# weilonghu/KGC-GCN

Hardware: NVIDIA B200
Metric: edges/sec GCN fwd+bwd (higher is better)
Workload: dtype f32

## Files before the change

### include/kgc_b200.h

```cpp
#ifndef KGC_B200_H_
#define KGC_B200_H_

#include <stddef.h>
#include <stdint.h>

#ifdef __cplusplus
extern "C" {
#endif
#if defined(__GNUC__)
#pragma GCC visibility push(default)
#endif

#define KGC_ABI_VERSION 1

typedef struct { int32_t beg, end, out, flags; } kgc_item_t;

#define KGC_CHUNK_EDGES 32
typedef struct { int32_t head_slot, tail_slot; } kgc_chunk_t;

typedef struct { int32_t eid, a, b; float norm; } kgc_edge_rec_t;

const char* kgc_last_error(void);
int kgc_abi_version(void);

size_t kgc_csr_workspace_bytes(int64_t n_edges2, int64_t n_nodes, int64_t n_types);
int kgc_csr_build(const int64_t* src, const int64_t* dst, const int64_t* type,
                  int64_t n_edges2, int64_t n_edges_in, int64_t n_nodes, int64_t n_dst_rows, int64_t dst_offset,
                  int64_t n_types, int32_t deg_given, int32_t* deg, float* norm,
                  int32_t* perm_dst, int32_t* rowptr_dst, int32_t* rowmid_dst, kgc_edge_rec_t* rec_dst,
                  int32_t* perm_src, int32_t* rowptr_src, kgc_edge_rec_t* rec_src,
                  int32_t* perm_type, int32_t* rowptr_type, kgc_edge_rec_t* rec_type,
                  int64_t type_block_rows, void* workspace, size_t workspace_bytes, void* stream);
int64_t kgc_csr_type_rows(int64_t n_nodes, int64_t n_types, int64_t type_block_rows);
int kgc_block_sum(const float* in, int64_t n_blocks, int64_t n, float* out, void* stream);

int kgc_stream_plan_flags(const int32_t* seg_beg, const int32_t* seg_end, const int32_t* seg_row, int64_t n_seg,
                          int64_t n_rec, int32_t chunk, uint32_t* rowflags, int32_t* rec_seg, int32_t* inter, void* stream);

int kgc_agg_fwd(const float* x, const float* rel, int64_t n_types, const float* ee,
                const kgc_edge_rec_t* rec_dst, const uint32_t* rowflags, const kgc_chunk_t* chunks, int64_t n_rec,
                float* out_final, float* carry, int32_t D, void* stream);

int kgc_rows_fill(const int32_t* rows, int64_t n_rows, const float* addend, float* out, int32_t D, void* stream);

int kgc_rows_reduce(const float* part_in, const kgc_item_t* items, int64_t n_items, int64_t n_large,
                    float* out_final, float* out_part, const float* addend, int32_t D, void* stream);

int kgc_agg_bwd_src(const float* x, const float* rel, int64_t n_types, const float* ee, const float* g3,
                    const kgc_edge_rec_t* rec_src, const uint32_t* rowflags, const kgc_chunk_t* chunks, int64_t n_rec,
                    int64_t n_dst_rows, int64_t n_edges_in, const float* loop_addend,
                    float* d_ee, float* dx_final, float* carry, int32_t D, void* stream);

int kgc_agg_bwd_rel(const float* x, const float* ee, const float* g3,
                    const kgc_edge_rec_t* rec_type, const uint32_t* rowflags, const kgc_chunk_t* chunks, int64_t n_rec,
                    int64_t n_dst_rows, int64_t n_edges_in,
                    float* drel_final, float* carry, int32_t D, void* stream);

int64_t kgc_tail_num_blocks(int64_t n_rows);
int kgc_dropout_mask(const int64_t* seed, int32_t plane, float drop_p, int64_t n_elem, uint8_t* mask, void* stream);
int32_t kgc_keep_pitch(void);
int kgc_tail_fwd(const float* res3, const uint8_t* mask_in, const uint8_t* mask_out, const int64_t* seed, float drop_p,
                 float keep_scale, const float* bias, int64_t n_rows, int32_t Dout, float* pre, double* partials,
                 uint8_t* keep, void* stream);
int kgc_colsum_finalize(const double* partials, int64_t n_blocks, int32_t Dout, double* sums, void* stream);
int kgc_colstats_from_sums(const double* sums, int64_t n_rows, int32_t Dout, float eps, int32_t training,
                           const float* running_mean, const float* running_var, float* stats, void* stream);
int kgc_colstats_finalize(const double* partials, int64_t n_blocks, int64_t n_rows, int32_t Dout, float eps,
                          float momentum, float* running_mean, float* running_var, int64_t* num_batches_tracked,
                          double* sums, float* stats, void* stream);
int kgc_colsum_finalize2(const double* partials, int64_t n_blocks, int32_t Dout, double* sums, float* sums32,
                         void* stream);
int kgc_tail_apply(const float* pre, const float* stats, const float* gamma, const float* beta,
                   int64_t n_rows, int32_t Dout, float* all_ent, const int64_t* out_seed, float out_drop_p,
                   uint8_t* out_keep, void* stream);
int kgc_tail_bwd_reduce(const float* g_ent, const float* pre, const float* stats, const float* gamma, const float* beta,
                        int64_t n_rows, int32_t Dout, double* partials, const uint8_t* out_keep, float out_scale,
                        void* stream);
int kgc_tail_bwd_apply(const float* g_ent, const float* pre, const float* stats, const float* gamma, const float* beta,
                       const double* sums, int32_t training, int64_t n_rows, int64_t n_rows_global, int32_t Dout,
                       float* d_out, const uint8_t* keep, float keep_scale, float* d_res2, const uint8_t* out_keep,
                       float out_scale, void* stream);

int kgc_conv_prep(const float* rels, int32_t n_rels, const float* loop_rel, const float* loop_edge, const float* w_in,
                  const float* w_out, const float* w_loop, const float* w_rel, int32_t D, int32_t Dout, float* relp,
                  float* all_rel, float* packed_fwd, float* packed_bwd, void* stream);
int kgc_conv_param_grads(const float* m_loop, const float* w_loop, const float* loop_rel, const float* loop_edge,
                         const float* relp, const float* w_rel, const float* g_rel, const float* d_relp,
                         int32_t n_rels, int32_t D, int32_t Dout, float* d_w_loop, float* d_loop_rel,
                         float* d_loop_edge, float* d_rels, float* d_w_rel, const float* rel_add, void* stream);

size_t kgc_gemm_packed_b_bytes(int32_t N, int32_t K);
int kgc_gemm_pack_b(const float* B, int64_t stride_k, int64_t stride_n, int32_t N, int32_t K, float* packed,
                    void* stream);
int kgc_gemm_nt(const float* A, int64_t M, int32_t K, int64_t lda, const float* packed_b, int32_t N, float* C,
                int64_t ldc, void* stream);
int kgc_gemm_nt_batch(int32_t n_prob, const float* const* A, int64_t M, int32_t K, int64_t lda,
                      const float* const* packed_b, int32_t N, float* const* C, int64_t ldc, void* stream);
int kgc_gemm_nt_batch_masked(int32_t n_prob, const float* const* A, int64_t M, int32_t K, int64_t lda,
                             const float* const* packed_b, int32_t N, float* const* C, int64_t ldc, const uint8_t* keep,
                             int32_t keep_pitch, float keep_scale, void* stream);
int kgc_gemm_nt_trans(const float* At, int64_t M, int32_t K, int64_t ldat, const float* packed_b, int32_t N,
                      float* Ct, int64_t ldct, void* stream);
void kgc_gemm_set_debug(long long* buf);

size_t kgc_gemm_tn_workspace_bytes(int64_t M, int32_t Ka, int32_t Nb);
int kgc_gemm_tn(const float* A, int64_t lda, const float* B, int64_t ldb, int64_t M, int32_t Ka, int32_t Nb,
                float* C, void* workspace, size_t workspace_bytes, void* stream);

size_t kgc_gemm_tn_tc_workspace_bytes(int64_t M, int32_t Ka, int32_t Nb);
int kgc_gemm_tn_tc(const float* A, int64_t lda, const float* B, int64_t ldb, int64_t M, int32_t Ka, int32_t Nb,
                   float* C, void* workspace, size_t workspace_bytes, void* stream);

int kgc_gemm_nt_splitk(const float* A, int64_t lda, const float* Bt, int64_t ldb, int64_t K, int32_t Ma, int32_t Nb,
                       float* C, void* workspace, size_t workspace_bytes, void* stream);

int kgc_gemm_tn_tc_batch(int32_t n_prob, const float* const* A, int64_t lda, const float* const* B, int64_t ldb,
                         int64_t M, int32_t Ka, int32_t Nb, float* const* C, void* workspace, size_t workspace_bytes,
                         void* stream);
int kgc_gemm_tn_tc_batch_masked(int32_t n_prob, const float* const* A, int64_t lda, const float* const* B, int64_t ldb,
                                int64_t M, int32_t Ka, int32_t Nb, float* const* C, void* workspace, size_t workspace_bytes,
                                const uint8_t* keep, int32_t keep_pitch, float keep_scale, void* stream);

int kgc_label_build(const int64_t* qid, int64_t B, const int64_t* triples, const int64_t* ptr,
                    const int32_t* idx, int64_t n_entity, float pos, float add,
                    int64_t* triple_out, float* label, void* stream);

int kgc_neg_sample(const int64_t* qid, int64_t B, const int64_t* ptr, const int32_t* idx, int64_t n_entity,
                   const uint32_t* draws, int32_t k, int32_t tries, int32_t* neg, void* stream);

int kgc_edge_sample(const int64_t* src, const int64_t* dst, const int64_t* type, int64_t n_triples, const uint32_t* draws,
                    int64_t m, int64_t* sub_src, int64_t* sub_dst, int64_t* sub_type, int64_t* eids, void* stream);

size_t kgc_bn2d_partials_bytes(int32_t C);
int kgc_bn2d_relu_drop_fwd(const float* x, int64_t B, int32_t C, int32_t HW, const float* gamma, const float* beta,
                           float* running_mean, float* running_var, float eps, float momentum, int32_t training,
                           int32_t relu, const int64_t* seed, float drop_p, double* partials, float* stats, float* y,
                           void* stream);
int kgc_bn2d_relu_drop_bwd(const float* dy, const float* x, int64_t B, int32_t C, int32_t HW, const float* gamma,
                           const float* beta, const float* stats, int32_t training, int32_t relu, const int64_t* seed,
                           float drop_p, double* partials, float* sums, float* dx, void* stream);

int kgc_conv1ch_supported(int32_t F, int32_t K, int32_t H, int32_t W);
size_t kgc_conv1ch_bwd_workspace_bytes(int64_t B, int32_t F, int32_t K);
int kgc_conv1ch_fwd(const float* x, const float* w, const float* bias, int64_t B, int32_t F, int32_t K, int32_t H,
                    int32_t W, float* y, void* stream);
int kgc_conv1ch_bwd(const float* dy, const float* x, const float* w, int64_t B, int32_t F, int32_t K, int32_t H,
                    int32_t W, float* dx, float* dw, void* workspace, void* stream);

typedef struct { float* param; const float* grad; float* exp_avg; float* exp_avg_sq; } kgc_opt_tensor_t;
int32_t kgc_opt_chunk_elems(void);
int kgc_clip_adam_step(const kgc_opt_tensor_t* tensors, const int32_t* items, int64_t n_items, const float* hyper,
                       double* state, double* partials, void* stream);

int kgc_p2p_allreduce(void* const* stage_ptrs_dev, int64_t offset_bytes, void* const* flag_ptrs_dev, int32_t rank,
                      int32_t world, uint32_t* epoch, int32_t* error, const void* in, void* out, int64_t n_bytes,
                      int32_t is_double, void* stream);
int kgc_p2p_barrier(void* const* flag_ptrs_dev, int32_t rank, int32_t world, uint32_t* epoch, int32_t* error, void* stream);
int kgc_p2p_halo_gather(void* const* table_ptrs_dev, int32_t rank, const int32_t* rows, const int32_t* order, int64_t n_rows,
                        int64_t block_rows, int32_t D, void* stream);
int kgc_p2p_halo_reduce(void* const* part_ptrs_dev, int32_t world, const int32_t* idx, const int32_t* row_ids, int64_t n_rows,
                        const float* addend, float* out, int32_t D, void* stream);

typedef struct kgc_ingest kgc_ingest_t;
int kgc_ingest_open(const char* data_dir, kgc_ingest_t** out);
void kgc_ingest_close(kgc_ingest_t* h);
int64_t kgc_ingest_count(const kgc_ingest_t* h, int32_t what);
int kgc_ingest_copy(const kgc_ingest_t* h, int32_t array, void* dst, int64_t capacity_bytes);
const char* kgc_ingest_name(const kgc_ingest_t* h, int32_t kind, int64_t id);

int kgc_score_1n_fwd(const float* ent, int64_t n_ent, int32_t D, int64_t ld_ent, const float* packed_x, int32_t B,
                     const float* bias, float* pred, int64_t ld_pred, void* stream);
int kgc_score_1n_logits(const float* ent, int64_t n_ent, int32_t D, int64_t ld_ent, const float* packed_x, int32_t B,
                        const float* bias, float* logits, int64_t ld_logits, void* stream);
int kgc_score_1n_bwd_logit(const float* d_pred, int64_t ld_dp, const float* pred, int64_t ld_p, int64_t n_ent,
                           int32_t B, int32_t ldt, float* d_logitT, float* d_bias, void* stream);

int64_t kgc_label_mask_words(int64_t n_entity);
int kgc_label_mask_build(const int64_t* qid, int64_t B, const int64_t* triples, const int64_t* ptr, const int32_t* idx,
                         int64_t n_entity, uint32_t* mask, int64_t* triple_out, void* stream);
int kgc_bce_1n_bwd_logit(const float* pred, int64_t ld_p, const uint32_t* mask, int64_t n_ent, int32_t B, int32_t ldt,
                         float pos, float add, float* d_logitT, float* d_bias, double* loss_partial, float* loss,
                         void* stream);
int kgc_score_1n_fwd_t(const float* ent, int64_t n_ent, int32_t D, int64_t ld_ent, const float* packed_x, int32_t B,
                       const float* bias, float* pred_t, int64_t ld_t, void* stream);
int64_t kgc_bce_1n_t_blocks(int64_t n_ent);
int kgc_label_mask_t_build(const int64_t* qid, int64_t B, const int64_t* ptr, const int32_t* idx, int64_t n_entity,
                           uint32_t* mask_t, void* stream);
int kgc_bce_1n_bwd_logit_t(float* pred_t, const uint32_t* mask_t, int64_t n_ent, int32_t B, int32_t ldt, float pos, float add,
                           float* d_bias, double* loss_partial, float* loss, void* stream);

int32_t kgc_score_kpad(int32_t d);
int kgc_score_pack_entities(const float* all_ent, const float* bias, int64_t n, int32_t d,
                            uint16_t* e_bf16, void* stream);
int kgc_score_pack_queries(const float* xq, int64_t b, int32_t d, uint16_t* q_bf16, void* stream);
size_t kgc_score_pairs_workspace_bytes(int64_t n_pairs, int32_t kpad);
int kgc_score_pairs(const uint16_t* q_bf16, const uint16_t* e_bf16, const int32_t* pair_q, const int32_t* pair_e,
                    int64_t n_pairs, int32_t kpad, float* s_out, void* workspace, size_t workspace_bytes,
                    void* stream);
int kgc_score_rank(const uint16_t* q_bf16, const uint16_t* e_bf16, int64_t b, int64_t n, int32_t kpad,
                   const float* thr, int32_t* count_gt, int32_t* count_eq, void* stream);
int kgc_rank_count_dense(const float* logits, int64_t ld, int64_t n_ent, int64_t b, const float* thr,
                         int32_t* count_gt, int32_t* count_eq, void* stream);
int kgc_rank_finalize(const int32_t* count_gt, const int32_t* count_eq, const float* thr, const float* s_filt,
                      const int64_t* filt_ptr, const int32_t* filt_idx, const int64_t* obj, int64_t b,
                      int32_t* ranks, int32_t* eq_out, double* sums13, void* stream);

#if defined(__GNUC__)
#pragma GCC visibility pop
#endif
#ifdef __cplusplus
}
#endif
#endif
```

### kgc-gcn_b200/_lib.py

```python
import ctypes
import os

import torch

_HERE = os.path.dirname(os.path.abspath(__file__))
LIB_PATH = os.environ.get('KGC_LIB_PATH') or os.path.join(_HERE, 'libkgc_b200.so')
_LIB = None

_vp, _i64, _i32, _f32, _sz = ctypes.c_void_p, ctypes.c_int64, ctypes.c_int32, ctypes.c_float, ctypes.c_size_t

SIGNATURES = {
    'kgc_last_error': (ctypes.c_char_p, []),
    'kgc_abi_version': (ctypes.c_int, []),
    'kgc_csr_workspace_bytes': (_sz, [_i64, _i64, _i64]),
    'kgc_csr_build': (ctypes.c_int, [_vp, _vp, _vp, _i64, _i64, _i64, _i64, _i64, _i64, _i32, _vp, _vp, _vp, _vp, _vp,
                                     _vp, _vp, _vp, _vp, _vp, _vp, _vp, _i64, _vp, _sz, _vp]),
    'kgc_csr_type_rows': (_i64, [_i64, _i64, _i64]),
    'kgc_block_sum': (ctypes.c_int, [_vp, _i64, _i64, _vp, _vp]),
    'kgc_stream_plan_flags': (ctypes.c_int, [_vp, _vp, _vp, _i64, _i64, _i32, _vp, _vp, _vp, _vp]),
    'kgc_agg_fwd': (ctypes.c_int, [_vp, _vp, _i64, _vp, _vp, _vp, _vp, _i64, _vp, _vp, _i32, _vp]),
    'kgc_rows_fill': (ctypes.c_int, [_vp, _i64, _vp, _vp, _i32, _vp]),
    'kgc_rows_reduce': (ctypes.c_int, [_vp, _vp, _i64, _i64, _vp, _vp, _vp, _i32, _vp]),
    'kgc_agg_bwd_src': (ctypes.c_int, [_vp, _vp, _i64, _vp, _vp, _vp, _vp, _vp, _i64, _i64, _i64, _vp, _vp, _vp, _vp, _i32, _vp]),
    'kgc_agg_bwd_rel': (ctypes.c_int, [_vp, _vp, _vp, _vp, _vp, _vp, _i64, _i64, _i64, _vp, _vp, _i32, _vp]),
    'kgc_tail_num_blocks': (_i64, [_i64]),
    'kgc_dropout_mask': (ctypes.c_int, [_vp, _i32, _f32, _i64, _vp, _vp]),
    'kgc_keep_pitch': (_i32, []),
    'kgc_tail_fwd': (ctypes.c_int, [_vp, _vp, _vp, _vp, _f32, _f32, _vp, _i64, _i32, _vp, _vp, _vp, _vp]),
    'kgc_colsum_finalize': (ctypes.c_int, [_vp, _i64, _i32, _vp, _vp]),
    'kgc_colstats_from_sums': (ctypes.c_int, [_vp, _i64, _i32, _f32, _i32, _vp, _vp, _vp, _vp]),
    'kgc_colstats_finalize': (ctypes.c_int, [_vp, _i64, _i64, _i32, _f32, _f32, _vp, _vp, _vp, _vp, _vp, _vp]),
    'kgc_colsum_finalize2': (ctypes.c_int, [_vp, _i64, _i32, _vp, _vp, _vp]),
    'kgc_tail_apply': (ctypes.c_int, [_vp, _vp, _vp, _vp, _i64, _i32, _vp, _vp, _f32, _vp, _vp]),
    'kgc_tail_bwd_reduce': (ctypes.c_int, [_vp, _vp, _vp, _vp, _vp, _i64, _i32, _vp, _vp, _f32, _vp]),
    'kgc_tail_bwd_apply': (ctypes.c_int, [_vp, _vp, _vp, _vp, _vp, _vp, _i32, _i64, _i64, _i32, _vp, _vp, _f32, _vp, _vp, _f32, _vp]),
    'kgc_gemm_packed_b_bytes': (_sz, [_i32, _i32]),
    'kgc_gemm_pack_b': (ctypes.c_int, [_vp, _i64, _i64, _i32, _i32, _vp, _vp]),
    'kgc_gemm_nt': (ctypes.c_int, [_vp, _i64, _i32, _i64, _vp, _i32, _vp, _i64, _vp]),
    'kgc_conv_prep': (ctypes.c_int, [_vp, _i32] + [_vp] * 6 + [_i32, _i32] + [_vp] * 5),
    'kgc_conv_param_grads': (ctypes.c_int, [_vp] * 8 + [_i32, _i32, _i32] + [_vp] * 7),
    'kgc_gemm_nt_batch': (ctypes.c_int, [_i32, _vp, _i64, _i32, _i64, _vp, _i32, _vp, _i64, _vp]),
    'kgc_gemm_nt_batch_masked': (ctypes.c_int, [_i32, _vp, _i64, _i32, _i64, _vp, _i32, _vp, _i64, _vp, _i32, _f32, _vp]),
    'kgc_gemm_tn_tc_batch_masked': (ctypes.c_int, [_i32, _vp, _i64, _vp, _i64, _i64, _i32, _i32, _vp, _vp, _sz, _vp, _i32, _f32, _vp]),
    'kgc_gemm_nt_trans': (ctypes.c_int, [_vp, _i64, _i32, _i64, _vp, _i32, _vp, _i64, _vp]),
    'kgc_gemm_nt_splitk': (ctypes.c_int, [_vp, _i64, _vp, _i64, _i64, _i32, _i32, _vp, _vp, _sz, _vp]),
    'kgc_gemm_set_debug': (None, [_vp]),
    'kgc_gemm_tn_workspace_bytes': (_sz, [_i64, _i32, _i32]),
    'kgc_gemm_tn_tc_workspace_bytes': (_sz, [_i64, _i32, _i32]),
    'kgc_gemm_tn_tc': (ctypes.c_int, [_vp, _i64, _vp, _i64, _i64, _i32, _i32, _vp, _vp, _sz, _vp]),
    'kgc_gemm_tn_tc_batch': (ctypes.c_int, [_i32, _vp, _i64, _vp, _i64, _i64, _i32, _i32, _vp, _vp, _sz, _vp]),
    'kgc_gemm_tn': (ctypes.c_int, [_vp, _i64, _vp, _i64, _i64, _i32, _i32, _vp, _vp, _sz, _vp]),
    'kgc_label_build': (ctypes.c_int, [_vp, _i64, _vp, _vp, _vp, _i64, _f32, _f32, _vp, _vp, _vp]),
    'kgc_neg_sample': (ctypes.c_int, [_vp, _i64, _vp, _vp, _i64, _vp, _i32, _i32, _vp, _vp]),
    'kgc_edge_sample': (ctypes.c_int, [_vp, _vp, _vp, _i64, _vp, _i64, _vp, _vp, _vp, _vp, _vp]),
    'kgc_bn2d_partials_bytes': (_sz, [_i32]),
    'kgc_bn2d_relu_drop_fwd': (ctypes.c_int, [_vp, _i64, _i32, _i32, _vp, _vp, _vp, _vp, _f32, _f32, _i32, _i32, _vp, _f32, _vp, _vp, _vp, _vp]),
    'kgc_bn2d_relu_drop_bwd': (ctypes.c_int, [_vp, _vp, _i64, _i32, _i32, _vp, _vp, _vp, _i32, _i32, _vp, _f32, _vp, _vp, _vp, _vp]),
    'kgc_conv1ch_supported': (_i32, [_i32, _i32, _i32, _i32]),
    'kgc_conv1ch_bwd_workspace_bytes': (_sz, [_i64, _i32, _i32]),
    'kgc_conv1ch_fwd': (ctypes.c_int, [_vp, _vp, _vp, _i64, _i32, _i32, _i32, _i32, _vp, _vp]),
    'kgc_conv1ch_bwd': (ctypes.c_int, [_vp, _vp, _vp, _i64, _i32, _i32, _i32, _i32, _vp, _vp, _vp, _vp]),
    'kgc_opt_chunk_elems': (_i32, []),
    'kgc_clip_adam_step': (ctypes.c_int, [_vp, _vp, _i64, _vp, _vp, _vp, _vp]),
    'kgc_p2p_allreduce': (ctypes.c_int, [_vp, _i64, _vp, _i32, _i32, _vp, _vp, _vp, _vp, _i64, _i32, _vp]),
    'kgc_p2p_barrier': (ctypes.c_int, [_vp, _i32, _i32, _vp, _vp, _vp]),
    'kgc_p2p_halo_gather': (ctypes.c_int, [_vp, _i32, _vp, _vp, _i64, _i64, _i32, _vp]),
    'kgc_p2p_halo_reduce': (ctypes.c_int, [_vp, _i32, _vp, _vp, _i64, _vp, _vp, _i32, _vp]),
    'kgc_ingest_open': (ctypes.c_int, [ctypes.c_char_p, _vp]),
    'kgc_ingest_close': (None, [_vp]),
    'kgc_ingest_count': (_i64, [_vp, _i32]),
    'kgc_ingest_copy': (ctypes.c_int, [_vp, _i32, _vp, _i64]),
    'kgc_ingest_name': (ctypes.c_char_p, [_vp, _i32, _i64]),
    'kgc_score_1n_fwd': (ctypes.c_int, [_vp, _i64, _i32, _i64, _vp, _i32, _vp, _vp, _i64, _vp]),
    'kgc_score_1n_logits': (ctypes.c_int, [_vp, _i64, _i32, _i64, _vp, _i32, _vp, _vp, _i64, _vp]),
    'kgc_rank_count_dense': (ctypes.c_int, [_vp, _i64, _i64, _i64, _vp, _vp, _vp, _vp]),
    'kgc_score_1n_bwd_logit': (ctypes.c_int, [_vp, _i64, _vp, _i64, _i64, _i32, _i32, _vp, _vp, _vp]),
    'kgc_label_mask_words': (_i64, [_i64]),
    'kgc_label_mask_build': (ctypes.c_int, [_vp, _i64, _vp, _vp, _vp, _i64, _vp, _vp, _vp]),
    'kgc_bce_1n_bwd_logit': (ctypes.c_int, [_vp, _i64, _vp, _i64, _i32, _i32, _f32, _f32, _vp, _vp, _vp, _vp, _vp]),
    'kgc_score_1n_fwd_t': (ctypes.c_int, [_vp, _i64, _i32, _i64, _vp, _i32, _vp, _vp, _i64, _vp]),
    'kgc_bce_1n_t_blocks': (_i64, [_i64]),
    'kgc_label_mask_t_build': (ctypes.c_int, [_vp, _i64, _vp, _vp, _i64, _vp, _vp]),
    'kgc_bce_1n_bwd_logit_t': (ctypes.c_int, [_vp, _vp, _i64, _i32, _i32, _f32, _f32, _vp, _vp, _vp, _vp]),
    'kgc_score_kpad': (_i32, [_i32]),
    'kgc_score_pack_entities': (ctypes.c_int, [_vp, _vp, _i64, _i32, _vp, _vp]),
    'kgc_score_pack_queries': (ctypes.c_int, [_vp, _i64, _i32, _vp, _vp]),
    'kgc_score_pairs_workspace_bytes': (_sz, [_i64, _i32]),
    'kgc_score_pairs': (ctypes.c_int, [_vp, _vp, _vp, _vp, _i64, _i32, _vp, _vp, _sz, _vp]),
    'kgc_score_rank': (ctypes.c_int, [_vp, _vp, _i64, _i64, _i32, _vp, _vp, _vp, _vp]),
    'kgc_rank_finalize': (ctypes.c_int, [_vp, _vp, _vp, _vp, _vp, _vp, _vp, _i64, _vp, _vp, _vp, _vp]),
}


def lib():
    global _LIB
    if _LIB is None:
        if not os.path.exists(LIB_PATH):
            raise RuntimeError('{} is missing: build it with `python -c "import __graft_entry__ as g; g.build()"` '
                               '(nvcc, sm_100a). There is no CPU or PyTorch fallback.'.format(LIB_PATH))
        handle = ctypes.CDLL(LIB_PATH)
        for name, (res, args) in SIGNATURES.items():
            fn = getattr(handle, name)
            fn.restype, fn.argtypes = res, args
        if handle.kgc_abi_version() != 1:
            raise RuntimeError('libkgc_b200.so ABI version mismatch')
        _LIB = handle
    return _LIB


LAUNCHES = 0
_KERNELS_PER_CALL = {'kgc_csr_build': 16, 'kgc_label_mask_build': 2, 'kgc_bce_1n_bwd_logit': 2, 'kgc_bce_1n_bwd_logit_t': 2, 'kgc_label_mask_t_build': 2, 'kgc_score_pairs': 3, 'kgc_rank_finalize': 2, 'kgc_gemm_tn': 2, 'kgc_gemm_tn_tc': 2, 'kgc_gemm_tn_tc_batch': 2, 'kgc_gemm_tn_tc_batch_masked': 2}


def call(name, *args):
    global LAUNCHES
    h = lib()
    LAUNCHES += _KERNELS_PER_CALL.get(name, 1)
    rc = getattr(h, name)(*args)
    if rc != 0:
        raise RuntimeError('{} failed: {}'.format(name, h.kgc_last_error().decode('utf-8', 'replace')))


_WARNED = set()


def library_path(site, reason):
    msg = 'kgc_gcn_b200: {} is running on the torch library path ({})'.format(site, reason)
    if os.environ.get('KGC_STRICT', '0') not in ('', '0'):
        raise RuntimeError(msg + ' and KGC_STRICT=1 forbids it')
    if site not in _WARNED:
        _WARNED.add(site)
        import warnings
        warnings.warn(msg, RuntimeWarning, stacklevel=3)


def ptr(t):
    return None if t is None else ctypes.c_void_p(t.data_ptr())


def stream():
    return ctypes.c_void_p(torch.cuda.current_stream().cuda_stream)


def require_cuda(t, dtype, name):
    if not (torch.is_tensor(t) and t.is_cuda):
        raise RuntimeError('{} must be a CUDA tensor: the M-GCN hot path runs on the GPU only (no CPU fallback)'.format(name))
    if t.dtype != dtype:
        raise TypeError('{} must be {}, got {}'.format(name, dtype, t.dtype))
    return t if t.is_contiguous() else t.contiguous()
```

### kgc-gcn_b200/conv.py

```python
import os

import torch
import torch.nn as nn

from . import _lib
from .plan import get_plan


def get_param(shape):
    param = nn.Parameter(torch.empty(*shape))
    nn.init.xavier_uniform_(param.data)
    return param


def _mm(a, b, out):
    return torch.mm(a, b, out=out)


def gemm_nt(a, b_kn, out, plan=None, tag='b', packed=None):
    M, K = a.shape
    N = out.shape[1]
    if a.stride(1) != 1 or out.stride(1) != 1:
        raise ValueError('gemm_nt needs unit inner strides')
    p = _lib.ptr
    if packed is None:
        nbytes = int(_lib.lib().kgc_gemm_packed_b_bytes(N, K))
        if nbytes == 0:
            raise ValueError('gemm_nt: unsupported shape K={} N={}'.format(K, N))
        packed = plan.scratch('gemm_pack_' + tag, (nbytes // 4,)) if plan is not None else \
            torch.empty((nbytes // 4,), dtype=torch.float32, device=a.device)
        _lib.call('kgc_gemm_pack_b', p(b_kn), b_kn.stride(0), b_kn.stride(1), N, K, p(packed), _lib.stream())
    dst = out if (out.data_ptr() % 16 == 0 and out.stride(0) % 4 == 0) else \
        torch.empty((M, (N + 3) // 4 * 4), dtype=torch.float32, device=a.device)[:, :N]
    _lib.call('kgc_gemm_nt', p(a), M, K, a.stride(0), p(packed), N, p(dst), dst.stride(0), _lib.stream())
    if dst is not out:
        out.copy_(dst)
    return out


def gemm_nt_batch(a_list, packed_list, out_list, keep=None, keep_scale=1.0):
    import ctypes
    n = len(a_list)
    M, K = a_list[0].shape
    N = out_list[0].shape[1]
    lda, ldc = a_list[0].stride(0), out_list[0].stride(0)
    for a, o in zip(a_list, out_list):
        if a.shape != (M, K) or o.shape != (M, N) or a.stride() != (lda, 1) or o.stride() != (ldc, 1):
            raise ValueError('gemm_nt_batch needs operands of identical shape and strides')
    arr = lambda ts: (ctypes.c_void_p * n)(*[t.data_ptr() for t in ts])
    if keep is not None:
        _lib.call('kgc_gemm_nt_batch_masked', n, arr(a_list), M, K, lda, arr(packed_list), N, arr(out_list), ldc,
                  _lib.ptr(keep), keep.stride(0), float(keep_scale), _lib.stream())
    else:
        _lib.call('kgc_gemm_nt_batch', n, arr(a_list), M, K, lda, arr(packed_list), N, arr(out_list), ldc, _lib.stream())
    return out_list


def gemm_tn_batch(a_list, b_list, out_list, plan=None, keep=None, keep_scale=1.0):
    import ctypes
    n = len(a_list)
    M, Ka = a_list[0].shape
    Nb = b_list[0].shape[1]
    lda, ldb = a_list[0].stride(0), b_list[0].stride(0)
    same = all(a.shape == (M, Ka) and b.shape == (M, Nb) and a.stride() == (lda, 1) and b.stride() == (ldb, 1)
               and o.is_contiguous() for a, b, o in zip(a_list, b_list, out_list))
    if not same or Ka > 128 or Nb > 224:
        if keep is not None:
            raise ValueError('gemm_tn_batch: the masked form needs Ka <= 128, Nb <= 224 and operands of identical shape')
        for a, b, o in zip(a_list, b_list, out_list):
            gemm_tn(a, b, o, plan)
        return out_list
    nbytes = int(_lib.lib().kgc_gemm_tn_tc_workspace_bytes(M, Ka, Nb))
    ws = plan.scratch('kgc_gemm_tn_tc_ws', (nbytes // 4,)) if plan is not None else \
        torch.empty((nbytes // 4,), dtype=torch.float32, device=a_list[0].device)
    arr = lambda ts: (ctypes.c_void_p * n)(*[t.data_ptr() for t in ts])
    if keep is not None:
        _lib.call('kgc_gemm_tn_tc_batch_masked', n, arr(a_list), lda, arr(b_list), ldb, M, Ka, Nb, arr(out_list), _lib.ptr(ws),
                  nbytes, _lib.ptr(keep), keep.stride(0), float(keep_scale), _lib.stream())
    else:
        _lib.call('kgc_gemm_tn_tc_batch', n, arr(a_list), lda, arr(b_list), ldb, M, Ka, Nb, arr(out_list), _lib.ptr(ws), nbytes,
                  _lib.stream())
    return out_list


def _pack_b(b_kn):
    K, N = b_kn.shape
    nbytes = int(_lib.lib().kgc_gemm_packed_b_bytes(N, K))
    if nbytes == 0:
        raise ValueError('unsupported small operand K={} N={} (K <= 256, N <= 1024)'.format(K, N))
    packed = torch.empty((nbytes // 4,), dtype=torch.float32, device=b_kn.device)
    _lib.call('kgc_gemm_pack_b', _lib.ptr(b_kn), b_kn.stride(0), b_kn.stride(1), N, K, _lib.ptr(packed), _lib.stream())
    return packed


def gemm_nt_trans(a_t, b_kn, out_t):
    K, M = a_t.shape
    N = b_kn.shape[1]
    if a_t.stride(1) != 1 or out_t.stride(1) != 1 or out_t.shape != (N, M):
        raise ValueError('gemm_nt_trans needs unit inner strides and out_t of shape [N, M]')
    p = _lib.ptr
    _lib.call('kgc_gemm_nt_trans', p(a_t), M, K, a_t.stride(0), p(_pack_b(b_kn)), N, p(out_t), out_t.stride(0), _lib.stream())
    return out_t


def gemm_nt_splitk(a, bt, out):
    Ma, K = a.shape
    Nb = bt.shape[0]
    if a.stride(1) != 1 or bt.stride(1) != 1 or not out.is_contiguous():
        raise ValueError('gemm_nt_splitk needs unit inner strides and a contiguous output')
    nbytes = int(_lib.lib().kgc_gemm_tn_tc_workspace_bytes(K, Ma, Nb))
    ws = torch.empty((nbytes // 4,), dtype=torch.float32, device=a.device)
    p = _lib.ptr
    _lib.call('kgc_gemm_nt_splitk', p(a), a.stride(0), p(bt), bt.stride(0), K, Ma, Nb, p(out), p(ws), nbytes, _lib.stream())
    return out


class _LinearFn(torch.autograd.Function):

    @staticmethod
    def forward(ctx, x, weight, bias):
        x_, w_ = x.detach(), weight.detach()
        y = gemm_nt_splitk(x_, w_, torch.empty((x_.shape[0], w_.shape[0]), dtype=torch.float32, device=x.device))
        if bias is not None:
            y += bias.detach()
        ctx.save_for_backward(x_, w_)
        ctx.has_bias = bias is not None
        return y

    @staticmethod
    def backward(ctx, dy):
        x, w = ctx.saved_tensors
        dy = dy.contiguous()
        dx = dw = db = None
        if ctx.needs_input_grad[0]:
            dx = gemm_nt_trans(w, dy.t(), torch.empty_like(x))
        if ctx.needs_input_grad[1]:
            dw = gemm_nt_trans(x, dy, torch.empty_like(w))
        if ctx.has_bias and ctx.needs_input_grad[2]:
            db = dy.sum(0)
        return dx, dw, db


def linear_tc_supported(x, weight):
    B, F = x.shape
    O = weight.shape[0]
    return (x.is_cuda and x.dtype == torch.float32 and weight.dtype == torch.float32 and x.is_contiguous()
            and weight.is_contiguous() and 0 < B <= 128 and O <= 224 and O % 4 == 0 and F % 32 == 0 and F >= 4096
            and x.data_ptr() % 16 == 0 and weight.data_ptr() % 16 == 0)


def linear_tc(x, weight, bias=None):
    return _LinearFn.apply(x, weight, bias)


def gemm_tn(a, b, out, plan=None, tensor_cores=True):
    M, Ka = a.shape
    Nb = b.shape[1]
    if a.stride(1) != 1 or b.stride(1) != 1 or not out.is_contiguous():
        raise ValueError('gemm_tn needs unit inner strides and a contiguous output')
    if Nb > 256:
        raise ValueError('gemm_tn supports Nb <= 256')
    name = 'kgc_gemm_tn_tc' if (tensor_cores and Nb <= 224) else 'kgc_gemm_tn'
    for i0 in range(0, Ka, 128):
        kb = min(128, Ka - i0)
        a_blk, out_blk = a[:, i0:i0 + kb], out[i0:i0 + kb]
        nbytes = int(getattr(_lib.lib(), name + '_workspace_bytes')(M, kb, Nb))
        ws = plan.scratch(name + '_ws', (nbytes // 4,)) if plan is not None else \
            torch.empty((nbytes // 4,), dtype=torch.float32, device=a.device)
        p = _lib.ptr
        _lib.call(name, p(a_blk), a.stride(0), p(b), b.stride(0), M, kb, Nb, p(out_blk), p(ws), nbytes, _lib.stream())
    return out


class _Done(object):

    def wait(self):
        return None


class _StreamJoin(object):

    def __init__(self, stream):
        self.stream = stream

    def wait(self):
        torch.cuda.current_stream().wait_stream(self.stream)


class _Collectives(object):

    def __init__(self, group, world, n_global, n_hub=0, hub_idx_mine=None, hub_rows_mine=None, p2p=None, rank=0,
                 halo_rows=None, n_loc=None):
        self.group, self.world, self.n_global, self.rank = group, int(world), int(n_global), int(rank)
        self.n_loc = None if n_loc is None else int(n_loc)
        self.p2p = p2p
        self.halo_rows = halo_rows
        self.n_hub, self.hub_idx_mine, self.hub_rows_mine = int(n_hub), hub_idx_mine, hub_rows_mine

    def sum_hub_rows(self, planes, n_loc):
        if self.n_hub == 0:
            return
        buf = planes[:, n_loc:, :].contiguous()
        self.all_reduce(buf, 'hub_f')
        if self.hub_idx_mine.numel():
            planes[:, self.hub_rows_mine, :] = buf[:, self.hub_idx_mine, :]

    def spread_hub_rows(self, planes, n_planes, n_loc):
        if self.n_hub == 0:
            return
        buf = torch.zeros((n_planes, self.n_hub, planes.shape[2]), dtype=planes.dtype, device=planes.device)
        if self.hub_idx_mine.numel():
            buf[:, self.hub_idx_mine, :] = planes[:n_planes, self.hub_rows_mine, :]
        self.all_reduce(buf, 'hub_b')
        planes[:n_planes, n_loc:, :] = buf

    def all_gather_rows(self, x_local, async_op=False):
        import torch.distributed as dist
        out = torch.empty((self.world * x_local.shape[0],) + tuple(x_local.shape[1:]), dtype=x_local.dtype,
                          device=x_local.device)
        work = dist.all_gather_into_tensor(out, x_local.contiguous(), group=self.group, async_op=async_op)
        return (out, work) if async_op else out

    def gather_compact(self, x_blk):
        full = self.all_gather_rows(x_blk)
        return torch.cat([x_blk, full.index_select(0, self.halo_rows)], 0)

    def reduce_compact(self, partial, block):
        full = partial.new_zeros((self.world * block, partial.shape[1]))
        full[self.rank * block:(self.rank + 1) * block] = partial[:block]
        full[self.halo_rows] = partial[block:block + self.halo_rows.numel()]
        return self.reduce_scatter_rows(full)

    def reduce_scatter_rows(self, full, async_op=False):
        import torch.distributed as dist
        rows = full.shape[0] // self.world
        if dist.get_backend(self.group) == 'gloo':
            dist.all_reduce(full, group=self.group)
            r = dist.get_rank(self.group)
            out = full[r * rows:(r + 1) * rows].clone()
            return (out, None) if async_op else out
        out = torch.empty((rows,) + tuple(full.shape[1:]), dtype=full.dtype, device=full.device)
        work = dist.reduce_scatter_tensor(out, full.contiguous(), group=self.group, async_op=async_op)
        return (out, work) if async_op else out

    def all_reduce(self, t, tag=None):
        if self.p2p is not None and tag is not None and self.p2p.all_reduce(t, tag):
            return t
        import torch.distributed as dist
        dist.all_reduce(t, group=self.group)
        return t


class _ConvFn(torch.autograd.Function):

    @staticmethod
    def forward(ctx, x, rels, ee, w_in, w_out, w_loop, w_rel, loop_rel, loop_edge, gamma, beta, bias,
                plan, mask_in, mask_out, keep_scale, training, running_mean, running_var, eps, coll, seed, drop_p,
                bn_track=None, out_drop=None):
        Nl, D = x.shape
        Dout = w_in.shape[1]
        p, st = _lib.ptr, _lib.stream
        x = _lib.require_cuda(x, torch.float32, 'x')
        ee = _lib.require_cuda(ee, torch.float32, 'edge_embs')
        n_global = Nl if coll is None else coll.n_global
        n_hub = 0 if coll is None else coll.n_hub
        n_loc = Nl if coll is None or coll.n_loc is None else coll.n_loc
        if not 0 <= n_loc - Nl <= 1:
            raise ValueError('x has {} rows, the partition expects {} or {}'.format(Nl, n_loc, n_loc - 1))
        Nb = n_loc + n_hub
        compact = coll is not None and coll.halo_rows is not None
        n_table = Nl if coll is None else (Nb + coll.halo_rows.numel() if compact else Nb * coll.world)
        hybrid = coll is not None and coll.p2p is not None and coll.p2p.hybrid
        n_dst = n_table if hybrid else Nb
        if ee.shape[0] != plan.num_edges2 or n_dst != plan.num_dst_rows or plan.num_nodes != n_table:
            raise ValueError('edge_embs / x do not match the graph plan')
        T = rels.shape[0] + 1
        if T != plan.num_types:
            raise ValueError('rels_embs rows + 1 must equal the number of edge types of the plan')
        nf = int(_lib.lib().kgc_gemm_packed_b_bytes(Dout, D)) // 4
        nbk = int(_lib.lib().kgc_gemm_packed_b_bytes(D, Dout)) // 4
        if nf == 0 or nbk == 0:
            raise ValueError('unsupported layer width {} -> {} (<= 256)'.format(D, Dout))
        relp = torch.empty((T, D), dtype=torch.float32, device=x.device)
        all_rel_pad = torch.empty((T, Dout), dtype=torch.float32, device=x.device)
        packed_f = torch.empty((3, nf), dtype=torch.float32, device=x.device)
        packed_b = torch.empty((4, nbk), dtype=torch.float32, device=x.device)
        rels_c, wts = rels.detach().contiguous(), [w.detach().contiguous() for w in (w_in, w_out, w_loop, w_rel)]
        main, side = torch.cuda.current_stream(), plan.side_stream()
        side.wait_stream(main)
        with torch.cuda.stream(side):
            _lib.call('kgc_conv_prep', p(rels_c), T - 1, p(loop_rel.detach()), p(loop_edge.detach()), p(wts[0]), p(wts[1]),
                      p(wts[2]), p(wts[3]), D, Dout, p(relp), p(all_rel_pad), p(packed_f), p(packed_b), st())
        gather = None
        if coll is None:
            x_full = x
        elif coll.p2p is not None:
            ex = coll.p2p.exchange_stream
            ex.wait_stream(main)
            with torch.cuda.stream(ex):
                x_full = coll.p2p.gather(x, fence=not training)
            gather = _StreamJoin(ex)
        elif compact:
            x_blk = x if Nb == Nl else torch.cat([x, x.new_zeros((Nb - Nl, D))], 0)
            x_full, gather = coll.gather_compact(x_blk), _Done()
        else:
            x_full, gather = coll.all_gather_rows(x if Nb == Nl else torch.cat([x, x.new_zeros((Nb - Nl, D))], 0),
                                                  async_op=True)

        res3 = plan.scratch('res3', (3, Nl, Dout))
        if gather is not None:
            main.wait_stream(side)
            gemm_nt(x, None, res3[2], packed=packed_f[2])
            gather.wait()
        if max(x_full.shape[0], 3 * n_dst, ee.shape[0]) * (D // 4) >= 1 << 32:
            raise ValueError('kgc_gcn_b200: node / edge tables of 2^32 float4 elements or more are not supported')
        agg = torch.empty((2, n_dst, D), dtype=torch.float32, device=x.device)

        def level0(sp, out_final, carry):
            _lib.call('kgc_agg_fwd', p(x_full), p(rels_c), T - 1, p(ee), p(plan.rec_dst), p(sp.rowflags), p(sp.chunks), sp.n_rec,
                      p(out_final), p(carry), D, st())
        plan.run_reduction(plan.fwd, level0, agg, D, tag='f')
        if gather is None:
            main.wait_stream(side)

        if hybrid:
            coll.p2p.reduce_agg(agg)
        if gather is not None:
            coll.sum_hub_rows(agg, n_loc)
            gemm_nt_batch([agg[0, :Nl], agg[1, :Nl]], [packed_f[0], packed_f[1]], [res3[0], res3[1]])
        else:
            gemm_nt_batch([agg[0], agg[1], x], [packed_f[0], packed_f[1], packed_f[2]], [res3[0], res3[1], res3[2]])

        nb = int(_lib.lib().kgc_tail_num_blocks(Nl))
        partials = plan.scratch('colpart', (nb, 2, Dout), torch.float64)
        sums = torch.empty((2, Dout), dtype=torch.float64, device=x.device)
        pre = torch.empty((Nl, Dout), dtype=torch.float32, device=x.device)
        stats = torch.empty((3, Dout), dtype=torch.float32, device=x.device)
        all_ent = torch.empty((Nl, Dout), dtype=torch.float32, device=x.device)
        dropping = (mask_in is not None or seed is not None) and drop_p > 0.0
        keep = torch.empty((Nl, int(_lib.lib().kgc_keep_pitch())), dtype=torch.uint8, device=x.device) if dropping else None
        _lib.call('kgc_tail_fwd', p(res3), p(mask_in), p(mask_out), p(seed), float(drop_p), float(keep_scale), p(bias),
                  Nl, Dout, p(pre), p(partials), p(keep), st())
        if training and coll is None:
            mom, nbt = bn_track if bn_track is not None else (0.0, None)
            _lib.call('kgc_colstats_finalize', p(partials), nb, n_global, Dout, float(eps), float(mom),
                      p(running_mean) if bn_track is not None else None, p(running_var) if bn_track is not None else None,
                      p(nbt), None, p(stats), st())
        else:
            if training:
                _lib.call('kgc_colsum_finalize', p(partials), nb, Dout, p(sums), st())
                coll.all_reduce(sums, 'bn_f')
            _lib.call('kgc_colstats_from_sums', p(sums), n_global, Dout, float(eps), int(training), p(running_mean),
                      p(running_var), p(stats), st())
        out_p, out_seed = out_drop if out_drop is not None else (0.0, None)
        out_keep = torch.empty((Nl, int(_lib.lib().kgc_keep_pitch())), dtype=torch.uint8, device=x.device) if out_seed is not None else None
        _lib.call('kgc_tail_apply', p(pre), p(stats), p(gamma), p(beta), Nl, Dout, p(all_ent), p(out_seed), float(out_p),
                  p(out_keep), st())
        ctx.out_scale = 1.0 / (1.0 - float(out_p)) if out_seed is not None else 1.0
        all_rel = all_rel_pad[:-1]

        ctx.plan, ctx.training, ctx.keep_scale, ctx.has_bias, ctx.coll = plan, bool(training), float(keep_scale), \
            bias is not None, coll
        ctx.drop_p = float(drop_p)
        ctx.save_for_backward(x, x_full, relp, ee, w_in, w_out, w_loop, w_rel, loop_rel, loop_edge, gamma, beta, agg, pre,
                              all_ent, stats, keep, packed_b, out_keep)
        ctx.mark_non_differentiable(stats)
        return all_ent, all_rel, stats

    @staticmethod
    def backward(ctx, g_ent, g_rel, _g_stats):
        (x, x_full, relp, ee, w_in, w_out, w_loop, w_rel, loop_rel, loop_edge, gamma, beta, agg, pre, all_ent, stats, keep,
         packed_b, out_keep) = ctx.saved_tensors
        plan, coll = ctx.plan, ctx.coll
        Nl, D = x.shape
        n_global = Nl if coll is None else coll.n_global
        n_hub = 0 if coll is None else coll.n_hub
        n_loc = Nl if coll is None or coll.n_loc is None else coll.n_loc
        Nb = n_loc + n_hub
        Dout = w_in.shape[1]
        T = relp.shape[0]
        p, st = _lib.ptr, _lib.stream
        dev = x.device
        if g_ent is None:
            g_ent = torch.zeros_like(all_ent)
        g_ent = g_ent.contiguous()

        nb = int(_lib.lib().kgc_tail_num_blocks(Nl))
        partials = plan.scratch('colpart', (nb, 2, Dout), torch.float64)
        sums = torch.empty((2, Dout), dtype=torch.float64, device=dev)
        d_out = plan.scratch('d_out', (Nl, Dout))
        _lib.call('kgc_tail_bwd_reduce', p(g_ent), p(pre), p(stats), p(gamma), p(beta), Nl, Dout, p(partials), p(out_keep),
                  ctx.out_scale, st())
        if coll is None:
            sums32 = torch.empty((2, Dout), dtype=torch.float32, device=dev)
            _lib.call('kgc_colsum_finalize2', p(partials), nb, Dout, p(sums), p(sums32), st())
        else:
            _lib.call('kgc_colsum_finalize', p(partials), nb, Dout, p(sums), st())
            coll.all_reduce(sums, 'bn_b')
            sums32 = sums.float()
        mode = os.environ.get('KGC_TAIL_PLANES', '')
        three = (3 * Nl * Dout * 4 > (48 << 20)) if mode not in ('1', '3') else mode == '3'
        d_res2 = plan.scratch('d_res2', (2, Nl, Dout)) if three else None
        _lib.call('kgc_tail_bwd_apply', p(g_ent), p(pre), p(stats), p(gamma), p(beta), p(sums), int(ctx.training), Nl,
                  n_global, Dout, p(d_out), p(keep), ctx.keep_scale, p(d_res2), p(out_keep), ctx.out_scale, st())
        ups = [d_res2[0], d_res2[1], d_out] if three else [d_out, d_out, d_out]
        gkeep = None if three else keep
        d_beta, d_gamma = sums32[0], sums32[1]

        flat = torch.empty((3 * D * Dout + T * D + (Dout if ctx.has_bias else 0),), dtype=torch.float32, device=dev)
        d_w_in, d_w_out, m_loop = (flat[k * D * Dout:(k + 1) * D * Dout].view(D, Dout) for k in range(3))
        d_relp = flat[3 * D * Dout:3 * D * Dout + T * D].view(T, D)
        main, side = torch.cuda.current_stream(), plan.side_stream()
        side.wait_stream(main)
        with torch.cuda.stream(side):
            gemm_tn_batch([agg[0, :Nl], agg[1, :Nl], x], ups, [d_w_in, d_w_out, m_loop], plan,
                          keep=gkeep, keep_scale=ctx.keep_scale)
            if ctx.has_bias:
                torch.sum(d_out, 0, out=flat[3 * D * Dout + T * D:])

        hybrid = coll is not None and coll.p2p is not None and coll.p2p.hybrid
        g3 = coll.p2p.g3_planes() if hybrid else plan.scratch('g3', (3, Nb, D))
        gemm_nt_batch(ups, [packed_b[0], packed_b[1], packed_b[2]],
                      [g3[0, :Nl], g3[1, :Nl], g3[2, :Nl]], keep=gkeep, keep_scale=ctx.keep_scale)
        if n_hub:
            coll.spread_hub_rows(g3, 2, n_loc)
        if hybrid:
            coll.p2p.gather_g()
        p2p = None if coll is None else coll.p2p
        d_x_full = p2p.partial if (p2p is not None and not hybrid) else torch.empty((plan.num_nodes, D), dtype=torch.float32, device=dev)
        d_ee = torch.empty_like(ee)
        loop_addend = g3[2] if (coll is None or hybrid) else None

        def level0_src(sp, out_final, carry):
            _lib.call('kgc_agg_bwd_src', p(x_full), p(relp), relp.shape[0], p(ee), p(g3), p(plan.rec_src), p(sp.rowflags), p(sp.chunks),
                      sp.n_rec, plan.num_dst_rows, plan.num_edges_in, p(loop_addend), p(d_ee), p(out_final), p(carry),
                      D, st())
        plan.run_reduction(plan.bwd_src, level0_src, d_x_full, D, addend=loop_addend, tag='s')
        scatter = None
        if hybrid:
            ex = p2p.exchange_stream
            ex.wait_stream(main)
            with torch.cuda.stream(ex):
                p2p.reduce_dx(d_x_full, channel=1)
            d_x = d_x_full[:Nl]
        elif p2p is not None:
            d_x = torch.empty((Nl, D), dtype=torch.float32, device=dev)
            ex = p2p.exchange_stream
            ex.wait_stream(main)
            with torch.cuda.stream(ex):
                p2p.reduce(g3[2, :Nl], Nl, out=d_x, channel=1)
        compact = coll is not None and coll.halo_rows is not None
        if coll is not None and p2p is None and not compact:
            d_x, scatter = coll.reduce_scatter_rows(d_x_full, async_op=True)

        def level0_rel(sp, out_final, carry):
            _lib.call('kgc_agg_bwd_rel', p(x_full), p(ee), p(g3), p(plan.rec_type), p(sp.rowflags), p(sp.chunks), sp.n_rec,
                      plan.num_dst_rows, plan.num_edges_in, p(out_final), p(carry), D, st())
        plan.run_rel_reduction(level0_rel, d_relp, D)

        main.wait_stream(side)
        if coll is None:
            d_x = d_x_full
        elif p2p is not None:
            coll.all_reduce(flat, 'flat')
            main.wait_stream(p2p.exchange_stream)
        elif compact:
            coll.all_reduce(flat, 'flat')
            d_x = coll.reduce_compact(d_x_full, Nb)[:Nl] + g3[2, :Nl]
        else:
            coll.all_reduce(flat, 'flat')
            if scatter is not None:
                scatter.wait()
            d_x = d_x[:Nl] + g3[2, :Nl]
        d_bias = flat[3 * D * Dout + T * D:] * 3.0 if ctx.has_bias else None
        small = torch.empty((2 * D * Dout + 2 * D + (T - 1) * D,), dtype=torch.float32, device=dev)
        d_w_loop, d_w_rel = small[:D * Dout].view(D, Dout), small[D * Dout:2 * D * Dout].view(D, Dout)
        o = 2 * D * Dout
        d_loop_rel, d_loop_edge, d_rels = small[o:o + D].view(1, D), small[o + D:o + 2 * D].view(1, D), small[o + 2 * D:].view(T - 1, D)
        g_rel_c = None if g_rel is None else g_rel.contiguous()
        rel_add = None
        if g_rel_c is not None and T - 1 >= 256 and g_rel_c.data_ptr() % 16 == 0 and Dout % 4 == 0 and (D * Dout) % 32 == 0:
            rel_add = gemm_nt(g_rel_c, None, torch.empty((T - 1, D), dtype=torch.float32, device=dev), packed=packed_b[3])
            gemm_tn(relp[:T - 1], g_rel_c, d_w_rel, plan)
        _lib.call('kgc_conv_param_grads', p(m_loop), p(w_loop.detach().contiguous()), p(loop_rel.detach()), p(loop_edge.detach()),
                  p(relp), p(w_rel.detach().contiguous()), p(g_rel_c), p(d_relp), T - 1, D, Dout, p(d_w_loop), p(d_loop_rel),
                  p(d_loop_edge), p(d_rels), p(d_w_rel), p(rel_add), st())
        return (d_x, d_rels, d_ee, d_w_in, d_w_out, d_w_loop, d_w_rel, d_loop_rel, d_loop_edge, d_gamma, d_beta, d_bias,
                None, None, None, None, None, None, None, None, None, None, None, None, None)


class MGCNConv(nn.Module):

    def __init__(self, in_channels, out_channels, num_relations, bias=False, dropout=0.1, **kwargs):
        super(MGCNConv, self).__init__()
        self.in_channels = in_channels
        self.out_channels = out_channels
        self.num_relations = num_relations
        self.aggr = 'add'

        self.ent_bn = nn.BatchNorm1d(out_channels)
        self.drop = nn.Dropout(dropout)
        self.act = torch.tanh

        self.loop_weight = get_param((in_channels, out_channels))
        self.in_weight = get_param((in_channels, out_channels))
        self.out_weight = get_param((in_channels, out_channels))
        self.rels_weight = get_param((in_channels, out_channels))
        self.loop_rel = get_param((1, in_channels))
        self.loop_edge = get_param((1, in_channels))

        if bias is True:
            self.register_parameter('bias', nn.Parameter(torch.zeros(out_channels)))
        else:
            self.register_parameter('bias', None)
        self._forced_masks = None
        self.register_buffer('_drop_seed', torch.zeros(1, dtype=torch.int64), persistent=False)
        self._drop_seeded = False

    def set_dropout_masks(self, mask_in, mask_out):
        self._forced_masks = None if mask_in is None else (mask_in, mask_out)

    def compute_norm(self, edge_index, num_ent):
        ei = torch.cat([edge_index, edge_index], 1).contiguous()
        et = torch.zeros(ei.size(1), dtype=torch.int64, device=ei.device)
        return get_plan(ei, et, num_ent, 1).norm[:edge_index.size(1)].clone()

    def _masks(self, n_rows, device):
        p = self.drop.p
        if not self.training or p == 0.0:
            return None, None, 1.0, None, 0.0
        if self._forced_masks is not None:
            m_in, m_out = self._forced_masks
            return (m_in.to(device=device, dtype=torch.uint8).contiguous(),
                    m_out.to(device=device, dtype=torch.uint8).contiguous(), 1.0 / (1.0 - p), None, p)
        if not self._drop_seeded:
            self._drop_seed.fill_(int(torch.randint(0, 2 ** 62, (1,)).item()))
            self._drop_seeded = True
        self._drop_seed.add_(0x9E3779B97F4A7C15 & 0x7FFFFFFFFFFFFFFF)
        return None, None, 1.0 / (1.0 - p), self._drop_seed.clone(), p

    def _out_drop_cfg(self, p, seed):
        if not self.training or not p or p <= 0.0:
            return None
        if seed is None:
            if not self._drop_seeded:
                self._drop_seed.fill_(int(torch.randint(0, 2 ** 62, (1,)).item()))
                self._drop_seeded = True
            self._drop_seed.add_(0x9E3779B97F4A7C15 & 0x7FFFFFFFFFFFFFFF)
            seed = self._drop_seed.clone()
        self._last_out_seed = seed
        return float(p), seed

    def dropout_masks(self, seed, n_rows):
        out = []
        for plane in (0, 1):
            m = torch.empty((n_rows, self.out_channels), dtype=torch.uint8, device=seed.device)
            _lib.call('kgc_dropout_mask', _lib.ptr(seed), plane, float(self.drop.p), m.numel(), _lib.ptr(m), _lib.stream())
            out.append(m)
        return out

    def forward(self, x, edge_index, edge_type, edge_norm, edge_embs, rels_embs, size=None, _out_drop=0.0):
        num_ent = x.size(0)
        plan = get_plan(edge_index, edge_type, num_ent, rels_embs.size(0) + 1)
        m_in, m_out, keep_scale, seed, drop_p = self._masks(num_ent, x.device)
        self._last_seed = seed
        bn = self.ent_bn
        use_batch_stats = self.training or bn.running_mean is None
        track = self.training and bn.track_running_stats and bn.running_mean is not None
        fused = track and bn.momentum is not None
        all_ent, all_rel, stats = _ConvFn.apply(
            x, rels_embs, edge_embs, self.in_weight, self.out_weight, self.loop_weight, self.rels_weight,
            self.loop_rel, self.loop_edge, bn.weight, bn.bias, self.bias, plan, m_in, m_out, keep_scale,
            use_batch_stats, bn.running_mean, bn.running_var, bn.eps, None, seed, drop_p,
            (float(bn.momentum), bn.num_batches_tracked) if fused else None, self._out_drop_cfg(_out_drop, seed))
        if track and not fused:
            self._update_running_stats(stats, num_ent)
        return all_ent, all_rel

    def _update_running_stats(self, stats, n_rows):
        bn = self.ent_bn
        if self.training and bn.track_running_stats and bn.running_mean is not None:
            with torch.no_grad():
                bn.num_batches_tracked += 1
                mom = bn.momentum if bn.momentum is not None else 1.0 / float(bn.num_batches_tracked)
                unbias = float(n_rows) / float(max(n_rows - 1, 1))
                bn.running_mean.mul_(1.0 - mom).add_(stats[0], alpha=mom)
                bn.running_var.mul_(1.0 - mom).add_(stats[1], alpha=mom * unbias)

    def forward_partitioned(self, x_local, part, edge_embs_local, rels_embs):
        m_in, m_out, keep_scale, seed, drop_p = self._masks(x_local.size(0), x_local.device)
        if seed is not None:
            seed = seed + part.rank
        self._last_seed = seed
        bn = self.ent_bn
        use_batch_stats = self.training or bn.running_mean is None
        coll = _Collectives(part.group, part.world, part.num_nodes, part.n_hub, part.hub_idx_mine, part.hub_rows_mine,
                            part.p2p(x_local.shape[1]), part.rank, getattr(part, 'halo_rows64', None), part.n_loc)
        all_ent, all_rel, stats = _ConvFn.apply(
            x_local, rels_embs, edge_embs_local, self.in_weight, self.out_weight, self.loop_weight, self.rels_weight,
            self.loop_rel, self.loop_edge, bn.weight, bn.bias, self.bias, part.plan, m_in, m_out, keep_scale,
            use_batch_stats, bn.running_mean, bn.running_var, bn.eps, coll, seed, drop_p)
        self._update_running_stats(stats, part.num_nodes)
        return all_ent, all_rel

    def __repr__(self):
        return '{}({}, {}, num_relations={})'.format(self.__class__.__name__, self.in_channels, self.out_channels,
                                                     self.num_relations)
```

### kgc-gcn_b200/csrc/common.cuh

```cuda
#pragma once
#include <cuda_runtime.h>
#include <stdint.h>
#include <stdio.h>
#include <string>

#include "kgc_b200.h"

namespace kgc {

void set_error(const std::string& msg);

inline int fail(const char* where, const std::string& what) {
  set_error(std::string(where) + ": " + what);
  return 1;
}

#define KGC_CUDA_TRY(expr)                                                          \
  do {                                                                              \
    cudaError_t _e = (expr);                                                        \
    if (_e != cudaSuccess) return ::kgc::fail(__func__, std::string(#expr) + " -> " + cudaGetErrorString(_e)); \
  } while (0)

#define KGC_REQUIRE(cond, msg)                          \
  do {                                                  \
    if (!(cond)) return ::kgc::fail(__func__, (msg));   \
  } while (0)

#define KGC_LAUNCH_CHECK() KGC_CUDA_TRY(cudaGetLastError())

inline cudaStream_t as_stream(void* s) { return reinterpret_cast<cudaStream_t>(s); }

constexpr int kNumSMs = 148;

struct SmemAttrCache {
  size_t set[64] = {0};
  template <typename Kernel>
  cudaError_t ensure(Kernel kern, size_t smem) {
    int dev = 0;
    cudaError_t e = cudaGetDevice(&dev);
    if (e != cudaSuccess) return e;
    const bool tracked = dev >= 0 && dev < 64;
    if (tracked && smem <= set[dev]) return cudaSuccess;
    e = cudaFuncSetAttribute(kern, cudaFuncAttributeMaxDynamicSharedMemorySize, (int)smem);
    if (e == cudaSuccess && tracked) set[dev] = smem;
    return e;
  }
};

__host__ __device__ inline int64_t ceil_div(int64_t a, int64_t b) { return (a + b - 1) / b; }

__device__ __forceinline__ float4 ld_stream(const float4* p) {
  float4 r;
  asm volatile("ld.global.nc.L1::no_allocate.v4.f32 {%0,%1,%2,%3}, [%4];"
               : "=f"(r.x), "=f"(r.y), "=f"(r.z), "=f"(r.w)
               : "l"(p));
  return r;
}
__device__ __forceinline__ void st_stream(float4* p, const float4& v) {
  asm volatile("st.global.L1::no_allocate.v4.f32 [%0], {%1,%2,%3,%4};" ::"l"(p), "f"(v.x), "f"(v.y), "f"(v.z),
               "f"(v.w));
}
__device__ __forceinline__ int4 ld_rec(const kgc_edge_rec_t* p) {
  return __ldg(reinterpret_cast<const int4*>(p));
}

__device__ __forceinline__ uint4 philox4x32_10(uint4 c, uint2 k) {
#pragma unroll
  for (int r = 0; r < 10; ++r) {
    const uint32_t hi0 = __umulhi(0xD2511F53u, c.x), lo0 = 0xD2511F53u * c.x;
    const uint32_t hi1 = __umulhi(0xCD9E8D57u, c.z), lo1 = 0xCD9E8D57u * c.z;
    c = make_uint4(hi1 ^ c.y ^ k.x, lo1, hi0 ^ c.w ^ k.y, lo0);
    k.x += 0x9E3779B9u;
    k.y += 0xBB67AE85u;
  }
  return c;
}
__device__ __forceinline__ float4 philox_mask4(int64_t idx4, uint32_t plane, uint64_t seed, uint32_t drop_thr, float s) {
  const uint4 r = philox4x32_10(make_uint4((uint32_t)idx4, (uint32_t)(idx4 >> 32), plane, 0u),
                                make_uint2((uint32_t)seed, (uint32_t)(seed >> 32)));
  return make_float4(r.x >= drop_thr ? s : 0.f, r.y >= drop_thr ? s : 0.f, r.z >= drop_thr ? s : 0.f,
                     r.w >= drop_thr ? s : 0.f);
}

inline void ensure_thread_context() {
  static thread_local bool done = false;
  if (!done) {
    cudaFree(nullptr);
    done = true;
  }
}

}
```

### kgc-gcn_b200/csrc/gemm_tf32x3.cu

```cuda
#include <cuda.h>

#include <cstdlib>
#include "common.cuh"

namespace kgc {
namespace {

constexpr int kBM = 128;
constexpr int kBK = 32;
constexpr int kUK = 8;
constexpr int kMaxKB = 8;
constexpr int kMaxStages = 8;
constexpr int kAStages = 4;
constexpr int kAccCols = 256;
constexpr int kTmemColsTS = kAccCols + kAStages * 64;
constexpr int kTileA = kBM * kBK * 4;
constexpr int kThreadsG = 480;
constexpr int kSplitWarps = 8;
constexpr int kBBudget = 116 * 1024;
constexpr int kTmemColsG = 256;
constexpr int kEpiBuf = 32 * 128;
constexpr int kEpiStage = 4 * 2 * kEpiBuf;

__device__ __forceinline__ uint32_t s_u32(const void* p) { return (uint32_t)__cvta_generic_to_shared(p); }
__device__ __forceinline__ void mb_init(uint64_t* bar, uint32_t count) {
  asm volatile("mbarrier.init.shared::cta.b64 [%0], %1;" ::"r"(s_u32(bar)), "r"(count));
}
__device__ __forceinline__ void mb_expect_tx(uint64_t* bar, uint32_t bytes) {
  asm volatile("mbarrier.arrive.expect_tx.shared::cta.b64 _, [%0], %1;" ::"r"(s_u32(bar)), "r"(bytes) : "memory");
}
__device__ __forceinline__ void mb_arrive(uint64_t* bar) {
  asm volatile("mbarrier.arrive.shared::cta.b64 _, [%0];" ::"r"(s_u32(bar)) : "memory");
}
__device__ __forceinline__ void mb_wait(uint64_t* bar, uint32_t parity) {
  asm volatile(
      "{\n"
      ".reg .pred P1;\n"
      "LAB_WAIT:\n"
      "mbarrier.try_wait.parity.shared::cta.b64 P1, [%0], %1;\n"
      "@P1 bra DONE;\n"
      "bra LAB_WAIT;\n"
      "DONE:\n"
      "}" ::"r"(s_u32(bar)),
      "r"(parity)
      : "memory");
}
__device__ __forceinline__ void tma_2d(void* smem_dst, const CUtensorMap* map, uint64_t* bar, int c0, int c1) {
  asm volatile(
      "cp.async.bulk.tensor.2d.shared::cluster.global.mbarrier::complete_tx::bytes [%0], [%1, {%3, %4}], [%2];" ::"r"(
          s_u32(smem_dst)),
      "l"(reinterpret_cast<uint64_t>(map)), "r"(s_u32(bar)), "r"(c0), "r"(c1)
      : "memory");
}
__device__ __forceinline__ void tma_3d(void* smem_dst, const CUtensorMap* map, uint64_t* bar, int c0, int c1, int c2) {
  asm volatile(
      "cp.async.bulk.tensor.3d.shared::cluster.global.mbarrier::complete_tx::bytes [%0], [%1, {%3, %4, %5}], [%2];" ::"r"(
          s_u32(smem_dst)),
      "l"(reinterpret_cast<uint64_t>(map)), "r"(s_u32(bar)), "r"(c0), "r"(c1), "r"(c2)
      : "memory");
}
__device__ __forceinline__ void tma_store_2d(const CUtensorMap* map, const void* smem_src, int c0, int c1) {
  asm volatile("cp.async.bulk.tensor.2d.global.shared::cta.bulk_group [%0, {%2, %3}], [%1];" ::"l"(
                   reinterpret_cast<uint64_t>(map)),
               "r"(s_u32(smem_src)), "r"(c0), "r"(c1)
               : "memory");
}
__device__ __forceinline__ void tma_store_3d(const CUtensorMap* map, const void* smem_src, int c0, int c1, int c2) {
  asm volatile("cp.async.bulk.tensor.3d.global.shared::cta.bulk_group [%0, {%2, %3, %4}], [%1];" ::"l"(
                   reinterpret_cast<uint64_t>(map)),
               "r"(s_u32(smem_src)), "r"(c0), "r"(c1), "r"(c2)
               : "memory");
}
__device__ __forceinline__ void umma_tf32(uint32_t tmem_d, uint64_t adesc, uint64_t bdesc, uint32_t idesc, uint32_t acc) {
  asm volatile(
      "{\n"
      ".reg .pred p;\n"
      "setp.ne.b32 p, %4, 0;\n"
      "tcgen05.mma.cta_group::1.kind::tf32 [%0], %1, %2, %3, p;\n"
      "}" ::"r"(tmem_d),
      "l"(adesc), "l"(bdesc), "r"(idesc), "r"(acc)
      : "memory");
}
__device__ __forceinline__ void umma_tf32_ts(uint32_t tmem_d, uint32_t a_tmem, uint64_t bdesc, uint32_t idesc, uint32_t acc) {
  asm volatile(
      "{\n"
      ".reg .pred p;\n"
      "setp.ne.b32 p, %4, 0;\n"
      "tcgen05.mma.cta_group::1.kind::tf32 [%0], [%1], %2, %3, p;\n"
      "}" ::"r"(tmem_d),
      "r"(a_tmem), "l"(bdesc), "r"(idesc), "r"(acc)
      : "memory");
}
__device__ __forceinline__ void tmem_st16_g(uint32_t taddr, const uint32_t (&v)[16]) {
  asm volatile(
      "tcgen05.st.sync.aligned.32x32b.x16.b32 [%0], "
      "{%1, %2, %3, %4, %5, %6, %7, %8, %9, %10, %11, %12, %13, %14, %15, %16};" ::"r"(taddr),
      "r"(v[0]), "r"(v[1]), "r"(v[2]), "r"(v[3]), "r"(v[4]), "r"(v[5]), "r"(v[6]), "r"(v[7]), "r"(v[8]), "r"(v[9]),
      "r"(v[10]), "r"(v[11]), "r"(v[12]), "r"(v[13]), "r"(v[14]), "r"(v[15])
      : "memory");
}
__device__ __forceinline__ bool elect_one() {
  uint32_t pred = 0;
  asm volatile(
      "{\n"
      ".reg .b32 rx;\n"
      ".reg .pred px;\n"
      "elect.sync rx|px, 0xFFFFFFFF;\n"
      "@px mov.s32 %0, 1;\n"
      "}"
      : "+r"(pred));
  return pred != 0;
}
__device__ __forceinline__ uint32_t tf32_rn(float v) { return (__float_as_uint(v) + 0x1000u) & 0xFFFFE000u; }
__device__ __forceinline__ void split_tf32(uint32_t v, uint32_t& hi, uint32_t& lo) {
  hi = tf32_rn(__uint_as_float(v));
  lo = tf32_rn(__uint_as_float(v) - __uint_as_float(hi));
}
__device__ __forceinline__ void umma_commit_g(uint64_t* bar) {
  asm volatile("tcgen05.commit.cta_group::1.mbarrier::arrive::one.shared::cluster.b64 [%0];" ::"r"(s_u32(bar)) : "memory");
}
__device__ __forceinline__ void tmem_ld32_g(uint32_t taddr, uint32_t (&v)[32]) {
  asm volatile(
      "tcgen05.ld.sync.aligned.32x32b.x32.b32 "
      "{%0, %1, %2, %3, %4, %5, %6, %7, %8, %9, %10, %11, %12, %13, %14, %15, "
      "%16, %17, %18, %19, %20, %21, %22, %23, %24, %25, %26, %27, %28, %29, %30, %31}, [%32];"
      : "=r"(v[0]), "=r"(v[1]), "=r"(v[2]), "=r"(v[3]), "=r"(v[4]), "=r"(v[5]), "=r"(v[6]), "=r"(v[7]), "=r"(v[8]),
        "=r"(v[9]), "=r"(v[10]), "=r"(v[11]), "=r"(v[12]), "=r"(v[13]), "=r"(v[14]), "=r"(v[15]), "=r"(v[16]),
        "=r"(v[17]), "=r"(v[18]), "=r"(v[19]), "=r"(v[20]), "=r"(v[21]), "=r"(v[22]), "=r"(v[23]), "=r"(v[24]),
        "=r"(v[25]), "=r"(v[26]), "=r"(v[27]), "=r"(v[28]), "=r"(v[29]), "=r"(v[30]), "=r"(v[31])
      : "r"(taddr));
}
__device__ __forceinline__ uint64_t sw128_desc(uint32_t smem_addr) {
  uint64_t d = 0;
  d |= (uint64_t)((smem_addr & 0x3FFFF) >> 4);
  d |= (uint64_t)(1024 >> 4) << 32;
  d |= (uint64_t)1 << 46;
  d |= (uint64_t)2 << 61;
  return d;
}

constexpr int kMaxBatch = 3;
struct GemmMaps {
  CUtensorMap a[kMaxBatch], bhi[kMaxBatch], blo[kMaxBatch], c[kMaxBatch], c16[kMaxBatch];
};

struct GemmParams {
  int64_t M;
  int32_t n_prob;
  int32_t N, K;
  int32_t n_kb, ksteps, NT, n_ntiles, n_mtiles, stages;
  float* C;
  int64_t ldc;
  const float* row_bias;
  int32_t act;
  int32_t trans_c;
  int32_t trans_a;
  const uint8_t* keep;
  int32_t keep_pitch;
  float keep_scale;
  long long* dbg;
};

__global__ void __launch_bounds__(kThreadsG, 1)
gemm_tf32x3_kernel(const __grid_constant__ GemmMaps maps, const GemmParams P) {
  extern __shared__ uint8_t smem_raw[];
  if (P.dbg != nullptr && threadIdx.x == 0) {
    long long g;
    asm volatile("mov.u64 %0, %globaltimer;" : "=l"(g));
    atomicMin(reinterpret_cast<long long*>(P.dbg) + 8 * 64 + 0, g);
    if (blockIdx.x == 0) { P.dbg[8 * 64 + 2] = g; P.dbg[8 * 64 + 3] = clock64(); }
  }
  uint8_t* base = reinterpret_cast<uint8_t*>((reinterpret_cast<uintptr_t>(smem_raw) + 1023) & ~uintptr_t(1023));
  const int warp = threadIdx.x / 32, lane = threadIdx.x % 32;
  const int tile_b = P.NT * kBK * 4;
  const int tile_b_al = (tile_b + 1023) & ~1023;
  uint8_t* s_bhi = base;
  uint8_t* s_blo = s_bhi + P.n_kb * tile_b_al;
  const int kStages = P.stages;
  uint8_t* s_a = s_blo + P.n_kb * tile_b_al;
  uint8_t* s_stage = s_a + kStages * kTileA;
  uint64_t* bars = reinterpret_cast<uint64_t*>(s_stage + kEpiStage);
  uint64_t* b_full = bars;
  uint64_t* raw_full = bars + 1;
  uint64_t* raw_empty = raw_full + kMaxStages;
  uint64_t* split_full = raw_empty + kMaxStages;
  uint64_t* split_empty = split_full + kAStages;
  uint64_t* acc_full = split_empty + kAStages;
  uint64_t* acc_empty = acc_full + 2;
  uint32_t* tmem_slot = reinterpret_cast<uint32_t*>(acc_empty + 2);

  if (warp == 0 && lane == 0) {
    mb_init(b_full, 1);
    for (int i = 0; i < kStages; ++i) {
      mb_init(raw_full + i, 1);
      mb_init(raw_empty + i, kSplitWarps);
    }
    for (int i = 0; i < kAStages; ++i) {
      mb_init(split_full + i, kSplitWarps);
      mb_init(split_empty + i, 1);
    }
    for (int i = 0; i < 2; ++i) {
      mb_init(acc_full + i, 1);
      mb_init(acc_empty + i, 4);
    }
    asm volatile("fence.mbarrier_init.release.cluster;" ::: "memory");
    asm volatile("fence.proxy.async.shared::cta;" ::: "memory");
  }
  if (warp == 14) {
    asm volatile("tcgen05.alloc.cta_group::1.sync.aligned.shared::cta.b32 [%0], %1;" ::"r"(s_u32(tmem_slot)), "r"(kTmemColsTS)
                 : "memory");
    asm volatile("tcgen05.relinquish_alloc_permit.cta_group::1.sync.aligned;" ::: "memory");
  }
  asm volatile("tcgen05.fence::before_thread_sync;" ::: "memory");
  __syncthreads();
  asm volatile("tcgen05.fence::after_thread_sync;" ::: "memory");
  const uint32_t tmem_base = *tmem_slot;
  const uint32_t tmem_a = tmem_base + kAccCols;
  const bool dbg_on = P.dbg != nullptr && blockIdx.x == 0;
  int dbg_n = 0;
#define KGC_DBG(role) do { if (dbg_on && dbg_n < 64) P.dbg[(role) * 64 + dbg_n++] = clock64(); } while (0)

  const int groups = P.n_prob * P.n_ntiles;
  const int prob = (blockIdx.x % groups) / P.n_ntiles;
  const int nt = blockIdx.x % P.n_ntiles;
  const int first = blockIdx.x / groups;
  const int step = gridDim.x / groups;
  const CUtensorMap* map_a = &maps.a[prob];
  const CUtensorMap* map_bhi = &maps.bhi[prob];
  const CUtensorMap* map_blo = &maps.blo[prob];
  const CUtensorMap* map_c = &maps.c[prob];
  const CUtensorMap* map_c16 = &maps.c16[prob];

  if (warp == 0) {
    if (lane == 0) {
      mb_expect_tx(b_full, 2u * P.n_kb * tile_b);
      for (int kb = 0; kb < P.n_kb; ++kb) {
        tma_2d(s_bhi + kb * tile_b_al, map_bhi, b_full, kb * kBK, nt * P.NT);
        tma_2d(s_blo + kb * tile_b_al, map_blo, b_full, kb * kBK, nt * P.NT);
      }
      int stage = 0;
      uint32_t phase = 0;
      for (int mt = first; mt < P.n_mtiles; mt += step) {
        for (int kb = 0; kb < P.n_kb; ++kb) {
          mb_wait(raw_empty + stage, phase ^ 1);
          KGC_DBG(0);
          mb_expect_tx(raw_full + stage, kTileA);
          if (P.trans_a) tma_3d(s_a + stage * kTileA, map_a, raw_full + stage, 0, kb * kBK, mt * (kBM / 32));
          else tma_2d(s_a + stage * kTileA, map_a, raw_full + stage, kb * kBK, mt * kBM);
          if (++stage == kStages) { stage = 0; phase ^= 1; }
        }
      }
    }
  } else if (warp >= 2 && warp < 2 + kSplitWarps) {
    const int quarter = warp % 4, half = (warp - 2) / 4;
    const int r = quarter * 32 + lane;
    int stage = 0, ts = 0;
    uint32_t phase = 0, tphase = 0;
    const bool masked = P.keep != nullptr && prob < 2 && !P.trans_a;
    uint32_t kcur[kMaxKB], knxt[kMaxKB];
#pragma unroll
    for (int j = 0; j < kMaxKB; ++j) kcur[j] = knxt[j] = 0u;
    auto load_keep = [&](int mt_, uint32_t (&w)[kMaxKB]) {
      const int64_t grow = (int64_t)mt_ * kBM + r;
      if (mt_ < P.n_mtiles && grow < P.M) {
        const uint4* kp = reinterpret_cast<const uint4*>(P.keep + grow * P.keep_pitch);
#pragma unroll
        for (int q = 0; q < kMaxKB / 2; ++q) {
          const uint4 t4 = __ldg(kp + q);
          w[2 * q] = half ? t4.y : t4.x;
          w[2 * q + 1] = half ? t4.w : t4.z;
        }
      }
    };
    if (masked) load_keep(first, knxt);
    for (int mt = first; mt < P.n_mtiles; mt += step) {
      if (masked) {
#pragma unroll
        for (int j = 0; j < kMaxKB; ++j) kcur[j] = knxt[j];
        load_keep(mt + step, knxt);
      }
      for (int kb = 0; kb < P.n_kb; ++kb) {
        uint32_t kw = 0;
        if (masked) {
#pragma unroll
          for (int j = 0; j < kMaxKB; ++j)
            if (kb == j) kw = kcur[j];
          if (prob == 1) kw >>= 4;
        }
        mb_wait(raw_full + stage, phase);
        if (warp == 2 && lane == 0) KGC_DBG(1);
        uint32_t h[16], l[16];
        if (P.trans_a) {
          const uint8_t* col = s_a + stage * kTileA + quarter * 4096 + ((lane & 3) << 2);
#pragma unroll
          for (int i = 0; i < 16; ++i) {
            const int kk = half * 16 + i;
            const uint32_t v = *reinterpret_cast<const uint32_t*>(col + kk * 128 + (((lane >> 2) ^ (kk & 7)) << 4));
            split_tf32(v, h[i], l[i]);
          }
        } else {
          const uint8_t* row = s_a + stage * kTileA + r * 128;
          uint4 v[4];
#pragma unroll
          for (int i = 0; i < 4; ++i) v[i] = *reinterpret_cast<const uint4*>(row + (((half * 4 + i) ^ (r & 7)) << 4));
          if (masked) {
#pragma unroll
            for (int i = 0; i < 4; ++i) {
              const uint32_t nb = kw >> (8 * i);
              v[i].x = (nb & 1u) ? __float_as_uint(__uint_as_float(v[i].x) * P.keep_scale) : 0u;
              v[i].y = (nb & 2u) ? __float_as_uint(__uint_as_float(v[i].y) * P.keep_scale) : 0u;
              v[i].z = (nb & 4u) ? __float_as_uint(__uint_as_float(v[i].z) * P.keep_scale) : 0u;
              v[i].w = (nb & 8u) ? __float_as_uint(__uint_as_float(v[i].w) * P.keep_scale) : 0u;
            }
          }
#pragma unroll
          for (int i = 0; i < 4; ++i) {
            split_tf32(v[i].x, h[4 * i + 0], l[4 * i + 0]);
            split_tf32(v[i].y, h[4 * i + 1], l[4 * i + 1]);
            split_tf32(v[i].z, h[4 * i + 2], l[4 * i + 2]);
            split_tf32(v[i].w, h[4 * i + 3], l[4 * i + 3]);
          }
        }
        __syncwarp();
        if (lane == 0) mb_arrive(raw_empty + stage);
        mb_wait(split_empty + ts, tphase ^ 1);
        if (warp == 2 && lane == 0) KGC_DBG(2);
        asm volatile("tcgen05.fence::after_thread_sync;" ::: "memory");
        const uint32_t taddr = tmem_a + ((uint32_t)(quarter * 32) << 16) + ts * 64 + half * 16;
        tmem_st16_g(taddr, h);
        tmem_st16_g(taddr + 32, l);
        asm volatile("tcgen05.wait::st.sync.aligned;" ::: "memory");
        asm volatile("tcgen05.fence::before_thread_sync;" ::: "memory");
        __syncwarp();
        if (lane == 0) mb_arrive(split_full + ts);
        if (warp == 2 && lane == 0) KGC_DBG(3);
        if (++stage == kStages) { stage = 0; phase ^= 1; }
        if (++ts == kAStages) { ts = 0; tphase ^= 1; }
      }
    }
  } else if (warp == 1) {
    {
      const uint32_t idesc = (1u << 4) | (2u << 7) | (2u << 10) | ((uint32_t)(P.NT >> 3) << 17) | ((uint32_t)(kBM >> 4) << 24);
      int ts = 0, acc = 0;
      uint32_t tphase = 0, acc_phase = 0;
      mb_wait(b_full, 0);
      asm volatile("tcgen05.fence::after_thread_sync;" ::: "memory");
      for (int mt = first; mt < P.n_mtiles; mt += step) {
        mb_wait(acc_empty + acc, acc_phase ^ 1);
        asm volatile("tcgen05.fence::after_thread_sync;" ::: "memory");
        const uint32_t d_addr = tmem_base + acc * (kAccCols / 2);
        for (int kb = 0; kb < P.n_kb; ++kb) {
          mb_wait(split_full + ts, tphase);
          if (lane == 0) KGC_DBG(4);
          asm volatile("tcgen05.fence::after_thread_sync;" ::: "memory");
          const int nk = min(kBK / kUK, P.ksteps - kb * (kBK / kUK));
          const uint32_t a_hi = tmem_a + ts * 64, a_lo = a_hi + 32;
          const uint64_t b_hi = sw128_desc(s_u32(s_bhi + kb * tile_b_al));
          const uint64_t b_lo = sw128_desc(s_u32(s_blo + kb * tile_b_al));
          if (elect_one()) {
#pragma unroll
            for (int k = 0; k < kBK / kUK; ++k) {
              if (k < nk) {
                umma_tf32_ts(d_addr, a_lo + 8 * k, b_hi + 2 * k, idesc, (k != 0 || kb != 0) ? 1u : 0u);
                umma_tf32_ts(d_addr, a_hi + 8 * k, b_lo + 2 * k, idesc, 1u);
                umma_tf32_ts(d_addr, a_hi + 8 * k, b_hi + 2 * k, idesc, 1u);
              }
            }
            umma_commit_g(split_empty + ts);
            if (kb == P.n_kb - 1) umma_commit_g(acc_full + acc);
          }
          __syncwarp();
          if (lane == 0) KGC_DBG(5);
          if (++ts == kAStages) { ts = 0; tphase ^= 1; }
        }
        if (++acc == 2) { acc = 0; acc_phase ^= 1; }
      }
    }
  } else if (warp >= 10 && warp <= 13) {
    const int quarter = warp % 4;
    uint8_t* stg = s_stage + (warp - 10) * (2 * kEpiBuf);
    const int64_t row_q = quarter * 32;
    int acc = 0, buf = 0;
    uint32_t acc_phase = 0;
    for (int mt = first; mt < P.n_mtiles; mt += step) {
      mb_wait(acc_full + acc, acc_phase);
      if (warp == 10 && lane == 0) KGC_DBG(6);
      asm volatile("tcgen05.fence::after_thread_sync;" ::: "memory");
      const int64_t m0 = (int64_t)mt * kBM + row_q;
      const uint32_t taddr = tmem_base + ((uint32_t)(quarter * 32) << 16) + acc * (kAccCols / 2);
      for (int c0 = 0; c0 < P.NT; c0 += 32) {
        uint32_t v[32];
        tmem_ld32_g(taddr + c0, v);
        asm volatile("tcgen05.wait::ld.sync.aligned;" ::: "memory");
        if (c0 + 32 >= P.NT) {
          asm volatile("tcgen05.fence::before_thread_sync;" ::: "memory");
          __syncwarp();
          if (lane == 0) mb_arrive(acc_empty + acc);
        }
        if (lane == 0) asm volatile("cp.async.bulk.wait_group.read 1;" ::: "memory");
        __syncwarp();
        uint8_t* bb = stg + buf * kEpiBuf;
        const bool wide = c0 + 32 <= P.NT;
        if (P.row_bias != nullptr) {
          const float bv = m0 + lane < P.M ? P.row_bias[m0 + lane] : 0.f;
#pragma unroll
          for (int j = 0; j < 32; ++j) {
            const float z = __uint_as_float(v[j]) + bv;
            v[j] = __float_as_uint(P.act == 1 ? 1.f / (1.f + expf(-z)) : z);
          }
        }
        if (P.trans_c) {
#pragma unroll
          for (int j = 0; j < 32; ++j)
            *reinterpret_cast<uint32_t*>(bb + j * 128 + ((((lane >> 2) ^ (j & 7)) << 4) | ((lane & 3) << 2))) = v[j];
        } else if (wide) {
          uint8_t* bx = bb + lane * 128;
          const int sw = lane & 7;
#pragma unroll
          for (int q = 0; q < 8; ++q)
            *reinterpret_cast<uint4*>(bx + ((q ^ sw) << 4)) = make_uint4(v[4 * q], v[4 * q + 1], v[4 * q + 2], v[4 * q + 3]);
        } else {
          uint8_t* bx = bb + lane * 64;
          const int sw = (lane >> 1) & 3;
#pragma unroll
          for (int q = 0; q < 4; ++q)
            *reinterpret_cast<uint4*>(bx + ((q ^ sw) << 4)) = make_uint4(v[4 * q], v[4 * q + 1], v[4 * q + 2], v[4 * q + 3]);
        }
        asm volatile("fence.proxy.async.shared::cta;" ::: "memory");
        __syncwarp();
        if (lane == 0) {
          const int col = nt * P.NT + c0;
          if (m0 < P.M && col < P.N) {
            if (P.trans_c) tma_store_2d(wide ? map_c : map_c16, bb, (int)m0, col);
            else tma_store_2d(wide ? map_c : map_c16, bb, col, (int)m0);
          }
          asm volatile("cp.async.bulk.commit_group;" ::: "memory");
        }
        buf ^= 1;
      }
      if (warp == 10 && lane == 0) KGC_DBG(7);
      if (++acc == 2) { acc = 0; acc_phase ^= 1; }
    }
    if (lane == 0) asm volatile("cp.async.bulk.wait_group 0;" ::: "memory");
  }
  asm volatile("tcgen05.fence::before_thread_sync;" ::: "memory");
  __syncthreads();
  if (P.dbg != nullptr && threadIdx.x == 0) {
    long long g;
    asm volatile("mov.u64 %0, %globaltimer;" : "=l"(g));
    atomicMax(reinterpret_cast<long long*>(P.dbg) + 8 * 64 + 1, g);
    if (blockIdx.x == 0) { P.dbg[8 * 64 + 4] = g; P.dbg[8 * 64 + 5] = clock64(); }
  }
  if (warp == 14) {
    asm volatile("tcgen05.dealloc.cta_group::1.sync.aligned.b32 %0, %1;" ::"r"(tmem_base), "r"(kTmemColsTS) : "memory");
  }
}

__global__ void pack_b_kernel(const float* __restrict__ B, int64_t sk, int64_t sn, int N, int K, int n_pad, int k_pad,
                              float* __restrict__ hi, float* __restrict__ lo) {
  const int i = blockIdx.x * blockDim.x + threadIdx.x;
  if (i >= n_pad * k_pad) return;
  const int n = i / k_pad, k = i % k_pad;
  float v = 0.f;
  if (n < N && k < K) v = B[(int64_t)k * sk + (int64_t)n * sn];
  uint32_t h, l;
  split_tf32(__float_as_uint(v), h, l);
  hi[i] = __uint_as_float(h);
  lo[i] = __uint_as_float(l);
}

struct PrepArgs {
  const float *rels, *loop_rel, *loop_edge, *w0, *w1, *w2, *w_rel;
  int n_rels, D, Dout;
  int n_pad_f, k_pad_f, n_pad_b, k_pad_b;
  float *relp, *all_rel, *packed_f, *packed_b;
};

__global__ void __launch_bounds__(256) conv_prep_kernel(const PrepArgs a) {
  const int T = a.n_rels + 1;
  int i = blockIdx.x * blockDim.x + threadIdx.x;
  const int n0 = T * a.D, n1 = T * a.Dout, nf = a.n_pad_f * a.k_pad_f, nb = a.n_pad_b * a.k_pad_b;
  if (i < n0) {
    const int t = i / a.D, c = i % a.D;
    a.relp[i] = t < a.n_rels ? a.rels[i] : a.loop_rel[c];
    return;
  }
  i -= n0;
  if (i < n1) {
    const int t = i / a.Dout, o = i % a.Dout;
    const float* r = t < a.n_rels ? a.rels + (int64_t)t * a.D : a.loop_rel;
    float acc = 0.f;
#pragma unroll 25
    for (int c = 0; c < a.D; ++c) acc = fmaf(r[c], a.w_rel[(int64_t)c * a.Dout + o], acc);
    a.all_rel[i] = acc;
    return;
  }
  i -= n1;
  if (i < 3 * nf) {
    const int h = i / nf, j0 = i % nf, k = j0 / a.n_pad_f, n = j0 % a.n_pad_f, j = n * a.k_pad_f + k;
    float v = 0.f;
    if (n < a.Dout && k < a.D) {
      const float* wh = h == 0 ? a.w0 : (h == 1 ? a.w1 : a.w2);
      v = wh[(int64_t)k * a.Dout + n];
      if (h == 2) v *= a.loop_rel[k] * a.loop_edge[k];
    }
    uint32_t hi, lo;
    split_tf32(__float_as_uint(v), hi, lo);
    float* dst = a.packed_f + (int64_t)h * 2 * nf;
    dst[j] = __uint_as_float(hi);
    dst[nf + j] = __uint_as_float(lo);
    return;
  }
  i -= 3 * nf;
  if (i < 4 * nb) {
    const int h = i / nb, j = i % nb, n = j / a.k_pad_b, k = j % a.k_pad_b;
    float v = 0.f;
    if (n < a.D && k < a.Dout) {
      const float* wh = h == 0 ? a.w0 : (h == 1 ? a.w1 : (h == 2 ? a.w2 : a.w_rel));
      v = wh[(int64_t)n * a.Dout + k];
      if (h == 2) v *= a.loop_rel[n] * a.loop_edge[n];
    }
    uint32_t hi, lo;
    split_tf32(__float_as_uint(v), hi, lo);
    float* dst = a.packed_b + (int64_t)h * 2 * nb;
    dst[j] = __uint_as_float(hi);
    dst[nb + j] = __uint_as_float(lo);
  }
}

struct ParamGradArgs {
  const float *m_loop, *w_loop, *loop_rel, *loop_edge, *relp, *w_rel, *g_rel, *d_relp;
  int n_rels, D, Dout;
  float *d_w_loop, *d_loop_rel, *d_loop_edge, *d_rels, *d_w_rel;
};

__global__ void __launch_bounds__(256) conv_param_grads_kernel(const ParamGradArgs a) {
  const int T = a.n_rels + 1;
  int i = blockIdx.x * blockDim.x + threadIdx.x;
  const int nw = a.D * a.Dout;
  if (i < nw) {
    const int c = i / a.Dout;
    a.d_w_loop[i] = a.loop_rel[c] * a.loop_edge[c] * a.m_loop[i];
    return;
  }
  i -= nw;
  if (i < nw) {
    const int c = i / a.Dout, o = i % a.Dout;
    float acc = 0.f;
    if (a.g_rel != nullptr) {
#pragma unroll 8
      for (int t = 0; t < a.n_rels; ++t) acc = fmaf(a.relp[(int64_t)t * a.D + c], a.g_rel[(int64_t)t * a.Dout + o], acc);
    }
    a.d_w_rel[i] = acc;
    return;
  }
  i -= nw;
  const int pair = i / 32, lane = i % 32;
  if (pair < T * a.D) {
    const int t = pair / a.D, c = pair % a.D;
    const float* u = t < a.n_rels ? a.g_rel + (int64_t)t * a.Dout : a.m_loop + (int64_t)c * a.Dout;
    const float* w = t < a.n_rels ? a.w_rel + (int64_t)c * a.Dout : a.w_loop + (int64_t)c * a.Dout;
    float acc = 0.f;
    if (t == a.n_rels || a.g_rel != nullptr)
      for (int o = lane; o < a.Dout; o += 32) acc = fmaf(u[o], w[o], acc);
#pragma unroll
    for (int s = 16; s > 0; s >>= 1) acc += __shfl_xor_sync(0xFFFFFFFFu, acc, s);
    if (lane == 0) {
      const float val = a.d_relp[pair];
      if (t < a.n_rels) {
        a.d_rels[pair] = val + acc;
      } else {
        a.d_loop_edge[c] = acc * a.loop_rel[c];
        a.d_loop_rel[c] = acc * a.loop_edge[c] + val;
      }
    }
  }
}

__global__ void __launch_bounds__(256) conv_param_grads2_kernel(const ParamGradArgs a, const float* __restrict__ rel_add) {
  int i = blockIdx.x * blockDim.x + threadIdx.x;
  const int nw = a.D * a.Dout;
  if (i < nw) {
    const int c = i / a.Dout;
    a.d_w_loop[i] = a.loop_rel[c] * a.loop_edge[c] * a.m_loop[i];
    return;
  }
  i -= nw;
  const int n_el = a.n_rels * a.D, n_el_pad = (n_el + 31) & ~31;
  if (i < n_el_pad) {
    if (i < n_el) a.d_rels[i] = a.d_relp[i] + rel_add[i];
    return;
  }
  i -= n_el_pad;
  const int c = i / 32, lane = i % 32;
  if (c < a.D) {
    const float* u = a.m_loop + (int64_t)c * a.Dout;
    const float* w = a.w_loop + (int64_t)c * a.Dout;
    float acc = 0.f;
    for (int o = lane; o < a.Dout; o += 32) acc = fmaf(u[o], w[o], acc);
#pragma unroll
    for (int s = 16; s > 0; s >>= 1) acc += __shfl_xor_sync(0xFFFFFFFFu, acc, s);
    if (lane == 0) {
      a.d_loop_edge[c] = acc * a.loop_rel[c];
      a.d_loop_rel[c] = acc * a.loop_edge[c] + a.d_relp[(int64_t)a.n_rels * a.D + c];
    }
  }
}

typedef CUresult (*EncodeTiledFn)(CUtensorMap*, CUtensorMapDataType, cuuint32_t, void*, const cuuint64_t*, const cuuint64_t*,
                                  const cuuint32_t*, const cuuint32_t*, CUtensorMapInterleave, CUtensorMapSwizzle,
                                  CUtensorMapL2promotion, CUtensorMapFloatOOBfill);
int encode_fn(EncodeTiledFn* out) {
  ensure_thread_context();
  static EncodeTiledFn cached = nullptr;
  if (!cached) {
    void* fn = nullptr;
    cudaDriverEntryPointQueryResult qres;
    KGC_CUDA_TRY(cudaGetDriverEntryPoint("cuTensorMapEncodeTiled", &fn, cudaEnableDefault, &qres));
    KGC_REQUIRE(qres == cudaDriverEntryPointSuccess && fn != nullptr, "cuTensorMapEncodeTiled not available");
    cached = reinterpret_cast<EncodeTiledFn>(fn);
  }
  *out = cached;
  return 0;
}
int make_map_f32(CUtensorMap* map, const void* ptr, int64_t rows, int64_t cols, int64_t pitch, int box_rows,
                 CUtensorMapSwizzle swizzle = CU_TENSOR_MAP_SWIZZLE_128B, int box_cols = kBK) {
  EncodeTiledFn enc;
  if (encode_fn(&enc)) return 1;
  KGC_REQUIRE((reinterpret_cast<uintptr_t>(ptr) & 15) == 0 && (pitch * 4) % 16 == 0, "operand must be 16-byte aligned with a 16-byte pitch");
  cuuint64_t dims[2] = {(cuuint64_t)cols, (cuuint64_t)rows};
  cuuint64_t strides[1] = {(cuuint64_t)pitch * 4};
  cuuint32_t box[2] = {(cuuint32_t)box_cols, (cuuint32_t)box_rows};
  cuuint32_t estr[2] = {1, 1};
  CUresult r = enc(map, CU_TENSOR_MAP_DATA_TYPE_FLOAT32, 2, const_cast<void*>(ptr), dims, strides, box, estr,
                   CU_TENSOR_MAP_INTERLEAVE_NONE, swizzle, CU_TENSOR_MAP_L2_PROMOTION_L2_256B,
                   CU_TENSOR_MAP_FLOAT_OOB_FILL_NONE);
  KGC_REQUIRE(r == CUDA_SUCCESS, "cuTensorMapEncodeTiled failed (" + std::to_string((int)r) + ")");
  return 0;
}

int make_map_f32_groups(CUtensorMap* map, const void* ptr, int64_t rows, int groups, int64_t pitch, int box_groups,
                        CUtensorMapSwizzle swizzle) {
  EncodeTiledFn enc;
  if (encode_fn(&enc)) return 1;
  KGC_REQUIRE((reinterpret_cast<uintptr_t>(ptr) & 15) == 0 && (pitch * 4) % 16 == 0, "operand must be 16-byte aligned with a 16-byte pitch");
  cuuint64_t dims[3] = {32, (cuuint64_t)rows, (cuuint64_t)groups};
  cuuint64_t strides[2] = {(cuuint64_t)pitch * 4, 128};
  cuuint32_t box[3] = {32, 32, (cuuint32_t)box_groups};
  cuuint32_t estr[3] = {1, 1, 1};
  CUresult r = enc(map, CU_TENSOR_MAP_DATA_TYPE_FLOAT32, 3, const_cast<void*>(ptr), dims, strides, box, estr,
                   CU_TENSOR_MAP_INTERLEAVE_NONE, swizzle, CU_TENSOR_MAP_L2_PROMOTION_L2_256B,
                   CU_TENSOR_MAP_FLOAT_OOB_FILL_NONE);
  KGC_REQUIRE(r == CUDA_SUCCESS, "cuTensorMapEncodeTiled (grouped operand) failed (" + std::to_string((int)r) + ")");
  return 0;
}
int make_map_f32_mn_groups(CUtensorMap* map, const void* ptr, int64_t rows, int groups, int64_t pitch) {
  return make_map_f32_groups(map, ptr, rows, groups, pitch, groups, CU_TENSOR_MAP_SWIZZLE_128B_ATOM_32B);
}

int make_map_f32_parts(CUtensorMap* map, const void* ptr, int64_t parts, int64_t rows, int64_t cols) {
  EncodeTiledFn enc;
  if (encode_fn(&enc)) return 1;
  KGC_REQUIRE((reinterpret_cast<uintptr_t>(ptr) & 15) == 0 && cols % 4 == 0, "partials must be 16-byte aligned with a 16-byte pitch");
  cuuint64_t dims[3] = {(cuuint64_t)cols, (cuuint64_t)rows, (cuuint64_t)parts};
  cuuint64_t strides[2] = {(cuuint64_t)cols * 4, (cuuint64_t)rows * cols * 4};
  cuuint32_t box[3] = {32, 32, 1};
  cuuint32_t estr[3] = {1, 1, 1};
  CUresult r = enc(map, CU_TENSOR_MAP_DATA_TYPE_FLOAT32, 3, const_cast<void*>(ptr), dims, strides, box, estr,
                   CU_TENSOR_MAP_INTERLEAVE_NONE, CU_TENSOR_MAP_SWIZZLE_128B, CU_TENSOR_MAP_L2_PROMOTION_L2_256B,
                   CU_TENSOR_MAP_FLOAT_OOB_FILL_NONE);
  KGC_REQUIRE(r == CUDA_SUCCESS, "cuTensorMapEncodeTiled failed (" + std::to_string((int)r) + ")");
  return 0;
}

struct Tiling {
  int n_kb, k_pad, ksteps, NT, n_ntiles, n_pad;
};
int make_tiling(int N, int K, Tiling* t) {
  if (N <= 0 || K <= 0 || K > kMaxKB * kBK || N > 1024) return 1;
  t->n_kb = (K + kBK - 1) / kBK;
  t->k_pad = t->n_kb * kBK;
  t->ksteps = (K + kUK - 1) / kUK;
  int nt_max = kBBudget / (2 * t->n_kb * kBK * 4);
  nt_max = nt_max / 16 * 16;
  if (nt_max > 128) nt_max = 128;
  if (nt_max < 16) return 1;
  t->n_ntiles = (N + nt_max - 1) / nt_max;
  t->NT = ((N + t->n_ntiles - 1) / t->n_ntiles + 15) / 16 * 16;
  t->n_pad = t->NT * t->n_ntiles;
  return 0;
}


constexpr int kTnRows = 32;
constexpr int kTnBox = kTnRows * 128;
constexpr int kTnStages = 3;
constexpr int kTnLoStages = 2;
constexpr int kTnMaxGb = 7;

struct GemmTnMaps {
  CUtensorMap a[kMaxBatch], b[kMaxBatch], a3[kMaxBatch], b3[kMaxBatch], p[kMaxBatch];
};

struct GemmTnParams {
  int64_t M;
  int32_t n_prob, n_slabs;
  int32_t Ka, Nb, ga, gb, n_pad;
  int32_t ga_full, gb_full;
  int32_t kmajor;
  int64_t rows_per_cta;
  float* partial;
  const uint8_t* keep;
  int32_t keep_pitch;
  float keep_scale;
  long long* dbg;
};

__device__ __forceinline__ uint64_t sw128_mn_desc(uint32_t smem_addr) {
  uint64_t d = 0;
  d |= (uint64_t)((smem_addr & 0x3FFFF) >> 4);
  d |= (uint64_t)(kTnBox >> 4) << 16;
  d |= (uint64_t)(512 >> 4) << 32;
  d |= (uint64_t)1 << 46;
  d |= (uint64_t)1 << 61;
  return d;
}

__global__ void __launch_bounds__(kThreadsG, 1)
gemm_tn_tc_kernel(const __grid_constant__ GemmTnMaps maps, const GemmTnParams P) {
  extern __shared__ uint8_t smem_raw[];
  if (P.dbg != nullptr && threadIdx.x == 0) {
    long long g;
    asm volatile("mov.u64 %0, %globaltimer;" : "=l"(g));
    atomicMin(reinterpret_cast<long long*>(P.dbg) + 8 * 64 + 0, g);
    if (blockIdx.x == 0) { P.dbg[8 * 64 + 2] = g; P.dbg[8 * 64 + 3] = clock64(); }
  }
  uint8_t* base = reinterpret_cast<uint8_t*>((reinterpret_cast<uintptr_t>(smem_raw) + 1023) & ~uintptr_t(1023));
  const int warp = threadIdx.x / 32, lane = threadIdx.x % 32;
  const int stage_bytes = (P.ga + P.gb) * kTnBox;
  uint8_t* s_raw = base;
  uint8_t* s_lo = s_raw + kTnStages * stage_bytes;
  uint64_t* bars = reinterpret_cast<uint64_t*>(s_lo + kTnLoStages * stage_bytes);
  uint64_t* raw_full = bars;
  uint64_t* split_full = raw_full + kTnStages;
  uint64_t* empty = split_full + kTnStages;
  uint64_t* lo_empty = empty + kTnStages;
  uint64_t* acc_full = lo_empty + kTnLoStages;
  uint32_t* tmem_slot = reinterpret_cast<uint32_t*>(acc_full + 1);

  if (warp == 0 && lane == 0) {
    for (int i = 0; i < kTnStages; ++i) {
      mb_init(raw_full + i, 1);
      mb_init(split_full + i, kSplitWarps);
      mb_init(empty + i, 1);
    }
    for (int i = 0; i < kTnLoStages; ++i) mb_init(lo_empty + i, 1);
    mb_init(acc_full, 1);
    asm volatile("fence.mbarrier_init.release.cluster;" ::: "memory");
    asm volatile("fence.proxy.async.shared::cta;" ::: "memory");
  }
  if (warp == 14) {
    asm volatile("tcgen05.alloc.cta_group::1.sync.aligned.shared::cta.b32 [%0], %1;" ::"r"(s_u32(tmem_slot)), "r"(kTmemColsG)
                 : "memory");
    asm volatile("tcgen05.relinquish_alloc_permit.cta_group::1.sync.aligned;" ::: "memory");
  }
  asm volatile("tcgen05.fence::before_thread_sync;" ::: "memory");
  __syncthreads();
  asm volatile("tcgen05.fence::after_thread_sync;" ::: "memory");
  const uint32_t tmem_base = *tmem_slot;
  const bool dbg_on = P.dbg != nullptr && blockIdx.x == 0;
  int dbg_n = 0;

  const int prob = blockIdx.x % P.n_prob, slab = blockIdx.x / P.n_prob;
  const CUtensorMap* map_a = &maps.a[prob];
  const CUtensorMap* map_b = &maps.b[prob];
  const CUtensorMap* map_a3 = &maps.a3[prob];
  const CUtensorMap* map_b3 = &maps.b3[prob];
  const CUtensorMap* map_p = &maps.p[prob];
  const int64_t m0 = slab * P.rows_per_cta;
  const int64_t m1 = m0 + P.rows_per_cta < P.M ? m0 + P.rows_per_cta : P.M;
  const int n_kb = m1 > m0 ? (int)((m1 - m0 + kTnRows - 1) / kTnRows) : 0;

  if (warp == 0) {
    if (lane == 0) {
      int stage = 0;
      uint32_t phase = 0;
      for (int kb = 0; kb < n_kb; ++kb) {
        mb_wait(empty + stage, phase ^ 1);
        KGC_DBG(0);
        uint8_t* dst = s_raw + stage * stage_bytes;
        const int row = (int)(m0 + (int64_t)kb * kTnRows);
        if (P.kmajor) {
          mb_expect_tx(raw_full + stage, (uint32_t)(kTileA + P.n_pad * 128));
          tma_2d(dst, map_a, raw_full + stage, row, 0);
          tma_2d(dst + kTileA, map_b, raw_full + stage, row, 0);
          if (++stage == kTnStages) { stage = 0; phase ^= 1; }
          continue;
        }
        mb_expect_tx(raw_full + stage, (uint32_t)stage_bytes);
        if (P.ga_full > 0) tma_3d(dst, map_a3, raw_full + stage, 0, row, 0);
        for (int g = P.ga_full; g < P.ga; ++g) tma_2d(dst + g * kTnBox, map_a, raw_full + stage, g * 32, row);
        if (P.gb_full > 0) tma_3d(dst + P.ga * kTnBox, map_b3, raw_full + stage, 0, row, 0);
        for (int g = P.gb_full; g < P.gb; ++g) tma_2d(dst + (P.ga + g) * kTnBox, map_b, raw_full + stage, g * 32, row);
        if (++stage == kTnStages) { stage = 0; phase ^= 1; }
      }
    }
  } else if (warp >= 2 && warp < 2 + kSplitWarps) {
    const int t = threadIdx.x - 64;
    constexpr int kSplitThreads = kSplitWarps * 32;
    int stage = 0, ls = 0;
    uint32_t phase = 0, lphase = 0;
    const int n_vec = stage_bytes / 16;
    const bool masked = P.keep != nullptr && prob < 2 && !P.kmajor;
    const int brow_t = (t & 255) >> 3;
    const int c16_t = ((((t & 7) >> 1) ^ (brow_t & 3)) << 1) | (t & 1);
    uint32_t nbn[kTnMaxGb];
#pragma unroll
    for (int g = 0; g < kTnMaxGb; ++g) nbn[g] = 0u;
    if (masked && n_kb > 0 && m0 + brow_t < m1) {
      const uint8_t* kp = P.keep + (m0 + brow_t) * P.keep_pitch + c16_t;
#pragma unroll
      for (int g = 0; g < kTnMaxGb; ++g)
        if (g < P.gb) nbn[g] = (uint32_t)__ldg(kp + g * 8);
    }
    for (int kb = 0; kb < n_kb; ++kb) {
      mb_wait(raw_full + stage, phase);
      if (t == 0) KGC_DBG(1);
      mb_wait(lo_empty + ls, lphase ^ 1);
      if (t == 0) KGC_DBG(2);
      uint4* hi = reinterpret_cast<uint4*>(s_raw + stage * stage_bytes);
      uint4* lo = reinterpret_cast<uint4*>(s_lo + ls * stage_bytes);
      const int rows_valid = P.kmajor ? kTnRows : (int)min((int64_t)kTnRows, m1 - (m0 + (int64_t)kb * kTnRows));
      if (masked) {
        uint32_t nbc[kTnMaxGb];
#pragma unroll
        for (int g = 0; g < kTnMaxGb; ++g) nbc[g] = nbn[g];
        if (kb + 1 < n_kb) {
          const uint8_t* kp = P.keep + (m0 + (int64_t)(kb + 1) * kTnRows + brow_t) * P.keep_pitch + c16_t;
          const bool ok = m0 + (int64_t)(kb + 1) * kTnRows + brow_t < m1;
#pragma unroll
          for (int g = 0; g < kTnMaxGb; ++g) nbn[g] = (ok && g < P.gb) ? (uint32_t)__ldg(kp + g * 8) : 0u;
        }
#pragma unroll
        for (int k = 0; k < 4 + kTnMaxGb; ++k) {
          if (k < 4 + P.gb) {
            const int v = t + k * kSplitThreads;
            uint4 x = hi[v];
            if (brow_t >= rows_valid) x = make_uint4(0u, 0u, 0u, 0u);
            else if (k >= 4) {
              uint32_t nb = nbc[k >= 4 ? k - 4 : 0];
              if (prob == 1) nb >>= 4;
              x.x = (nb & 1u) ? __float_as_uint(__uint_as_float(x.x) * P.keep_scale) : 0u;
              x.y = (nb & 2u) ? __float_as_uint(__uint_as_float(x.y) * P.keep_scale) : 0u;
              x.z = (nb & 4u) ? __float_as_uint(__uint_as_float(x.z) * P.keep_scale) : 0u;
              x.w = (nb & 8u) ? __float_as_uint(__uint_as_float(x.w) * P.keep_scale) : 0u;
            }
            uint4 h, l;
            split_tf32(x.x, h.x, l.x);
            split_tf32(x.y, h.y, l.y);
            split_tf32(x.z, h.z, l.z);
            split_tf32(x.w, h.w, l.w);
            hi[v] = h;
            lo[v] = l;
          }
        }
      } else
      for (int v = t; v < n_vec; v += kSplitThreads) {
        uint4 x = hi[v];
        if (((v & 255) >> 3) >= rows_valid) x = make_uint4(0u, 0u, 0u, 0u);
        uint4 h, l;
        split_tf32(x.x, h.x, l.x);
        split_tf32(x.y, h.y, l.y);
        split_tf32(x.z, h.z, l.z);
        split_tf32(x.w, h.w, l.w);
        hi[v] = h;
        lo[v] = l;
      }
      asm volatile("fence.proxy.async.shared::cta;" ::: "memory");
      __syncwarp();
      if (lane == 0) mb_arrive(split_full + stage);
      if (t == 0) KGC_DBG(3);
      if (++stage == kTnStages) { stage = 0; phase ^= 1; }
      if (++ls == kTnLoStages) { ls = 0; lphase ^= 1; }
    }
  } else if (warp == 1) {
    const uint32_t idesc = (1u << 4) | (2u << 7) | (2u << 10) | (1u << 15) | (1u << 16) | ((uint32_t)(P.n_pad >> 3) << 17) |
                           ((uint32_t)(kBM >> 4) << 24);
    int stage = 0, ls = 0;
    uint32_t phase = 0;
    for (int kb = 0; kb < n_kb; ++kb) {
      mb_wait(split_full + stage, phase);
      if (lane == 0) KGC_DBG(4);
      asm volatile("tcgen05.fence::after_thread_sync;" ::: "memory");
      const uint32_t hi_a = s_u32(s_raw + stage * stage_bytes), hi_b = hi_a + P.ga * kTnBox;
      const uint32_t lo_a = s_u32(s_lo + ls * stage_bytes), lo_b = lo_a + P.ga * kTnBox;
      if (P.kmajor) {
        const uint32_t idesc_k = (1u << 4) | (2u << 7) | (2u << 10) | ((uint32_t)(P.n_pad >> 3) << 17) | ((uint32_t)(kBM >> 4) << 24);
        const uint64_t a_hi = sw128_desc(hi_a), a_lo = sw128_desc(lo_a);
        const uint64_t b_hi = sw128_desc(hi_a + kTileA), b_lo = sw128_desc(lo_a + kTileA);
        if (elect_one()) {
          for (int k = 0; k < kTnRows / kUK; ++k) {
            umma_tf32(tmem_base, a_lo + 2 * k, b_hi + 2 * k, idesc_k, (kb | k) != 0 ? 1u : 0u);
            umma_tf32(tmem_base, a_hi + 2 * k, b_lo + 2 * k, idesc_k, 1u);
            umma_tf32(tmem_base, a_hi + 2 * k, b_hi + 2 * k, idesc_k, 1u);
          }
          umma_commit_g(empty + stage);
          umma_commit_g(lo_empty + ls);
          if (kb == n_kb - 1) umma_commit_g(acc_full);
        }
      } else if (elect_one()) {
        for (int k = 0; k < kTnRows / kUK; ++k) {
          const uint32_t off = k * 1024;
          umma_tf32(tmem_base, sw128_mn_desc(lo_a + off), sw128_mn_desc(hi_b + off), idesc, (kb | k) != 0 ? 1u : 0u);
          umma_tf32(tmem_base, sw128_mn_desc(hi_a + off), sw128_mn_desc(lo_b + off), idesc, 1u);
          umma_tf32(tmem_base, sw128_mn_desc(hi_a + off), sw128_mn_desc(hi_b + off), idesc, 1u);
        }
        umma_commit_g(empty + stage);
        umma_commit_g(lo_empty + ls);
        if (kb == n_kb - 1) umma_commit_g(acc_full);
      }
      __syncwarp();
      if (lane == 0) KGC_DBG(5);
      if (++stage == kTnStages) { stage = 0; phase ^= 1; }
      if (++ls == kTnLoStages) ls = 0;
    }
  } else if (warp >= 10 && warp <= 13) {
    const int quarter = warp % 4;
    const int i = quarter * 32 + lane;
    float* out = P.partial + (((int64_t)prob * P.n_slabs + slab) * P.Ka + i) * P.Nb;
    if (n_kb > 0) {
      mb_wait(acc_full, 0);
      if (warp == 10 && lane == 0) KGC_DBG(6);
      asm volatile("tcgen05.fence::after_thread_sync;" ::: "memory");
      const uint32_t taddr = tmem_base + ((uint32_t)(quarter * 32) << 16);
      uint8_t* stg = s_raw + (warp - 10) * (2 * kEpiBuf);
      int buf = 0;
      for (int c0 = 0; c0 < P.n_pad; c0 += 32) {
        uint32_t v[32];
        tmem_ld32_g(taddr + c0, v);
        asm volatile("tcgen05.wait::ld.sync.aligned;" ::: "memory");
        if (lane == 0) asm volatile("cp.async.bulk.wait_group.read 1;" ::: "memory");
        __syncwarp();
        uint8_t* bb = stg + buf * kEpiBuf;
        uint8_t* bx = bb + lane * 128;
        const int sw = lane & 7;
#pragma unroll
        for (int q = 0; q < 8; ++q)
          *reinterpret_cast<uint4*>(bx + ((q ^ sw) << 4)) = make_uint4(v[4 * q], v[4 * q + 1], v[4 * q + 2], v[4 * q + 3]);
        asm volatile("fence.proxy.async.shared::cta;" ::: "memory");
        __syncwarp();
        if (lane == 0) {
          if (c0 < P.Nb && quarter * 32 < P.Ka) tma_store_3d(map_p, bb, c0, quarter * 32, slab);
          asm volatile("cp.async.bulk.commit_group;" ::: "memory");
        }
        buf ^= 1;
      }
      if (lane == 0) asm volatile("cp.async.bulk.wait_group 0;" ::: "memory");
      if (warp == 10 && lane == 0) KGC_DBG(7);
    } else if (i < P.Ka) {
      for (int j = 0; j < P.Nb; ++j) out[j] = 0.f;
    }
  }
  asm volatile("tcgen05.fence::before_thread_sync;" ::: "memory");
  __syncthreads();
  if (P.dbg != nullptr && threadIdx.x == 0) {
    long long g;
    asm volatile("mov.u64 %0, %globaltimer;" : "=l"(g));
    atomicMax(reinterpret_cast<long long*>(P.dbg) + 8 * 64 + 1, g);
    if (blockIdx.x == 0) { P.dbg[8 * 64 + 4] = g; P.dbg[8 * 64 + 5] = clock64(); }
  }
  if (warp == 14) {
    asm volatile("tcgen05.dealloc.cta_group::1.sync.aligned.b32 %0, %1;" ::"r"(tmem_base), "r"(kTmemColsG) : "memory");
  }
}

struct TnOut { float* c[kMaxBatch]; };
__global__ void __launch_bounds__(256)
gemm_tn_partials_reduce(const float* __restrict__ partial_all, int n_parts, int n_elem, const TnOut outs) {
  __shared__ double sm[8][33];
  const float* partial = partial_all + (int64_t)blockIdx.y * n_parts * n_elem;
  float* C = blockIdx.y == 0 ? outs.c[0] : (blockIdx.y == 1 ? outs.c[1] : outs.c[2]);
  const int e = blockIdx.x * 32 + threadIdx.x;
  double s = 0.0;
  if (e < n_elem) {
    int g = threadIdx.y;
    for (; g + 24 < n_parts; g += 32) {
      const float v0 = partial[(int64_t)g * n_elem + e], v1 = partial[(int64_t)(g + 8) * n_elem + e];
      const float v2 = partial[(int64_t)(g + 16) * n_elem + e], v3 = partial[(int64_t)(g + 24) * n_elem + e];
      s += (double)v0; s += (double)v1; s += (double)v2; s += (double)v3;
    }
    for (; g < n_parts; g += 8) s += (double)partial[(int64_t)g * n_elem + e];
  }
  sm[threadIdx.y][threadIdx.x] = s;
  __syncthreads();
  if (threadIdx.y == 0 && e < n_elem) {
    double t = sm[0][threadIdx.x];
#pragma unroll
    for (int k = 1; k < 8; ++k) t += sm[k][threadIdx.x];
    C[e] = (float)t;
  }
}

int make_map_f32_mn(CUtensorMap* map, const void* ptr, int64_t rows, int64_t cols, int64_t pitch) {
  return make_map_f32(map, ptr, rows, cols, pitch, kTnRows, CU_TENSOR_MAP_SWIZZLE_128B_ATOM_32B);
}

}
}

using namespace kgc;

static long long* g_gemm_dbg = nullptr;

extern "C" int kgc_conv_prep(const float* rels, int32_t n_rels, const float* loop_rel, const float* loop_edge, const float* w_in,
                             const float* w_out, const float* w_loop, const float* w_rel, int32_t D, int32_t Dout, float* relp,
                             float* all_rel, float* packed_fwd, float* packed_bwd, void* stream) {
  Tiling tf, tb;
  KGC_REQUIRE(make_tiling(Dout, D, &tf) == 0 && make_tiling(D, Dout, &tb) == 0, "unsupported layer width (<= 256)");
  KGC_REQUIRE(n_rels >= 0 && rels && loop_rel && loop_edge && w_in && w_out && w_loop && w_rel && relp && all_rel && packed_fwd && packed_bwd,
              "null buffer");
  PrepArgs a;
  a.rels = rels; a.loop_rel = loop_rel; a.loop_edge = loop_edge; a.w0 = w_in; a.w1 = w_out; a.w2 = w_loop; a.w_rel = w_rel;
  a.n_rels = n_rels; a.D = D; a.Dout = Dout;
  a.n_pad_f = tf.n_pad; a.k_pad_f = tf.k_pad; a.n_pad_b = tb.n_pad; a.k_pad_b = tb.k_pad;
  a.relp = relp; a.all_rel = all_rel; a.packed_f = packed_fwd; a.packed_b = packed_bwd;
  const int64_t total = (int64_t)(n_rels + 1) * (D + Dout) + 3 * (int64_t)tf.n_pad * tf.k_pad + 4 * (int64_t)tb.n_pad * tb.k_pad;
  conv_prep_kernel<<<(unsigned)ceil_div(total, 256), 256, 0, as_stream(stream)>>>(a);
  KGC_LAUNCH_CHECK();
  return 0;
}

extern "C" int kgc_conv_param_grads(const float* m_loop, const float* w_loop, const float* loop_rel, const float* loop_edge,
                                    const float* relp, const float* w_rel, const float* g_rel, const float* d_relp,
                                    int32_t n_rels, int32_t D, int32_t Dout, float* d_w_loop, float* d_loop_rel,
                                    float* d_loop_edge, float* d_rels, float* d_w_rel, const float* rel_add, void* stream) {
  KGC_REQUIRE(m_loop && w_loop && loop_rel && loop_edge && relp && w_rel && d_relp && d_w_loop && d_loop_rel && d_loop_edge && d_rels && d_w_rel,
              "null buffer");
  ParamGradArgs a;
  a.m_loop = m_loop; a.w_loop = w_loop; a.loop_rel = loop_rel; a.loop_edge = loop_edge; a.relp = relp; a.w_rel = w_rel;
  a.g_rel = g_rel; a.d_relp = d_relp; a.n_rels = n_rels; a.D = D; a.Dout = Dout;
  a.d_w_loop = d_w_loop; a.d_loop_rel = d_loop_rel; a.d_loop_edge = d_loop_edge; a.d_rels = d_rels; a.d_w_rel = d_w_rel;
  if (rel_add != nullptr) {
    KGC_REQUIRE((D * Dout) % 32 == 0, "D * Dout must be a multiple of 32");
    const int64_t total2 = (int64_t)D * Dout + (((int64_t)n_rels * D + 31) & ~31ll) + (int64_t)D * 32;
    conv_param_grads2_kernel<<<(unsigned)ceil_div(total2, 256), 256, 0, as_stream(stream)>>>(a, rel_add);
    KGC_LAUNCH_CHECK();
    return 0;
  }
  const int64_t total = 2 * (int64_t)D * Dout + (int64_t)(n_rels + 1) * D * 32;
  conv_param_grads_kernel<<<(unsigned)ceil_div(total, 256), 256, 0, as_stream(stream)>>>(a);
  KGC_LAUNCH_CHECK();
  return 0;
}

extern "C" size_t kgc_gemm_packed_b_bytes(int32_t N, int32_t K) {
  Tiling t;
  if (make_tiling(N, K, &t)) return 0;
  return (size_t)2 * t.n_pad * t.k_pad * sizeof(float);
}

extern "C" int kgc_gemm_pack_b(const float* B, int64_t stride_k, int64_t stride_n, int32_t N, int32_t K, float* packed,
                               void* stream) {
  Tiling t;
  KGC_REQUIRE(make_tiling(N, K, &t) == 0, "unsupported GEMM shape (K <= 256, N <= 1024)");
  const int total = t.n_pad * t.k_pad;
  pack_b_kernel<<<(total + 255) / 256, 256, 0, as_stream(stream)>>>(B, stride_k, stride_n, N, K, t.n_pad, t.k_pad, packed,
                                                                    packed + total);
  KGC_LAUNCH_CHECK();
  return 0;
}

extern "C" void kgc_gemm_set_debug(long long* buf) { g_gemm_dbg = buf; }

static int launch_gemm_nt(int n_prob, const float* const* A, int64_t M, int32_t K, int64_t lda, const float* const* packed_b,
                          int32_t N, float* const* C, int64_t ldc, const float* row_bias, int32_t act, int32_t trans_c,
                          int32_t trans_a, void* stream, const uint8_t* keep = nullptr, int32_t keep_pitch = 0,
                          float keep_scale = 1.f) {
  Tiling t;
  KGC_REQUIRE(n_prob >= 1 && n_prob <= kMaxBatch, "1..3 problems per launch");
  KGC_REQUIRE(make_tiling(N, K, &t) == 0, "unsupported GEMM shape (K <= 256, N <= 1024)");
  KGC_REQUIRE(M > 0 && lda >= (trans_a ? M : (int64_t)K) && ldc >= (trans_c ? M : (int64_t)N), "bad leading dimensions");
  KGC_REQUIRE(!trans_a || M % 32 == 0, "a transposed A operand needs M % 32 == 0");
  KGC_REQUIRE(ldc % 4 == 0, "C needs a 16-byte row pitch (TMA store)");
  GemmMaps maps;
  const int total = t.n_pad * t.k_pad;
  for (int i = 0; i < kMaxBatch; ++i) {
    const int j = i < n_prob ? i : 0;
    KGC_REQUIRE((reinterpret_cast<uintptr_t>(C[j]) & 15) == 0, "C must be 16-byte aligned (TMA store)");
    if (trans_c) {
      if (make_map_f32(&maps.c[i], C[j], N, M, ldc, 32, CU_TENSOR_MAP_SWIZZLE_128B, 32)) return 1;
      if (make_map_f32(&maps.c16[i], C[j], N, M, ldc, 16, CU_TENSOR_MAP_SWIZZLE_128B, 32)) return 1;
    } else {
      if (make_map_f32(&maps.c[i], C[j], M, N, ldc, 32, CU_TENSOR_MAP_SWIZZLE_128B, 32)) return 1;
      if (make_map_f32(&maps.c16[i], C[j], M, N, ldc, 32, CU_TENSOR_MAP_SWIZZLE_64B, 16)) return 1;
    }
    if (trans_a) {
      if (make_map_f32_groups(&maps.a[i], A[j], K, (int)(M / 32), lda, kBM / 32, CU_TENSOR_MAP_SWIZZLE_128B)) return 1;
    } else if (make_map_f32(&maps.a[i], A[j], M, K, lda, kBM)) {
      return 1;
    }
    if (make_map_f32(&maps.bhi[i], packed_b[j], t.n_pad, t.k_pad, t.k_pad, t.NT)) return 1;
    if (make_map_f32(&maps.blo[i], packed_b[j] + total, t.n_pad, t.k_pad, t.k_pad, t.NT)) return 1;
  }
  GemmParams P;
  P.M = M; P.N = N; P.K = K; P.n_prob = n_prob;
  P.n_kb = t.n_kb; P.ksteps = t.ksteps; P.NT = t.NT; P.n_ntiles = t.n_ntiles;
  P.n_mtiles = (int32_t)ceil_div(M, kBM);
  P.C = C[0]; P.ldc = ldc; P.row_bias = row_bias; P.act = act; P.trans_c = trans_c; P.trans_a = trans_a; P.dbg = g_gemm_dbg;
  KGC_REQUIRE(keep == nullptr || (!trans_a && keep_pitch % 16 == 0 && keep_pitch >= 8 * kMaxKB && (reinterpret_cast<uintptr_t>(keep) & 15) == 0),
              "keep flags: one byte per 4 columns, 16-byte aligned rows of at least 64 bytes");
  P.keep = keep; P.keep_pitch = keep_pitch; P.keep_scale = keep_scale;
  const int tile_b_al = (t.NT * kBK * 4 + 1023) & ~1023;
  const size_t fixed = (size_t)2 * t.n_kb * tile_b_al + kEpiStage + 512 + 1024;
  int stages = (int)((226 * 1024 - fixed) / kTileA);
  if (stages > kMaxStages) stages = kMaxStages;
  KGC_REQUIRE(stages >= 2, "shared-memory plan does not fit");
  P.stages = stages;
  const size_t smem = fixed + (size_t)stages * kTileA;
  static SmemAttrCache attr;
  KGC_CUDA_TRY(attr.ensure(gemm_tf32x3_kernel, smem));
  const int groups = n_prob * t.n_ntiles;
  int per = kNumSMs / groups;
  if (per > P.n_mtiles) per = P.n_mtiles;
  if (per < 1) per = 1;
  gemm_tf32x3_kernel<<<per * groups, kThreadsG, smem, as_stream(stream)>>>(maps, P);
  KGC_LAUNCH_CHECK();
  return 0;
}

extern "C" int kgc_gemm_nt(const float* A, int64_t M, int32_t K, int64_t lda, const float* packed_b, int32_t N, float* C,
                           int64_t ldc, void* stream) {
  return launch_gemm_nt(1, &A, M, K, lda, &packed_b, N, &C, ldc, nullptr, 0, 0, 0, stream);
}

extern "C" int kgc_gemm_nt_batch(int32_t n_prob, const float* const* A, int64_t M, int32_t K, int64_t lda,
                                 const float* const* packed_b, int32_t N, float* const* C, int64_t ldc, void* stream) {
  KGC_REQUIRE(A && packed_b && C, "null pointer table");
  return launch_gemm_nt(n_prob, A, M, K, lda, packed_b, N, C, ldc, nullptr, 0, 0, 0, stream);
}

extern "C" int kgc_gemm_nt_batch_masked(int32_t n_prob, const float* const* A, int64_t M, int32_t K, int64_t lda,
                                        const float* const* packed_b, int32_t N, float* const* C, int64_t ldc,
                                        const uint8_t* keep, int32_t keep_pitch, float keep_scale, void* stream) {
  KGC_REQUIRE(A && packed_b && C, "null pointer table");
  return launch_gemm_nt(n_prob, A, M, K, lda, packed_b, N, C, ldc, nullptr, 0, 0, 0, stream, keep, keep_pitch, keep_scale);
}

extern "C" int kgc_gemm_nt_trans(const float* At, int64_t M, int32_t K, int64_t ldat, const float* packed_b, int32_t N,
                                 float* Ct, int64_t ldct, void* stream) {
  return launch_gemm_nt(1, &At, M, K, ldat, &packed_b, N, &Ct, ldct, nullptr, 0, 1, 1, stream);
}

extern "C" int kgc_score_1n_fwd(const float* ent, int64_t n_ent, int32_t D, int64_t ld_ent, const float* packed_x, int32_t B,
                                const float* bias, float* pred, int64_t ld_pred, void* stream) {
  KGC_REQUIRE(bias != nullptr, "bias is required");
  return launch_gemm_nt(1, &ent, n_ent, D, ld_ent, &packed_x, B, &pred, ld_pred, bias, 1, 1, 0, stream);
}

constexpr int64_t kTnMaxSlabRows = 1024;

static int64_t tn_max_slab_rows() {
  static int64_t rows = 0;
  if (rows == 0) {
    const char* e = getenv("KGC_TN_SLAB_ROWS");
    rows = e != nullptr && atoll(e) >= 64 ? atoll(e) : kTnMaxSlabRows;
  }
  return rows;
}

static int64_t tn_slabs(int64_t M, int n_prob) {
  const int64_t per_wave = kNumSMs / n_prob > 0 ? kNumSMs / n_prob : 1;
  int64_t slabs = ceil_div(M, (int64_t)2 * kTnRows);
  if (slabs > per_wave) slabs = per_wave;
  const int64_t need = ceil_div(M, tn_max_slab_rows());
  if (slabs < need) slabs = ceil_div(need, per_wave) * per_wave;
  return slabs < 1 ? 1 : slabs;
}

extern "C" int kgc_score_1n_fwd_t(const float* ent, int64_t n_ent, int32_t D, int64_t ld_ent, const float* packed_x, int32_t B,
                                  const float* bias, float* pred_t, int64_t ld_t, void* stream) {
  KGC_REQUIRE(bias != nullptr, "bias is required");
  return launch_gemm_nt(1, &ent, n_ent, D, ld_ent, &packed_x, B, &pred_t, ld_t, bias, 1, 0, 0, stream);
}

extern "C" int kgc_score_1n_logits(const float* ent, int64_t n_ent, int32_t D, int64_t ld_ent, const float* packed_x, int32_t B,
                                   const float* bias, float* logits, int64_t ld_logits, void* stream) {
  KGC_REQUIRE(bias != nullptr, "bias is required");
  return launch_gemm_nt(1, &ent, n_ent, D, ld_ent, &packed_x, B, &logits, ld_logits, bias, 0, 1, 0, stream);
}

extern "C" size_t kgc_gemm_tn_tc_workspace_bytes(int64_t M, int32_t Ka, int32_t Nb) {
  int64_t parts = kNumSMs;
  for (int n = 1; n <= kMaxBatch; ++n) {
    const int64_t s = tn_slabs(M > 0 ? M : 1, n) * n;
    if (s > parts) parts = s;
  }
  return (size_t)parts * Ka * Nb * sizeof(float);
}

static int launch_gemm_tn_tc(int n_prob, const float* const* A, int64_t lda, const float* const* B, int64_t ldb, int64_t M,
                             int32_t Ka, int32_t Nb, float* const* C, void* workspace, size_t workspace_bytes, int32_t kmajor,
                             void* stream, const uint8_t* keep = nullptr, int32_t keep_pitch = 0, float keep_scale = 1.f) {
  KGC_REQUIRE(n_prob >= 1 && n_prob <= kMaxBatch, "1..3 problems per launch");
  KGC_REQUIRE(M > 0 && Ka > 0 && Nb > 0 && Ka <= 128 && Nb <= 224, "supported: Ka <= 128, Nb <= 224");
  KGC_REQUIRE(Nb % 4 == 0 && lda % 4 == 0 && ldb % 4 == 0 && (kmajor || Ka % 4 == 0), "dimensions and leading dimensions must be multiples of 4");
  KGC_REQUIRE(workspace && workspace_bytes >= kgc_gemm_tn_tc_workspace_bytes(M, Ka, Nb), "workspace too small");
  GemmTnParams P;
  P.n_pad = (Nb + 15) / 16 * 16;
  P.kmajor = kmajor;
  P.M = M; P.Ka = Ka; P.Nb = Nb; P.n_prob = n_prob;
  P.ga = 4;
  P.gb = (P.n_pad + 31) / 32;
  int slabs = (int)tn_slabs(M, n_prob);
  P.rows_per_cta = ceil_div(ceil_div(M, slabs), kTnRows) * kTnRows;
  slabs = (int)ceil_div(M, P.rows_per_cta);
  P.n_slabs = slabs;
  P.partial = static_cast<float*>(workspace);
  P.dbg = g_gemm_dbg;
  KGC_REQUIRE(keep == nullptr || (!kmajor && keep_pitch >= 8 * P.gb), "keep flags: one byte per 4 columns of B, rows that cover the padded width");
  P.keep = keep; P.keep_pitch = keep_pitch; P.keep_scale = keep_scale;
  P.ga_full = kmajor ? 0 : Ka / 32;
  P.gb_full = kmajor ? 0 : Nb / 32;
  GemmTnMaps maps;
  TnOut outs;
  for (int i = 0; i < kMaxBatch; ++i) {
    const int j = i < n_prob ? i : 0;
    outs.c[i] = C[j];
    if (kmajor) {
      if (make_map_f32(&maps.a[i], A[j], Ka, M, lda, kBM) || make_map_f32(&maps.b[i], B[j], Nb, M, ldb, P.n_pad)) return 1;
    } else if (make_map_f32_mn(&maps.a[i], A[j], M, Ka, lda) || make_map_f32_mn(&maps.b[i], B[j], M, Nb, ldb)) {
      return 1;
    }
    maps.a3[i] = maps.a[i]; maps.b3[i] = maps.b[i];
    if (P.ga_full > 0 && make_map_f32_mn_groups(&maps.a3[i], A[j], M, P.ga_full, lda)) return 1;
    if (P.gb_full > 0 && make_map_f32_mn_groups(&maps.b3[i], B[j], M, P.gb_full, ldb)) return 1;
    if (make_map_f32_parts(&maps.p[i], P.partial + (int64_t)j * slabs * Ka * Nb, slabs, Ka, Nb)) return 1;
  }
  const size_t stage = (size_t)(P.ga + P.gb) * kTnBox;
  const size_t smem = (kTnStages + kTnLoStages) * stage + 512 + 1024;
  KGC_REQUIRE(smem <= 227 * 1024, "shared-memory plan does not fit");
  static SmemAttrCache attr;
  KGC_CUDA_TRY(attr.ensure(gemm_tn_tc_kernel, smem));
  cudaStream_t st = as_stream(stream);
  gemm_tn_tc_kernel<<<slabs * n_prob, kThreadsG, smem, st>>>(maps, P);
  KGC_LAUNCH_CHECK();
  gemm_tn_partials_reduce<<<dim3((Ka * Nb + 31) / 32, n_prob), dim3(32, 8), 0, st>>>(P.partial, slabs, Ka * Nb, outs);
  KGC_LAUNCH_CHECK();
  return 0;
}

extern "C" int kgc_gemm_tn_tc(const float* A, int64_t lda, const float* B, int64_t ldb, int64_t M, int32_t Ka, int32_t Nb,
                              float* C, void* workspace, size_t workspace_bytes, void* stream) {
  return launch_gemm_tn_tc(1, &A, lda, &B, ldb, M, Ka, Nb, &C, workspace, workspace_bytes, 0, stream);
}

extern "C" int kgc_gemm_tn_tc_batch(int32_t n_prob, const float* const* A, int64_t lda, const float* const* B, int64_t ldb,
                                    int64_t M, int32_t Ka, int32_t Nb, float* const* C, void* workspace,
                                    size_t workspace_bytes, void* stream) {
  KGC_REQUIRE(A && B && C, "null pointer table");
  return launch_gemm_tn_tc(n_prob, A, lda, B, ldb, M, Ka, Nb, C, workspace, workspace_bytes, 0, stream);
}

extern "C" int kgc_gemm_tn_tc_batch_masked(int32_t n_prob, const float* const* A, int64_t lda, const float* const* B, int64_t ldb,
                                           int64_t M, int32_t Ka, int32_t Nb, float* const* C, void* workspace,
                                           size_t workspace_bytes, const uint8_t* keep, int32_t keep_pitch, float keep_scale,
                                           void* stream) {
  KGC_REQUIRE(A && B && C, "null pointer table");
  return launch_gemm_tn_tc(n_prob, A, lda, B, ldb, M, Ka, Nb, C, workspace, workspace_bytes, 0, stream, keep, keep_pitch,
                           keep_scale);
}

extern "C" int kgc_gemm_nt_splitk(const float* A, int64_t lda, const float* Bt, int64_t ldb, int64_t K, int32_t Ma, int32_t Nb,
                                  float* C, void* workspace, size_t workspace_bytes, void* stream) {
  return launch_gemm_tn_tc(1, &A, lda, &Bt, ldb, K, Ma, Nb, &C, workspace, workspace_bytes, 1, stream);
}
```

### kgc-gcn_b200/csrc/tail.cu

```cuda
#include "common.cuh"

namespace kgc {
namespace {

constexpr int kThreads = 256;
constexpr int kMaxBlocks = 4 * kNumSMs;

struct Stripe {
  int64_t row_beg, row_end;
};
__device__ __forceinline__ Stripe block_stripe(int64_t n_rows) {
  const int64_t per = (n_rows + gridDim.x - 1) / gridDim.x;
  Stripe s;
  s.row_beg = blockIdx.x * per;
  s.row_end = s.row_beg + per < n_rows ? s.row_beg + per : n_rows;
  return s;
}

__device__ __forceinline__ float4 mask4(const uint8_t* m, int64_t idx4, float s) {
  const uchar4 v = *reinterpret_cast<const uchar4*>(m + idx4 * 4);
  return make_float4(v.x ? s : 0.f, v.y ? s : 0.f, v.z ? s : 0.f, v.w ? s : 0.f);
}

constexpr int kKeepPitch = 64;
__device__ __forceinline__ uint32_t nibble(const float4& m) {
  return (m.x != 0.f ? 1u : 0u) | (m.y != 0.f ? 2u : 0u) | (m.z != 0.f ? 4u : 0u) | (m.w != 0.f ? 8u : 0u);
}

__device__ __forceinline__ float4 keep4(const float4& g, uint32_t nb, float s) {
  return make_float4((nb & 1u) ? g.x * s : 0.f, (nb & 2u) ? g.y * s : 0.f, (nb & 4u) ? g.z * s : 0.f, (nb & 8u) ? g.w * s : 0.f);
}

struct DropCfg {
  const uint8_t* mask_in;
  const uint8_t* mask_out;
  const int64_t* seed;
  uint32_t drop_thr;
  float keep_scale;
};
__device__ __forceinline__ float4 drop_scale4(const DropCfg& d, int plane, int64_t i) {
  const uint8_t* m = plane == 0 ? d.mask_in : d.mask_out;
  if (m != nullptr) return mask4(m, i, d.keep_scale);
  if (d.seed != nullptr) return philox_mask4(i, (uint32_t)plane, (uint64_t)__ldg(d.seed), d.drop_thr, d.keep_scale);
  return make_float4(1.f, 1.f, 1.f, 1.f);
}

__device__ __forceinline__ void block_store_partials(double4 a, double4 b, int rl, int c, int RL, int Do4,
                                                     double* partials, double4* sm) {
  const bool active = rl < RL;
  if (active) {
    sm[(0 * RL + rl) * Do4 + c] = a;
    sm[(1 * RL + rl) * Do4 + c] = b;
  }
  __syncthreads();
  if (active && rl == 0) {
    double4 sa = sm[c], sb = sm[RL * Do4 + c];
    for (int k = 1; k < RL; ++k) {
      const double4 ta = sm[(0 * RL + k) * Do4 + c], tb = sm[(1 * RL + k) * Do4 + c];
      sa.x += ta.x; sa.y += ta.y; sa.z += ta.z; sa.w += ta.w;
      sb.x += tb.x; sb.y += tb.y; sb.z += tb.z; sb.w += tb.w;
    }
    double4* out = reinterpret_cast<double4*>(partials) + (int64_t)blockIdx.x * 2 * Do4;
    out[c] = sa;
    out[Do4 + c] = sb;
  }
}

__global__ void __launch_bounds__(kThreads)
tail_fwd_kernel(const float4* __restrict__ res3, const DropCfg drop, const float4* __restrict__ bias,
                int64_t n_rows, int Do4, float4* __restrict__ pre, double* __restrict__ partials,
                uint8_t* __restrict__ keep) {
  extern __shared__ double4 sm[];
  const int RL = kThreads / Do4;
  const int rl = threadIdx.x / Do4, c = threadIdx.x % Do4;
  const Stripe s = block_stripe(n_rows);
  const int64_t plane = n_rows * (int64_t)Do4;
  double4 sum = make_double4(0, 0, 0, 0), sq = make_double4(0, 0, 0, 0);
  if (rl < RL) {
    const float4 bv = bias ? __ldg(bias + c) : make_float4(0.f, 0.f, 0.f, 0.f);
    for (int64_t r = s.row_beg + rl; r < s.row_end; r += RL) {
      const int64_t i = r * Do4 + c;
      float4 a = __ldg(res3 + i), b = __ldg(res3 + plane + i);
      const float4 l = __ldg(res3 + 2 * plane + i);
      uint32_t kb = 0;
      { const float4 m = drop_scale4(drop, 0, i); a.x *= m.x; a.y *= m.y; a.z *= m.z; a.w *= m.w; kb |= nibble(m); }
      { const float4 m = drop_scale4(drop, 1, i); b.x *= m.x; b.y *= m.y; b.z *= m.z; b.w *= m.w; kb |= nibble(m) << 4; }
      if (keep != nullptr) keep[r * kKeepPitch + c] = (uint8_t)kb;
      float4 o;
      o.x = (a.x + b.x + l.x) / 3.0f + bv.x;
      o.y = (a.y + b.y + l.y) / 3.0f + bv.y;
      o.z = (a.z + b.z + l.z) / 3.0f + bv.z;
      o.w = (a.w + b.w + l.w) / 3.0f + bv.w;
      pre[i] = o;
      sum.x += o.x; sum.y += o.y; sum.z += o.z; sum.w += o.w;
      sq.x += (double)o.x * o.x; sq.y += (double)o.y * o.y; sq.z += (double)o.z * o.z; sq.w += (double)o.w * o.w;
    }
  }
  block_store_partials(sum, sq, rl, c, RL, Do4, partials, sm);
}

constexpr int kFinCols = 2, kFinLanes = 128;

__device__ __forceinline__ void reduce_partials(const double* __restrict__ partials, int64_t n_blocks, int Dout,
                                                int c, int lane, double (*sm)[kFinLanes][kFinCols], double* s_out,
                                                double* q_out) {
  double s = 0, q = 0;
  if (c < Dout) {
    for (int64_t b = lane; b < n_blocks; b += kFinLanes) {
      s += partials[(b * 2 + 0) * Dout + c];
      q += partials[(b * 2 + 1) * Dout + c];
    }
  }
  const int cc = threadIdx.x % kFinCols;
  sm[0][lane][cc] = s;
  sm[1][lane][cc] = q;
  __syncthreads();
  if (lane == 0) {
    s = sm[0][0][cc];
    q = sm[1][0][cc];
    for (int k = 1; k < kFinLanes; ++k) {
      s += sm[0][k][cc];
      q += sm[1][k][cc];
    }
  }
  *s_out = s;
  *q_out = q;
}

__global__ void __launch_bounds__(kFinCols * kFinLanes)
colsum_finalize_kernel(const double* __restrict__ partials, int64_t n_blocks, int Dout, double* __restrict__ sums) {
  __shared__ double sm[2][kFinLanes][kFinCols];
  const int c = blockIdx.x * kFinCols + threadIdx.x % kFinCols, lane = threadIdx.x / kFinCols;
  double s = 0, q = 0;
  reduce_partials(partials, n_blocks, Dout, c, lane, sm, &s, &q);
  if (lane != 0 || c >= Dout) return;
  sums[c] = s;
  sums[Dout + c] = q;
}

__global__ void __launch_bounds__(kFinCols * kFinLanes)
colsum_finalize2_kernel(const double* __restrict__ partials, int64_t n_blocks, int Dout, double* __restrict__ sums,
                        float* __restrict__ sums32) {
  __shared__ double sm[2][kFinLanes][kFinCols];
  const int c = blockIdx.x * kFinCols + threadIdx.x % kFinCols, lane = threadIdx.x / kFinCols;
  double s = 0, q = 0;
  reduce_partials(partials, n_blocks, Dout, c, lane, sm, &s, &q);
  if (lane != 0 || c >= Dout) return;
  sums[c] = s;
  sums[Dout + c] = q;
  sums32[c] = (float)s;
  sums32[Dout + c] = (float)q;
}

__global__ void __launch_bounds__(kFinCols * kFinLanes)
colstats_finalize_kernel(const double* __restrict__ partials, int64_t n_blocks, int64_t n_rows, int Dout, float eps,
                         float momentum, float* __restrict__ rmean, float* __restrict__ rvar,
                         int64_t* __restrict__ n_tracked, double* __restrict__ sums, float* __restrict__ stats) {
  __shared__ double sm[2][kFinLanes][kFinCols];
  const int c = blockIdx.x * kFinCols + threadIdx.x % kFinCols, lane = threadIdx.x / kFinCols;
  double s = 0, q = 0;
  reduce_partials(partials, n_blocks, Dout, c, lane, sm, &s, &q);
  if (blockIdx.x == 0 && threadIdx.x == 0 && n_tracked != nullptr) *n_tracked += 1;
  if (lane != 0 || c >= Dout) return;
  if (sums != nullptr) {
    sums[c] = s;
    sums[Dout + c] = q;
  }
  const double mean = s / (double)n_rows;
  double var = q / (double)n_rows - mean * mean;
  if (var < 0) var = 0;
  const float meanf = (float)mean, varf = (float)var;
  stats[c] = meanf;
  stats[Dout + c] = varf;
  stats[2 * Dout + c] = (float)(1.0 / sqrt(var + (double)eps));
  if (rmean != nullptr && rvar != nullptr) {
    const float unbias = (float)n_rows / (float)(n_rows > 1 ? n_rows - 1 : 1);
    rmean[c] = rmean[c] * (1.f - momentum) + momentum * meanf;
    rvar[c] = rvar[c] * (1.f - momentum) + (momentum * unbias) * varf;
  }
}

__global__ void colstats_from_sums_kernel(const double* __restrict__ sums, int64_t n_rows, int Dout, float eps,
                                          int training, const float* __restrict__ rmean,
                                          const float* __restrict__ rvar, float* __restrict__ stats) {
  const int c = blockIdx.x * blockDim.x + threadIdx.x;
  if (c >= Dout) return;
  double mean, var;
  if (training) {
    mean = sums[c] / (double)n_rows;
    var = sums[Dout + c] / (double)n_rows - mean * mean;
    if (var < 0) var = 0;
  } else {
    mean = rmean[c];
    var = rvar[c];
  }
  stats[c] = (float)mean;
  stats[Dout + c] = (float)var;
  stats[2 * Dout + c] = (float)(1.0 / sqrt(var + (double)eps));
}

struct OutDrop {
  const int64_t* seed;
  uint32_t drop_thr;
  float keep_scale;
  uint8_t* keep;
};

__global__ void __launch_bounds__(kThreads)
tail_apply_kernel(const float4* __restrict__ pre, const float4* __restrict__ stats, const float4* __restrict__ gamma,
                  const float4* __restrict__ beta, int64_t n4, int Do4, float4* __restrict__ all_ent, const OutDrop od) {
  const int64_t i = blockIdx.x * (int64_t)kThreads + threadIdx.x;
  if (i >= n4) return;
  const int c = (int)(i % Do4);
  const float4 v = __ldg(pre + i), m = __ldg(stats + c), rs = __ldg(stats + 2 * Do4 + c);
  const float4 ga = __ldg(gamma + c), be = __ldg(beta + c);
  float4 o;
  o.x = tanhf((v.x - m.x) * rs.x * ga.x + be.x);
  o.y = tanhf((v.y - m.y) * rs.y * ga.y + be.y);
  o.z = tanhf((v.z - m.z) * rs.z * ga.z + be.z);
  o.w = tanhf((v.w - m.w) * rs.w * ga.w + be.w);
  if (od.seed != nullptr) {
    const float4 k = philox_mask4(i, 2u, (uint64_t)__ldg(od.seed), od.drop_thr, od.keep_scale);
    o.x *= k.x; o.y *= k.y; o.z *= k.z; o.w *= k.w;
    od.keep[(i / Do4) * kKeepPitch + c] = (uint8_t)nibble(k);
  }
  all_ent[i] = o;
}

__global__ void __launch_bounds__(kThreads)
tail_bwd_reduce_kernel(const float4* __restrict__ g_ent, const float4* __restrict__ pre, const float4* __restrict__ stats,
                       const float4* __restrict__ gamma, const float4* __restrict__ beta, int64_t n_rows, int Do4,
                       double* __restrict__ partials, const uint8_t* __restrict__ out_keep, float out_scale) {
  extern __shared__ double4 sm[];
  const int RL = kThreads / Do4;
  const int rl = threadIdx.x / Do4, c = threadIdx.x % Do4;
  const Stripe s = block_stripe(n_rows);
  double4 s1 = make_double4(0, 0, 0, 0), s2 = make_double4(0, 0, 0, 0);
  if (rl < RL) {
    const float4 m = __ldg(stats + c), rs = __ldg(stats + 2 * Do4 + c), ga = __ldg(gamma + c), be = __ldg(beta + c);
    for (int64_t r = s.row_beg + rl; r < s.row_end; r += RL) {
      const int64_t i = r * Do4 + c;
      float4 g = __ldg(g_ent + i);
      const float4 v = __ldg(pre + i);
      if (out_keep != nullptr) g = keep4(g, out_keep[r * kKeepPitch + c], out_scale);
      const float4 xh = make_float4((v.x - m.x) * rs.x, (v.y - m.y) * rs.y, (v.z - m.z) * rs.z, (v.w - m.w) * rs.w);
      const float4 t = make_float4(tanhf(xh.x * ga.x + be.x), tanhf(xh.y * ga.y + be.y), tanhf(xh.z * ga.z + be.z),
                                   tanhf(xh.w * ga.w + be.w));
      const float dzx = g.x * (1.f - t.x * t.x), dzy = g.y * (1.f - t.y * t.y);
      const float dzz = g.z * (1.f - t.z * t.z), dzw = g.w * (1.f - t.w * t.w);
      s1.x += dzx; s1.y += dzy; s1.z += dzz; s1.w += dzw;
      s2.x += (double)dzx * xh.x;
      s2.y += (double)dzy * xh.y;
      s2.z += (double)dzz * xh.z;
      s2.w += (double)dzw * xh.w;
    }
  }
  block_store_partials(s1, s2, rl, c, RL, Do4, partials, sm);
}

__global__ void __launch_bounds__(kThreads)
tail_bwd_apply_kernel(const float4* __restrict__ g_ent, const float4* __restrict__ pre, const float4* __restrict__ stats,
                      const float4* __restrict__ gamma, const float4* __restrict__ beta, const double* __restrict__ sums,
                      int training, int64_t n_rows, int64_t n_rows_global, int Do4, float4* __restrict__ d_out,
                      const uint8_t* __restrict__ keep, float keep_scale, float4* __restrict__ d_res2,
                      const uint8_t* __restrict__ out_keep, float out_scale) {
  const int64_t n4 = n_rows * (int64_t)Do4;
  const int64_t i = blockIdx.x * (int64_t)kThreads + threadIdx.x;
  if (i >= n4) return;
  const int c = (int)(i % Do4);
  float4 g = __ldg(g_ent + i);
  const float4 v = __ldg(pre + i);
  if (out_keep != nullptr) g = keep4(g, out_keep[(i / Do4) * kKeepPitch + c], out_scale);
  const float4 m = __ldg(stats + c), rs = __ldg(stats + 2 * Do4 + c), ga = __ldg(gamma + c), be = __ldg(beta + c);
  const float4 xh = make_float4((v.x - m.x) * rs.x, (v.y - m.y) * rs.y, (v.z - m.z) * rs.z, (v.w - m.w) * rs.w);
  const float4 t = make_float4(tanhf(xh.x * ga.x + be.x), tanhf(xh.y * ga.y + be.y), tanhf(xh.z * ga.z + be.z),
                               tanhf(xh.w * ga.w + be.w));
  float4 dz = make_float4(g.x * (1.f - t.x * t.x), g.y * (1.f - t.y * t.y), g.z * (1.f - t.z * t.z),
                          g.w * (1.f - t.w * t.w));
  float4 dp;
  if (training) {
    const float inv_n = 1.0f / (float)n_rows_global;
    const double* sp = sums + 4 * c;
    const double* sq = sums + 4 * (Do4 + c);
    const float4 s1 = make_float4((float)sp[0], (float)sp[1], (float)sp[2], (float)sp[3]);
    const float4 s2 = make_float4((float)sq[0], (float)sq[1], (float)sq[2], (float)sq[3]);
    dp.x = ga.x * rs.x * (dz.x - s1.x * inv_n - xh.x * s2.x * inv_n);
    dp.y = ga.y * rs.y * (dz.y - s1.y * inv_n - xh.y * s2.y * inv_n);
    dp.z = ga.z * rs.z * (dz.z - s1.z * inv_n - xh.z * s2.z * inv_n);
    dp.w = ga.w * rs.w * (dz.w - s1.w * inv_n - xh.w * s2.w * inv_n);
  } else {
    dp = make_float4(ga.x * rs.x * dz.x, ga.y * rs.y * dz.y, ga.z * rs.z * dz.z, ga.w * rs.w * dz.w);
  }
  const float4 third = make_float4(dp.x / 3.0f, dp.y / 3.0f, dp.z / 3.0f, dp.w / 3.0f);
  d_out[i] = third;
  if (d_res2 != nullptr) {
    const uint32_t kb = keep != nullptr ? keep[(i / Do4) * kKeepPitch + c] : 0xFFu;
    const float s = keep != nullptr ? keep_scale : 1.f;
    d_res2[i] = make_float4((kb & 1u) ? third.x * s : 0.f, (kb & 2u) ? third.y * s : 0.f, (kb & 4u) ? third.z * s : 0.f,
                            (kb & 8u) ? third.w * s : 0.f);
    d_res2[n4 + i] = make_float4((kb & 16u) ? third.x * s : 0.f, (kb & 32u) ? third.y * s : 0.f, (kb & 64u) ? third.z * s : 0.f,
                                 (kb & 128u) ? third.w * s : 0.f);
  }
}

inline int check_dout(int32_t Dout) { return (Dout <= 0 || Dout % 4 != 0 || Dout > 1024) ? 1 : 0; }
inline size_t partial_smem(int Do4) { return size_t(2) * (kThreads / Do4) * Do4 * sizeof(double4); }

}
}

using namespace kgc;

extern "C" int64_t kgc_tail_num_blocks(int64_t n_rows) {
  int64_t nb = ceil_div(n_rows > 0 ? n_rows : 1, 32);
  return nb < kMaxBlocks ? nb : kMaxBlocks;
}

static DropCfg make_drop(const uint8_t* mask_in, const uint8_t* mask_out, const int64_t* seed, float drop_p, float keep_scale) {
  DropCfg d;
  d.mask_in = mask_in;
  d.mask_out = mask_out;
  d.seed = (seed != nullptr && drop_p > 0.f) ? seed : nullptr;
  const double thr = (double)drop_p * 4294967296.0;
  d.drop_thr = thr >= 4294967295.0 ? 0xFFFFFFFFu : (uint32_t)thr;
  d.keep_scale = keep_scale;
  return d;
}

__global__ void dropout_mask_kernel(const int64_t* __restrict__ seed, uint32_t plane, uint32_t drop_thr, int64_t n4,
                                    uchar4* __restrict__ out) {
  const int64_t i = blockIdx.x * (int64_t)blockDim.x + threadIdx.x;
  if (i >= n4) return;
  const float4 m = philox_mask4(i, plane, (uint64_t)__ldg(seed), drop_thr, 1.0f);
  out[i] = make_uchar4(m.x != 0.f, m.y != 0.f, m.z != 0.f, m.w != 0.f);
}

extern "C" int kgc_dropout_mask(const int64_t* seed, int32_t plane, float drop_p, int64_t n_elem, uint8_t* mask, void* stream) {
  KGC_REQUIRE(seed != nullptr && n_elem % 4 == 0 && plane >= 0, "bad arguments");
  const DropCfg d = make_drop(nullptr, nullptr, seed, drop_p, 1.0f);
  const int64_t n4 = n_elem / 4;
  if (n4 == 0) return 0;
  dropout_mask_kernel<<<(unsigned)ceil_div(n4, kThreads), kThreads, 0, as_stream(stream)>>>(seed, (uint32_t)plane, d.drop_thr,
                                                                                     n4, (uchar4*)mask);
  KGC_LAUNCH_CHECK();
  return 0;
}

extern "C" int32_t kgc_keep_pitch() { return kKeepPitch; }

extern "C" int kgc_tail_fwd(const float* res3, const uint8_t* mask_in, const uint8_t* mask_out, const int64_t* seed,
                            float drop_p, float keep_scale, const float* bias, int64_t n_rows, int32_t Dout, float* pre,
                            double* partials, uint8_t* keep, void* stream) {
  KGC_REQUIRE(check_dout(Dout) == 0, "Dout must be a multiple of 4 and <= 1024");
  KGC_REQUIRE(keep == nullptr || Dout <= 4 * kKeepPitch, "packed keep flags need Dout <= 256");
  KGC_REQUIRE(n_rows > 0, "n_rows must be positive");
  const int Do4 = Dout / 4;
  const size_t smem = partial_smem(Do4);
  tail_fwd_kernel<<<(unsigned)kgc_tail_num_blocks(n_rows), kThreads, smem, as_stream(stream)>>>(
      (const float4*)res3, make_drop(mask_in, mask_out, seed, drop_p, keep_scale), (const float4*)bias, n_rows, Do4,
      (float4*)pre, partials, keep);
  KGC_LAUNCH_CHECK();
  return 0;
}

extern "C" int kgc_colsum_finalize(const double* partials, int64_t n_blocks, int32_t Dout, double* sums, void* stream) {
  KGC_REQUIRE(check_dout(Dout) == 0, "Dout must be a multiple of 4 and <= 1024");
  colsum_finalize_kernel<<<(unsigned)ceil_div(Dout, kFinCols), kFinCols * kFinLanes, 0, as_stream(stream)>>>(
      partials, n_blocks, Dout, sums);
  KGC_LAUNCH_CHECK();
  return 0;
}

extern "C" int kgc_colsum_finalize2(const double* partials, int64_t n_blocks, int32_t Dout, double* sums, float* sums32,
                                    void* stream) {
  KGC_REQUIRE(check_dout(Dout) == 0, "Dout must be a multiple of 4 and <= 1024");
  KGC_REQUIRE(partials && sums && sums32 && n_blocks > 0, "null buffer");
  colsum_finalize2_kernel<<<(unsigned)ceil_div(Dout, kFinCols), kFinCols * kFinLanes, 0, as_stream(stream)>>>(
      partials, n_blocks, Dout, sums, sums32);
  KGC_LAUNCH_CHECK();
  return 0;
}

extern "C" int kgc_colstats_finalize(const double* partials, int64_t n_blocks, int64_t n_rows, int32_t Dout, float eps,
                                     float momentum, float* running_mean, float* running_var,
                                     int64_t* num_batches_tracked, double* sums, float* stats, void* stream) {
  KGC_REQUIRE(check_dout(Dout) == 0, "Dout must be a multiple of 4 and <= 1024");
  KGC_REQUIRE(partials && stats && n_blocks > 0 && n_rows > 0, "null buffer");
  KGC_REQUIRE((running_mean == nullptr) == (running_var == nullptr), "running_mean and running_var come together");
  colstats_finalize_kernel<<<(unsigned)ceil_div(Dout, kFinCols), kFinCols * kFinLanes, 0, as_stream(stream)>>>(
      partials, n_blocks, n_rows, Dout, eps, momentum, running_mean, running_var, num_batches_tracked, sums, stats);
  KGC_LAUNCH_CHECK();
  return 0;
}

extern "C" int kgc_colstats_from_sums(const double* sums, int64_t n_rows, int32_t Dout, float eps, int32_t training,
                                      const float* running_mean, const float* running_var, float* stats, void* stream) {
  KGC_REQUIRE(check_dout(Dout) == 0, "Dout must be a multiple of 4 and <= 1024");
  KGC_REQUIRE(training || (running_mean && running_var), "eval mode needs running statistics");
  KGC_REQUIRE(!training || sums, "training mode needs the column sums");
  colstats_from_sums_kernel<<<(unsigned)ceil_div(Dout, 128), 128, 0, as_stream(stream)>>>(
      sums, n_rows, Dout, eps, training, running_mean, running_var, stats);
  KGC_LAUNCH_CHECK();
  return 0;
}

extern "C" int kgc_tail_apply(const float* pre, const float* stats, const float* gamma, const float* beta,
                              int64_t n_rows, int32_t Dout, float* all_ent, const int64_t* out_seed, float out_drop_p,
                              uint8_t* out_keep, void* stream) {
  KGC_REQUIRE(check_dout(Dout) == 0, "Dout must be a multiple of 4 and <= 1024");
  const int Do4 = Dout / 4;
  const int64_t n4 = n_rows * Do4;
  OutDrop od;
  od.seed = (out_seed != nullptr && out_drop_p > 0.f) ? out_seed : nullptr;
  KGC_REQUIRE(od.seed == nullptr || (out_keep != nullptr && Dout <= 4 * kKeepPitch && out_drop_p < 1.f),
              "output dropout needs a keep-flag buffer, Dout <= 256 and p < 1");
  const DropCfg d = make_drop(nullptr, nullptr, out_seed, out_drop_p, 1.f);
  od.drop_thr = d.drop_thr;
  od.keep_scale = 1.f / (1.f - out_drop_p);
  od.keep = out_keep;
  tail_apply_kernel<<<(unsigned)ceil_div(n4, kThreads), kThreads, 0, as_stream(stream)>>>(
      (const float4*)pre, (const float4*)stats, (const float4*)gamma, (const float4*)beta, n4, Do4, (float4*)all_ent, od);
  KGC_LAUNCH_CHECK();
  return 0;
}

extern "C" int kgc_tail_bwd_reduce(const float* g_ent, const float* pre, const float* stats, const float* gamma,
                                   const float* beta, int64_t n_rows, int32_t Dout, double* partials, const uint8_t* out_keep,
                                   float out_scale, void* stream) {
  KGC_REQUIRE(check_dout(Dout) == 0, "Dout must be a multiple of 4 and <= 1024");
  const int Do4 = Dout / 4;
  const size_t smem = partial_smem(Do4);
  tail_bwd_reduce_kernel<<<(unsigned)kgc_tail_num_blocks(n_rows), kThreads, smem, as_stream(stream)>>>(
      (const float4*)g_ent, (const float4*)pre, (const float4*)stats, (const float4*)gamma, (const float4*)beta, n_rows, Do4,
      partials, out_keep, out_scale);
  KGC_LAUNCH_CHECK();
  return 0;
}

extern "C" int kgc_tail_bwd_apply(const float* g_ent, const float* pre, const float* stats, const float* gamma,
                                  const float* beta, const double* sums, int32_t training, int64_t n_rows,
                                  int64_t n_rows_global, int32_t Dout, float* d_out, const uint8_t* keep, float keep_scale,
                                  float* d_res2, const uint8_t* out_keep, float out_scale, void* stream) {
  KGC_REQUIRE(check_dout(Dout) == 0, "Dout must be a multiple of 4 and <= 1024");
  const int Do4 = Dout / 4;
  const int64_t n4 = n_rows * Do4;
  tail_bwd_apply_kernel<<<(unsigned)ceil_div(n4, kThreads), kThreads, 0, as_stream(stream)>>>(
      (const float4*)g_ent, (const float4*)pre, (const float4*)stats, (const float4*)gamma, (const float4*)beta, sums,
      training, n_rows, n_rows_global, Do4, (float4*)d_out, keep, keep_scale, (float4*)d_res2, out_keep, out_scale);
  KGC_LAUNCH_CHECK();
  return 0;
}
```

Baseline: 870.5 million.

## Use split-fp16 tcgen05 GEMM with amax scaling for backward input-gradient

Adds a new tcgen05 kind::f16 GEMM that splits the fp32 A operand into hi/lo fp16 halves inside the kernel, using a power-of-two scale derived from an amax that the tail backward kernel now reduces. The B weights are packed to fp16 hi/lo with their own scale on a side stream, overlapping with the tail kernel. This path replaces the 3xTF32 gradient GEMM when the layer is large, aiming to cut tensor-core and conversion cost. In exchange the tail kernel gains an amax reduction plus a memset, and accuracy now depends on fp16 range and the chosen scale.

```diff
diff --git a/include/kgc_b200.h b/include/kgc_b200.h
--- a/include/kgc_b200.h
+++ b/include/kgc_b200.h
@@ -79,7 +79,7 @@
 int kgc_tail_bwd_apply(const float* g_ent, const float* pre, const float* stats, const float* gamma, const float* beta,
                        const double* sums, int32_t training, int64_t n_rows, int64_t n_rows_global, int32_t Dout,
                        float* d_out, const uint8_t* keep, float keep_scale, float* d_res2, const uint8_t* out_keep,
-                       float out_scale, void* stream);
+                       float out_scale, uint32_t* amax, void* stream);
 
 int kgc_conv_prep(const float* rels, int32_t n_rels, const float* loop_rel, const float* loop_edge, const float* w_in,
                   const float* w_out, const float* w_loop, const float* w_rel, int32_t D, int32_t Dout, float* relp,
@@ -120,6 +120,13 @@
 int kgc_gemm_tn_tc_batch_masked(int32_t n_prob, const float* const* A, int64_t lda, const float* const* B, int64_t ldb,
                                 int64_t M, int32_t Ka, int32_t Nb, float* const* C, void* workspace, size_t workspace_bytes,
                                 const uint8_t* keep, int32_t keep_pitch, float keep_scale, void* stream);
+
+size_t kgc_gemm_f16_packed_b_bytes(int32_t N, int32_t K);
+int kgc_gemm_pack_b_f16(int32_t n_prob, const float* const* B, int64_t stride_k, int64_t stride_n, const float* const* mul0,
+                        const float* const* mul1, int32_t N, int32_t K, void* packed, float* inv_scale, void* stream);
+int kgc_gemm_nt_f16_batch(int32_t n_prob, const float* const* A, int64_t M, int32_t K, int64_t lda, const void* packed_b,
+                          const float* b_inv_scale, const uint32_t* a_amax, float a_amax_mul, int32_t N, float* const* C,
+                          int64_t ldc, const uint8_t* keep, int32_t keep_pitch, float keep_scale, void* stream);
 
 int kgc_label_build(const int64_t* qid, int64_t B, const int64_t* triples, const int64_t* ptr,
                     const int32_t* idx, int64_t n_entity, float pos, float add,
diff --git a/kgc-gcn_b200/_lib.py b/kgc-gcn_b200/_lib.py
--- a/kgc-gcn_b200/_lib.py
+++ b/kgc-gcn_b200/_lib.py
@@ -33,7 +33,7 @@
     'kgc_colsum_finalize2': (ctypes.c_int, [_vp, _i64, _i32, _vp, _vp, _vp]),
     'kgc_tail_apply': (ctypes.c_int, [_vp, _vp, _vp, _vp, _i64, _i32, _vp, _vp, _f32, _vp, _vp]),
     'kgc_tail_bwd_reduce': (ctypes.c_int, [_vp, _vp, _vp, _vp, _vp, _i64, _i32, _vp, _vp, _f32, _vp]),
-    'kgc_tail_bwd_apply': (ctypes.c_int, [_vp, _vp, _vp, _vp, _vp, _vp, _i32, _i64, _i64, _i32, _vp, _vp, _f32, _vp, _vp, _f32, _vp]),
+    'kgc_tail_bwd_apply': (ctypes.c_int, [_vp, _vp, _vp, _vp, _vp, _vp, _i32, _i64, _i64, _i32, _vp, _vp, _f32, _vp, _vp, _f32, _vp, _vp]),
     'kgc_gemm_packed_b_bytes': (_sz, [_i32, _i32]),
     'kgc_gemm_pack_b': (ctypes.c_int, [_vp, _i64, _i64, _i32, _i32, _vp, _vp]),
     'kgc_gemm_nt': (ctypes.c_int, [_vp, _i64, _i32, _i64, _vp, _i32, _vp, _i64, _vp]),
@@ -42,6 +42,9 @@
     'kgc_gemm_nt_batch': (ctypes.c_int, [_i32, _vp, _i64, _i32, _i64, _vp, _i32, _vp, _i64, _vp]),
     'kgc_gemm_nt_batch_masked': (ctypes.c_int, [_i32, _vp, _i64, _i32, _i64, _vp, _i32, _vp, _i64, _vp, _i32, _f32, _vp]),
     'kgc_gemm_tn_tc_batch_masked': (ctypes.c_int, [_i32, _vp, _i64, _vp, _i64, _i64, _i32, _i32, _vp, _vp, _sz, _vp, _i32, _f32, _vp]),
+    'kgc_gemm_f16_packed_b_bytes': (_sz, [_i32, _i32]),
+    'kgc_gemm_pack_b_f16': (ctypes.c_int, [_i32, _vp, _i64, _i64, _vp, _vp, _i32, _i32, _vp, _vp, _vp]),
+    'kgc_gemm_nt_f16_batch': (ctypes.c_int, [_i32, _vp, _i64, _i32, _i64, _vp, _vp, _vp, _f32, _i32, _vp, _i64, _vp, _i32, _f32, _vp]),
     'kgc_gemm_nt_trans': (ctypes.c_int, [_vp, _i64, _i32, _i64, _vp, _i32, _vp, _i64, _vp]),
     'kgc_gemm_nt_splitk': (ctypes.c_int, [_vp, _i64, _vp, _i64, _i64, _i32, _i32, _vp, _vp, _sz, _vp]),
     'kgc_gemm_set_debug': (None, [_vp]),
diff --git a/kgc-gcn_b200/conv.py b/kgc-gcn_b200/conv.py
--- a/kgc-gcn_b200/conv.py
+++ b/kgc-gcn_b200/conv.py
@@ -53,6 +53,44 @@
                   _lib.ptr(keep), keep.stride(0), float(keep_scale), _lib.stream())
     else:
         _lib.call('kgc_gemm_nt_batch', n, arr(a_list), M, K, lda, arr(packed_list), N, arr(out_list), ldc, _lib.stream())
+    return out_list
+
+
+AMAX_WORDS = 64 * 32
+
+
+def _ptrs(ts):
+    import ctypes
+    return (ctypes.c_void_p * len(ts))(*[None if t is None else t.data_ptr() for t in ts])
+
+
+def f16_pack_buffers(n, N, K, device):
+    nbytes = int(_lib.lib().kgc_gemm_f16_packed_b_bytes(N, K))
+    if nbytes == 0:
+        raise ValueError('fp16 split: unsupported shape K={} N={}'.format(K, N))
+    return (torch.empty((n * nbytes,), dtype=torch.uint8, device=device),
+            torch.empty((n,), dtype=torch.float32, device=device))
+
+
+def pack_b_f16(b_list, stride_k, stride_n, N, K, mul0=None, mul1=None, out=None):
+    packed, inv = out if out is not None else f16_pack_buffers(len(b_list), N, K, b_list[0].device)
+    n = len(b_list)
+    _lib.call('kgc_gemm_pack_b_f16', n, _ptrs(b_list), stride_k, stride_n, None if mul0 is None else _ptrs(mul0),
+              None if mul1 is None else _ptrs(mul1), N, K, _lib.ptr(packed), _lib.ptr(inv), _lib.stream())
+    return packed, inv
+
+
+def gemm_nt_f16_batch(a_list, packed, inv_scale, amax, amax_mul, out_list, keep=None, keep_scale=1.0):
+    n = len(a_list)
+    M, K = a_list[0].shape
+    N = out_list[0].shape[1]
+    lda, ldc = a_list[0].stride(0), out_list[0].stride(0)
+    for a, o in zip(a_list, out_list):
+        if a.shape != (M, K) or o.shape != (M, N) or a.stride() != (lda, 1) or o.stride() != (ldc, 1):
+            raise ValueError('gemm_nt_f16_batch needs operands of identical shape and strides')
+    p = _lib.ptr
+    _lib.call('kgc_gemm_nt_f16_batch', n, _ptrs(a_list), M, K, lda, p(packed), p(inv_scale), p(amax), float(amax_mul), N,
+              _ptrs(out_list), ldc, p(keep), 0 if keep is None else keep.stride(0), float(keep_scale), _lib.stream())
     return out_list
 
 
@@ -384,6 +422,16 @@
         if g_ent is None:
             g_ent = torch.zeros_like(all_ent)
         g_ent = g_ent.contiguous()
+        main, side = torch.cuda.current_stream(), plan.side_stream()
+        packed_b16 = inv_b16 = packed_ev = None
+        if 3 * Nl * Dout * 4 > (48 << 20) and int(_lib.lib().kgc_gemm_f16_packed_b_bytes(D, Dout)) > 0:
+            packed_b16, inv_b16 = f16_pack_buffers(3, D, Dout, dev)
+            side.wait_stream(main)
+            with torch.cuda.stream(side):
+                pack_b_f16([w.detach().contiguous() for w in (w_in, w_out, w_loop)], 1, Dout, D, Dout,
+                           [None, None, loop_rel.detach()], [None, None, loop_edge.detach()], out=(packed_b16, inv_b16))
+                packed_ev = torch.cuda.Event()
+                packed_ev.record(side)
 
         nb = int(_lib.lib().kgc_tail_num_blocks(Nl))
         partials = plan.scratch('colpart', (nb, 2, Dout), torch.float64)
@@ -401,8 +449,9 @@
         mode = os.environ.get('KGC_TAIL_PLANES', '')
         three = (3 * Nl * Dout * 4 > (48 << 20)) if mode not in ('1', '3') else mode == '3'
         d_res2 = plan.scratch('d_res2', (2, Nl, Dout)) if three else None
+        amax = plan.scratch('d_out_amax', (AMAX_WORDS,), torch.int32) if packed_b16 is not None else None
         _lib.call('kgc_tail_bwd_apply', p(g_ent), p(pre), p(stats), p(gamma), p(beta), p(sums), int(ctx.training), Nl,
-                  n_global, Dout, p(d_out), p(keep), ctx.keep_scale, p(d_res2), p(out_keep), ctx.out_scale, st())
+                  n_global, Dout, p(d_out), p(keep), ctx.keep_scale, p(d_res2), p(out_keep), ctx.out_scale, p(amax), st())
         ups = [d_res2[0], d_res2[1], d_out] if three else [d_out, d_out, d_out]
         gkeep = None if three else keep
         d_beta, d_gamma = sums32[0], sums32[1]
@@ -410,7 +459,6 @@
         flat = torch.empty((3 * D * Dout + T * D + (Dout if ctx.has_bias else 0),), dtype=torch.float32, device=dev)
         d_w_in, d_w_out, m_loop = (flat[k * D * Dout:(k + 1) * D * Dout].view(D, Dout) for k in range(3))
         d_relp = flat[3 * D * Dout:3 * D * Dout + T * D].view(T, D)
-        main, side = torch.cuda.current_stream(), plan.side_stream()
         side.wait_stream(main)
         with torch.cuda.stream(side):
             gemm_tn_batch([agg[0, :Nl], agg[1, :Nl], x], ups, [d_w_in, d_w_out, m_loop], plan,
@@ -420,8 +468,13 @@
 
         hybrid = coll is not None and coll.p2p is not None and coll.p2p.hybrid
         g3 = coll.p2p.g3_planes() if hybrid else plan.scratch('g3', (3, Nb, D))
-        gemm_nt_batch(ups, [packed_b[0], packed_b[1], packed_b[2]],
-                      [g3[0, :Nl], g3[1, :Nl], g3[2, :Nl]], keep=gkeep, keep_scale=ctx.keep_scale)
+        if packed_b16 is not None:
+            main.wait_event(packed_ev)
+            gemm_nt_f16_batch(ups, packed_b16, inv_b16, amax, ctx.keep_scale, [g3[0, :Nl], g3[1, :Nl], g3[2, :Nl]],
+                              keep=gkeep, keep_scale=ctx.keep_scale)
+        else:
+            gemm_nt_batch(ups, [packed_b[0], packed_b[1], packed_b[2]],
+                          [g3[0, :Nl], g3[1, :Nl], g3[2, :Nl]], keep=gkeep, keep_scale=ctx.keep_scale)
         if n_hub:
             coll.spread_hub_rows(g3, 2, n_loc)
         if hybrid:
diff --git a/kgc-gcn_b200/csrc/common.cuh b/kgc-gcn_b200/csrc/common.cuh
--- a/kgc-gcn_b200/csrc/common.cuh
+++ b/kgc-gcn_b200/csrc/common.cuh
@@ -31,6 +31,9 @@
 inline cudaStream_t as_stream(void* s) { return reinterpret_cast<cudaStream_t>(s); }
 
 constexpr int kNumSMs = 148;
+
+constexpr int kAmaxSlots = 64;
+constexpr int kAmaxStride = 32;
 
 struct SmemAttrCache {
   size_t set[64] = {0};
diff --git a/kgc-gcn_b200/csrc/gemm_tf32x3.cu b/kgc-gcn_b200/csrc/gemm_tf32x3.cu
--- a/kgc-gcn_b200/csrc/gemm_tf32x3.cu
+++ b/kgc-gcn_b200/csrc/gemm_tf32x3.cu
@@ -1,4 +1,5 @@
 #include <cuda.h>
+#include <cuda_fp16.h>
 
 #include <cstdlib>
 #include "common.cuh"
@@ -1003,6 +1004,369 @@
 
 int make_map_f32_mn(CUtensorMap* map, const void* ptr, int64_t rows, int64_t cols, int64_t pitch) {
   return make_map_f32(map, ptr, rows, cols, pitch, kTnRows, CU_TENSOR_MAP_SWIZZLE_128B_ATOM_32B);
+}
+
+
+constexpr int kF16BK = 64;
+constexpr int kF16UK = 16;
+constexpr int kF16AStages = 8;
+constexpr int kF16ScaleExp = 14;
+static_assert(kAccCols + kF16AStages * 32 == 512, "TMEM budget");
+
+struct GemmF16Params {
+  int64_t M;
+  int32_t n_prob, N, K;
+  int32_t n_kb, nb_b, ksteps, NT, n_mtiles, stages;
+  const uint32_t* a_amax;
+  float a_amax_mul;
+  const float* b_inv_scale;
+  const uint8_t* keep;
+  int32_t keep_pitch;
+  float keep_scale;
+};
+
+__device__ __forceinline__ int f16_scale_exp(float amax) {
+  const uint32_t b = __float_as_uint(amax) & 0x7FFFFFFFu;
+  if (b == 0u || b >= 0x7F800000u) return 0;
+  return max(-100, min(100, kF16ScaleExp - ((int)(b >> 23) - 127)));
+}
+__device__ __forceinline__ float exp2_int(int e) { return __uint_as_float((uint32_t)(127 + e) << 23); }
+__device__ __forceinline__ float amax_read(const uint32_t* slots) {
+  uint32_t m = 0u;
+  for (int i = 0; i < kAmaxSlots; ++i) m = max(m, slots[i * kAmaxStride]);
+  return __uint_as_float(m);
+}
+__device__ __forceinline__ void split_f16x2(float a, float b, uint32_t& hi, uint32_t& lo) {
+  const __half2 h = __floats2half2_rn(a, b);
+  const float2 hf = __half22float2(h);
+  const __half2 l = __floats2half2_rn(a - hf.x, b - hf.y);
+  hi = *reinterpret_cast<const uint32_t*>(&h);
+  lo = *reinterpret_cast<const uint32_t*>(&l);
+}
+__device__ __forceinline__ void umma_f16_ts(uint32_t tmem_d, uint32_t a_tmem, uint64_t bdesc, uint32_t idesc, uint32_t acc) {
+  asm volatile(
+      "{\n"
+      ".reg .pred p;\n"
+      "setp.ne.b32 p, %4, 0;\n"
+      "tcgen05.mma.cta_group::1.kind::f16 [%0], [%1], %2, %3, p;\n"
+      "}" ::"r"(tmem_d),
+      "r"(a_tmem), "l"(bdesc), "r"(idesc), "r"(acc)
+      : "memory");
+}
+__device__ __forceinline__ void tmem_st8_g(uint32_t taddr, const uint32_t (&v)[8]) {
+  asm volatile("tcgen05.st.sync.aligned.32x32b.x8.b32 [%0], {%1, %2, %3, %4, %5, %6, %7, %8};" ::"r"(taddr), "r"(v[0]),
+               "r"(v[1]), "r"(v[2]), "r"(v[3]), "r"(v[4]), "r"(v[5]), "r"(v[6]), "r"(v[7])
+               : "memory");
+}
+
+__global__ void __launch_bounds__(kThreadsG, 1)
+gemm_f16x2_kernel(const __grid_constant__ GemmMaps maps, const GemmF16Params P) {
+  extern __shared__ uint8_t smem_raw[];
+  uint8_t* base = reinterpret_cast<uint8_t*>((reinterpret_cast<uintptr_t>(smem_raw) + 1023) & ~uintptr_t(1023));
+  const int warp = threadIdx.x / 32, lane = threadIdx.x % 32;
+  const int tile_b = P.NT * kF16BK * 2;
+  const int tile_b_al = (tile_b + 1023) & ~1023;
+  uint8_t* s_bhi = base;
+  uint8_t* s_blo = s_bhi + P.nb_b * tile_b_al;
+  const int kStages = P.stages;
+  uint8_t* s_a = s_blo + P.nb_b * tile_b_al;
+  uint8_t* s_stage = s_a + kStages * kTileA;
+  uint64_t* bars = reinterpret_cast<uint64_t*>(s_stage + kEpiStage);
+  uint64_t* b_full = bars;
+  uint64_t* raw_full = bars + 1;
+  uint64_t* raw_empty = raw_full + kMaxStages;
+  uint64_t* split_full = raw_empty + kMaxStages;
+  uint64_t* split_empty = split_full + kF16AStages;
+  uint64_t* acc_full = split_empty + kF16AStages;
+  uint64_t* acc_empty = acc_full + 2;
+  uint32_t* tmem_slot = reinterpret_cast<uint32_t*>(acc_empty + 2);
+
+  if (warp == 0 && lane == 0) {
+    mb_init(b_full, 1);
+    for (int i = 0; i < kStages; ++i) {
+      mb_init(raw_full + i, 1);
+      mb_init(raw_empty + i, kSplitWarps);
+    }
+    for (int i = 0; i < kF16AStages; ++i) {
+      mb_init(split_full + i, kSplitWarps);
+      mb_init(split_empty + i, 1);
+    }
+    for (int i = 0; i < 2; ++i) {
+      mb_init(acc_full + i, 1);
+      mb_init(acc_empty + i, 4);
+    }
+    asm volatile("fence.mbarrier_init.release.cluster;" ::: "memory");
+    asm volatile("fence.proxy.async.shared::cta;" ::: "memory");
+  }
+  if (warp == 14) {
+    asm volatile("tcgen05.alloc.cta_group::1.sync.aligned.shared::cta.b32 [%0], %1;" ::"r"(s_u32(tmem_slot)), "r"(512)
+                 : "memory");
+    asm volatile("tcgen05.relinquish_alloc_permit.cta_group::1.sync.aligned;" ::: "memory");
+  }
+  asm volatile("tcgen05.fence::before_thread_sync;" ::: "memory");
+  __syncthreads();
+  asm volatile("tcgen05.fence::after_thread_sync;" ::: "memory");
+  const uint32_t tmem_base = *tmem_slot;
+  const uint32_t tmem_a = tmem_base + kAccCols;
+
+  const int prob = blockIdx.x % P.n_prob;
+  const int first = blockIdx.x / P.n_prob;
+  const int step = gridDim.x / P.n_prob;
+  const int a_exp = f16_scale_exp(amax_read(P.a_amax) * P.a_amax_mul);
+
+  if (warp == 0) {
+    if (lane == 0) {
+      mb_expect_tx(b_full, 2u * P.nb_b * tile_b);
+      for (int kb = 0; kb < P.nb_b; ++kb) {
+        tma_2d(s_bhi + kb * tile_b_al, &maps.bhi[prob], b_full, kb * kF16BK, 0);
+        tma_2d(s_blo + kb * tile_b_al, &maps.blo[prob], b_full, kb * kF16BK, 0);
+      }
+      int stage = 0;
+      uint32_t phase = 0;
+      for (int mt = first; mt < P.n_mtiles; mt += step) {
+        for (int kb = 0; kb < P.n_kb; ++kb) {
+          mb_wait(raw_empty + stage, phase ^ 1);
+          mb_expect_tx(raw_full + stage, kTileA);
+          tma_2d(s_a + stage * kTileA, &maps.a[prob], raw_full + stage, kb * kBK, mt * kBM);
+          if (++stage == kStages) { stage = 0; phase ^= 1; }
+        }
+      }
+    }
+  } else if (warp >= 2 && warp < 2 + kSplitWarps) {
+    const int quarter = warp % 4, half = (warp - 2) / 4;
+    const int r = quarter * 32 + lane;
+    int stage = 0, ts = 0;
+    uint32_t phase = 0, tphase = 0;
+    const float sc_a = exp2_int(a_exp);
+    const float sc_kept = sc_a * P.keep_scale;
+    const bool masked = P.keep != nullptr && prob < 2;
+    uint32_t kcur[kMaxKB], knxt[kMaxKB];
+#pragma unroll
+    for (int j = 0; j < kMaxKB; ++j) kcur[j] = knxt[j] = 0u;
+    auto load_keep = [&](int mt_, uint32_t (&w)[kMaxKB]) {
+      const int64_t grow = (int64_t)mt_ * kBM + r;
+      if (mt_ < P.n_mtiles && grow < P.M) {
+        const uint4* kp = reinterpret_cast<const uint4*>(P.keep + grow * P.keep_pitch);
+#pragma unroll
+        for (int q = 0; q < kMaxKB / 2; ++q) {
+          const uint4 t4 = __ldg(kp + q);
+          w[2 * q] = half ? t4.y : t4.x;
+          w[2 * q + 1] = half ? t4.w : t4.z;
+        }
+      }
+    };
+    if (masked) load_keep(first, knxt);
+    for (int mt = first; mt < P.n_mtiles; mt += step) {
+      if (masked) {
+#pragma unroll
+        for (int j = 0; j < kMaxKB; ++j) kcur[j] = knxt[j];
+        load_keep(mt + step, knxt);
+      }
+      for (int kb = 0; kb < P.n_kb; ++kb) {
+        uint32_t kw = 0;
+        if (masked) {
+#pragma unroll
+          for (int j = 0; j < kMaxKB; ++j)
+            if (kb == j) kw = kcur[j];
+          if (prob == 1) kw >>= 4;
+        }
+        mb_wait(raw_full + stage, phase);
+        const uint8_t* row = s_a + stage * kTileA + r * 128;
+        float f[16];
+#pragma unroll
+        for (int i = 0; i < 4; ++i) {
+          const float4 v = *reinterpret_cast<const float4*>(row + (((half * 4 + i) ^ (r & 7)) << 4));
+          f[4 * i + 0] = v.x; f[4 * i + 1] = v.y; f[4 * i + 2] = v.z; f[4 * i + 3] = v.w;
+        }
+        if (masked) {
+#pragma unroll
+          for (int j = 0; j < 16; ++j) {
+            const uint32_t nb = kw >> (8 * (j / 4));
+            f[j] = ((nb >> (j % 4)) & 1u) ? f[j] * sc_kept : 0.f;
+          }
+        } else {
+#pragma unroll
+          for (int j = 0; j < 16; ++j) f[j] *= sc_a;
+        }
+        uint32_t h[8], l[8];
+#pragma unroll
+        for (int j = 0; j < 8; ++j) split_f16x2(f[2 * j], f[2 * j + 1], h[j], l[j]);
+        __syncwarp();
+        if (lane == 0) mb_arrive(raw_empty + stage);
+        mb_wait(split_empty + ts, tphase ^ 1);
+        asm volatile("tcgen05.fence::after_thread_sync;" ::: "memory");
+        const uint32_t taddr = tmem_a + ((uint32_t)(quarter * 32) << 16) + ts * 32 + half * 8;
+        tmem_st8_g(taddr, h);
+        tmem_st8_g(taddr + 16, l);
+        asm volatile("tcgen05.wait::st.sync.aligned;" ::: "memory");
+        asm volatile("tcgen05.fence::before_thread_sync;" ::: "memory");
+        __syncwarp();
+        if (lane == 0) mb_arrive(split_full + ts);
+        if (++stage == kStages) { stage = 0; phase ^= 1; }
+        if (++ts == kF16AStages) { ts = 0; tphase ^= 1; }
+      }
+    }
+  } else if (warp == 1) {
+    const uint32_t idesc = (1u << 4) | ((uint32_t)(P.NT >> 3) << 17) | ((uint32_t)(kBM >> 4) << 24);
+    int ts = 0, acc = 0;
+    uint32_t tphase = 0, acc_phase = 0;
+    mb_wait(b_full, 0);
+    asm volatile("tcgen05.fence::after_thread_sync;" ::: "memory");
+    for (int mt = first; mt < P.n_mtiles; mt += step) {
+      mb_wait(acc_empty + acc, acc_phase ^ 1);
+      asm volatile("tcgen05.fence::after_thread_sync;" ::: "memory");
+      const uint32_t d_addr = tmem_base + acc * (kAccCols / 2);
+      for (int kb = 0; kb < P.n_kb; ++kb) {
+        mb_wait(split_full + ts, tphase);
+        asm volatile("tcgen05.fence::after_thread_sync;" ::: "memory");
+        const int nk = min(kBK / kF16UK, P.ksteps - kb * (kBK / kF16UK));
+        const uint32_t a_hi = tmem_a + ts * 32, a_lo = a_hi + 16;
+        const uint64_t b_hi = sw128_desc(s_u32(s_bhi + (kb >> 1) * tile_b_al)) + 4 * (kb & 1);
+        const uint64_t b_lo = sw128_desc(s_u32(s_blo + (kb >> 1) * tile_b_al)) + 4 * (kb & 1);
+        if (elect_one()) {
+#pragma unroll
+          for (int k = 0; k < kBK / kF16UK; ++k) {
+            if (k < nk) {
+              umma_f16_ts(d_addr, a_lo + 8 * k, b_hi + 2 * k, idesc, (k != 0 || kb != 0) ? 1u : 0u);
+              umma_f16_ts(d_addr, a_hi + 8 * k, b_lo + 2 * k, idesc, 1u);
+              umma_f16_ts(d_addr, a_hi + 8 * k, b_hi + 2 * k, idesc, 1u);
+            }
+          }
+          umma_commit_g(split_empty + ts);
+          if (kb == P.n_kb - 1) umma_commit_g(acc_full + acc);
+        }
+        __syncwarp();
+        if (++ts == kF16AStages) { ts = 0; tphase ^= 1; }
+      }
+      if (++acc == 2) { acc = 0; acc_phase ^= 1; }
+    }
+  } else if (warp >= 10 && warp <= 13) {
+    const int quarter = warp % 4;
+    uint8_t* stg = s_stage + (warp - 10) * (2 * kEpiBuf);
+    const int64_t row_q = quarter * 32;
+    const float inv_a = exp2_int(-a_exp), inv_b = P.b_inv_scale[prob];
+    int acc = 0, buf = 0;
+    uint32_t acc_phase = 0;
+    for (int mt = first; mt < P.n_mtiles; mt += step) {
+      mb_wait(acc_full + acc, acc_phase);
+      asm volatile("tcgen05.fence::after_thread_sync;" ::: "memory");
+      const int64_t m0 = (int64_t)mt * kBM + row_q;
+      const uint32_t taddr = tmem_base + ((uint32_t)(quarter * 32) << 16) + acc * (kAccCols / 2);
+      for (int c0 = 0; c0 < P.NT; c0 += 32) {
+        uint32_t v[32];
+        tmem_ld32_g(taddr + c0, v);
+        asm volatile("tcgen05.wait::ld.sync.aligned;" ::: "memory");
+        if (c0 + 32 >= P.NT) {
+          asm volatile("tcgen05.fence::before_thread_sync;" ::: "memory");
+          __syncwarp();
+          if (lane == 0) mb_arrive(acc_empty + acc);
+        }
+        if (lane == 0) asm volatile("cp.async.bulk.wait_group.read 1;" ::: "memory");
+        __syncwarp();
+#pragma unroll
+        for (int j = 0; j < 32; ++j) v[j] = __float_as_uint(__uint_as_float(v[j]) * inv_a * inv_b);
+        uint8_t* bb = stg + buf * kEpiBuf;
+        const bool wide = c0 + 32 <= P.NT;
+        if (wide) {
+          uint8_t* bx = bb + lane * 128;
+          const int sw = lane & 7;
+#pragma unroll
+          for (int q = 0; q < 8; ++q)
+            *reinterpret_cast<uint4*>(bx + ((q ^ sw) << 4)) = make_uint4(v[4 * q], v[4 * q + 1], v[4 * q + 2], v[4 * q + 3]);
+        } else {
+          uint8_t* bx = bb + lane * 64;
+          const int sw = (lane >> 1) & 3;
+#pragma unroll
+          for (int q = 0; q < 4; ++q)
+            *reinterpret_cast<uint4*>(bx + ((q ^ sw) << 4)) = make_uint4(v[4 * q], v[4 * q + 1], v[4 * q + 2], v[4 * q + 3]);
+        }
+        asm volatile("fence.proxy.async.shared::cta;" ::: "memory");
+        __syncwarp();
+        if (lane == 0) {
+          if (m0 < P.M && c0 < P.N) tma_store_2d(wide ? &maps.c[prob] : &maps.c16[prob], bb, c0, (int)m0);
+          asm volatile("cp.async.bulk.commit_group;" ::: "memory");
+        }
+        buf ^= 1;
+      }
+      if (++acc == 2) { acc = 0; acc_phase ^= 1; }
+    }
+    if (lane == 0) asm volatile("cp.async.bulk.wait_group 0;" ::: "memory");
+  }
+  asm volatile("tcgen05.fence::before_thread_sync;" ::: "memory");
+  __syncthreads();
+  if (warp == 14) {
+    asm volatile("tcgen05.dealloc.cta_group::1.sync.aligned.b32 %0, %1;" ::"r"(tmem_base), "r"(512) : "memory");
+  }
+}
+
+struct PackF16Args {
+  const float* B[kMaxBatch];
+  const float* mul0[kMaxBatch];
+  const float* mul1[kMaxBatch];
+  int64_t sk, sn;
+  int N, K, n_pad, k_pad;
+  __half* packed;
+  float* inv_scale;
+};
+__device__ __forceinline__ float pack_f16_value(const PackF16Args& a, int p, int n, int k) {
+  const float* B = p == 0 ? a.B[0] : (p == 1 ? a.B[1] : a.B[2]);
+  const float* m0 = p == 0 ? a.mul0[0] : (p == 1 ? a.mul0[1] : a.mul0[2]);
+  const float* m1 = p == 0 ? a.mul1[0] : (p == 1 ? a.mul1[1] : a.mul1[2]);
+  float v = B[(int64_t)k * a.sk + (int64_t)n * a.sn];
+  if (m0 != nullptr) v *= m0[n] * (m1 != nullptr ? m1[n] : 1.f);
+  return v;
+}
+__global__ void __launch_bounds__(1024) pack_b_f16_kernel(const PackF16Args a) {
+  __shared__ uint32_t wmax[32];
+  const int p = blockIdx.x;
+  uint32_t m = 0u;
+  for (int i = threadIdx.x; i < a.N * a.K; i += blockDim.x)
+    m = max(m, __float_as_uint(fabsf(pack_f16_value(a, p, i / a.K, i % a.K))));
+  m = __reduce_max_sync(0xFFFFFFFFu, m);
+  if (threadIdx.x % 32 == 0) wmax[threadIdx.x / 32] = m;
+  __syncthreads();
+  for (int w = 0; w < 32; ++w) m = max(m, wmax[w]);
+  const int e = f16_scale_exp(__uint_as_float(m));
+  const float s = exp2_int(e);
+  if (threadIdx.x == 0) a.inv_scale[p] = exp2_int(-e);
+  const int total = a.n_pad * a.k_pad;
+  __half* hi = a.packed + (int64_t)p * 2 * total;
+  for (int i = threadIdx.x; i < total; i += blockDim.x) {
+    const int n = i / a.k_pad, k = i % a.k_pad;
+    const float v = (n < a.N && k < a.K) ? pack_f16_value(a, p, n, k) * s : 0.f;
+    const __half h = __float2half_rn(v);
+    hi[i] = h;
+    hi[total + i] = __float2half_rn(v - __half2float(h));
+  }
+}
+
+struct TilingF16 {
+  int n_kb, nb_b, k_pad, ksteps, NT;
+};
+int make_tiling_f16(int N, int K, TilingF16* t) {
+  if (N <= 0 || K <= 0 || K > kMaxKB * kBK) return 1;
+  t->n_kb = (K + kBK - 1) / kBK;
+  t->nb_b = (K + kF16BK - 1) / kF16BK;
+  t->k_pad = t->nb_b * kF16BK;
+  t->ksteps = (K + kF16UK - 1) / kF16UK;
+  t->NT = (N + 15) / 16 * 16;
+  if (t->NT > kAccCols / 2 || 2 * t->nb_b * t->NT * kF16BK * 2 > kBBudget) return 1;
+  return 0;
+}
+
+int make_map_f16(CUtensorMap* map, const void* ptr, int64_t rows, int64_t cols, int64_t pitch, int box_rows) {
+  EncodeTiledFn enc;
+  if (encode_fn(&enc)) return 1;
+  KGC_REQUIRE((reinterpret_cast<uintptr_t>(ptr) & 15) == 0 && (pitch * 2) % 16 == 0, "operand must be 16-byte aligned with a 16-byte pitch");
+  cuuint64_t dims[2] = {(cuuint64_t)cols, (cuuint64_t)rows};
+  cuuint64_t strides[1] = {(cuuint64_t)pitch * 2};
+  cuuint32_t box[2] = {(cuuint32_t)kF16BK, (cuuint32_t)box_rows};
+  cuuint32_t estr[2] = {1, 1};
+  CUresult r = enc(map, CU_TENSOR_MAP_DATA_TYPE_FLOAT16, 2, const_cast<void*>(ptr), dims, strides, box, estr,
+                   CU_TENSOR_MAP_INTERLEAVE_NONE, CU_TENSOR_MAP_SWIZZLE_128B, CU_TENSOR_MAP_L2_PROMOTION_L2_256B,
+                   CU_TENSOR_MAP_FLOAT_OOB_FILL_NONE);
+  KGC_REQUIRE(r == CUDA_SUCCESS, "cuTensorMapEncodeTiled (fp16) failed (" + std::to_string((int)r) + ")");
+  return 0;
 }
 
 }
@@ -1274,3 +1638,78 @@
                                   float* C, void* workspace, size_t workspace_bytes, void* stream) {
   return launch_gemm_tn_tc(1, &A, lda, &Bt, ldb, K, Ma, Nb, &C, workspace, workspace_bytes, 1, stream);
 }
+
+extern "C" size_t kgc_gemm_f16_packed_b_bytes(int32_t N, int32_t K) {
+  TilingF16 t;
+  if (make_tiling_f16(N, K, &t)) return 0;
+  return (size_t)2 * t.NT * t.k_pad * sizeof(__half);
+}
+
+extern "C" int kgc_gemm_pack_b_f16(int32_t n_prob, const float* const* B, int64_t stride_k, int64_t stride_n,
+                                   const float* const* mul0, const float* const* mul1, int32_t N, int32_t K, void* packed,
+                                   float* inv_scale, void* stream) {
+  TilingF16 t;
+  KGC_REQUIRE(n_prob >= 1 && n_prob <= kMaxBatch, "1..3 operands per launch");
+  KGC_REQUIRE(make_tiling_f16(N, K, &t) == 0, "unsupported fp16-split shape (N <= 112 at K <= 256, N <= 128 at K <= 224)");
+  KGC_REQUIRE(B && packed && inv_scale, "null buffer");
+  PackF16Args a;
+  for (int i = 0; i < kMaxBatch; ++i) {
+    const int j = i < n_prob ? i : 0;
+    KGC_REQUIRE(B[j] != nullptr, "null operand");
+    a.B[i] = B[j];
+    a.mul0[i] = mul0 != nullptr ? mul0[j] : nullptr;
+    a.mul1[i] = mul1 != nullptr ? mul1[j] : nullptr;
+  }
+  a.sk = stride_k; a.sn = stride_n; a.N = N; a.K = K; a.n_pad = t.NT; a.k_pad = t.k_pad;
+  a.packed = static_cast<__half*>(packed); a.inv_scale = inv_scale;
+  pack_b_f16_kernel<<<n_prob, 1024, 0, as_stream(stream)>>>(a);
+  KGC_LAUNCH_CHECK();
+  return 0;
+}
+
+extern "C" int kgc_gemm_nt_f16_batch(int32_t n_prob, const float* const* A, int64_t M, int32_t K, int64_t lda,
+                                     const void* packed_b, const float* b_inv_scale, const uint32_t* a_amax, float a_amax_mul,
+                                     int32_t N, float* const* C, int64_t ldc, const uint8_t* keep, int32_t keep_pitch,
+                                     float keep_scale, void* stream) {
+  TilingF16 t;
+  KGC_REQUIRE(A && packed_b && C && b_inv_scale && a_amax, "null buffer");
+  KGC_REQUIRE(n_prob >= 1 && n_prob <= kMaxBatch, "1..3 problems per launch");
+  KGC_REQUIRE(make_tiling_f16(N, K, &t) == 0, "unsupported fp16-split shape (N <= 112 at K <= 256, N <= 128 at K <= 224)");
+  KGC_REQUIRE(M > 0 && lda >= K && ldc >= N, "bad leading dimensions");
+  KGC_REQUIRE(ldc % 4 == 0, "C needs a 16-byte row pitch (TMA store)");
+  KGC_REQUIRE(keep == nullptr || (keep_pitch % 16 == 0 && keep_pitch >= 8 * kMaxKB && (reinterpret_cast<uintptr_t>(keep) & 15) == 0),
+              "keep flags: one byte per 4 columns, 16-byte aligned rows of at least 64 bytes");
+  GemmMaps maps;
+  const int64_t total = (int64_t)t.NT * t.k_pad;
+  const __half* pb = static_cast<const __half*>(packed_b);
+  for (int i = 0; i < kMaxBatch; ++i) {
+    const int j = i < n_prob ? i : 0;
+    KGC_REQUIRE((reinterpret_cast<uintptr_t>(C[j]) & 15) == 0, "C must be 16-byte aligned (TMA store)");
+    if (make_map_f32(&maps.c[i], C[j], M, N, ldc, 32, CU_TENSOR_MAP_SWIZZLE_128B, 32)) return 1;
+    if (make_map_f32(&maps.c16[i], C[j], M, N, ldc, 32, CU_TENSOR_MAP_SWIZZLE_64B, 16)) return 1;
+    if (make_map_f32(&maps.a[i], A[j], M, K, lda, kBM)) return 1;
+    if (make_map_f16(&maps.bhi[i], pb + 2 * j * total, t.NT, t.k_pad, t.k_pad, t.NT)) return 1;
+    if (make_map_f16(&maps.blo[i], pb + (2 * j + 1) * total, t.NT, t.k_pad, t.k_pad, t.NT)) return 1;
+  }
+  GemmF16Params P;
+  P.M = M; P.n_prob = n_prob; P.N = N; P.K = K;
+  P.n_kb = t.n_kb; P.nb_b = t.nb_b; P.ksteps = t.ksteps; P.NT = t.NT;
+  P.n_mtiles = (int32_t)ceil_div(M, kBM);
+  P.a_amax = a_amax; P.a_amax_mul = a_amax_mul; P.b_inv_scale = b_inv_scale;
+  P.keep = keep; P.keep_pitch = keep_pitch; P.keep_scale = keep_scale;
+  const int tile_b_al = (t.NT * kF16BK * 2 + 1023) & ~1023;
+  const size_t fixed = (size_t)2 * t.nb_b * tile_b_al + kEpiStage + 512 + 1024;
+  int stages = (int)((226 * 1024 - fixed) / kTileA);
+  if (stages > kMaxStages) stages = kMaxStages;
+  KGC_REQUIRE(stages >= 2, "shared-memory plan does not fit");
+  P.stages = stages;
+  const size_t smem = fixed + (size_t)stages * kTileA;
+  static SmemAttrCache attr;
+  KGC_CUDA_TRY(attr.ensure(gemm_f16x2_kernel, smem));
+  int per = kNumSMs / n_prob;
+  if (per > P.n_mtiles) per = P.n_mtiles;
+  if (per < 1) per = 1;
+  gemm_f16x2_kernel<<<per * n_prob, kThreadsG, smem, as_stream(stream)>>>(maps, P);
+  KGC_LAUNCH_CHECK();
+  return 0;
+}
diff --git a/kgc-gcn_b200/csrc/tail.cu b/kgc-gcn_b200/csrc/tail.cu
--- a/kgc-gcn_b200/csrc/tail.cu
+++ b/kgc-gcn_b200/csrc/tail.cu
@@ -258,15 +258,11 @@
   block_store_partials(s1, s2, rl, c, RL, Do4, partials, sm);
 }
 
-__global__ void __launch_bounds__(kThreads)
-tail_bwd_apply_kernel(const float4* __restrict__ g_ent, const float4* __restrict__ pre, const float4* __restrict__ stats,
-                      const float4* __restrict__ gamma, const float4* __restrict__ beta, const double* __restrict__ sums,
-                      int training, int64_t n_rows, int64_t n_rows_global, int Do4, float4* __restrict__ d_out,
-                      const uint8_t* __restrict__ keep, float keep_scale, float4* __restrict__ d_res2,
-                      const uint8_t* __restrict__ out_keep, float out_scale) {
-  const int64_t n4 = n_rows * (int64_t)Do4;
-  const int64_t i = blockIdx.x * (int64_t)kThreads + threadIdx.x;
-  if (i >= n4) return;
+__device__ __forceinline__ float4 tail_bwd_apply_elem(
+    const float4* __restrict__ g_ent, const float4* __restrict__ pre, const float4* __restrict__ stats,
+    const float4* __restrict__ gamma, const float4* __restrict__ beta, const double* __restrict__ sums, int training,
+    int64_t n_rows_global, int Do4, float4* __restrict__ d_out, const uint8_t* __restrict__ keep, float keep_scale,
+    float4* __restrict__ d_res2, const uint8_t* __restrict__ out_keep, float out_scale, int64_t n4, int64_t i) {
   const int c = (int)(i % Do4);
   float4 g = __ldg(g_ent + i);
   const float4 v = __ldg(pre + i);
@@ -301,6 +297,33 @@
     d_res2[n4 + i] = make_float4((kb & 16u) ? third.x * s : 0.f, (kb & 32u) ? third.y * s : 0.f, (kb & 64u) ? third.z * s : 0.f,
                                  (kb & 128u) ? third.w * s : 0.f);
   }
+  return third;
+}
+
+__global__ void __launch_bounds__(kThreads)
+tail_bwd_apply_kernel(const float4* __restrict__ g_ent, const float4* __restrict__ pre, const float4* __restrict__ stats,
+                      const float4* __restrict__ gamma, const float4* __restrict__ beta, const double* __restrict__ sums,
+                      int training, int64_t n_rows, int64_t n_rows_global, int Do4, float4* __restrict__ d_out,
+                      const uint8_t* __restrict__ keep, float keep_scale, float4* __restrict__ d_res2,
+                      const uint8_t* __restrict__ out_keep, float out_scale, uint32_t* __restrict__ amax) {
+  const int64_t n4 = n_rows * (int64_t)Do4;
+  const int64_t i = blockIdx.x * (int64_t)kThreads + threadIdx.x;
+  float4 t = make_float4(0.f, 0.f, 0.f, 0.f);
+  if (i < n4) t = tail_bwd_apply_elem(g_ent, pre, stats, gamma, beta, sums, training, n_rows_global, Do4, d_out, keep,
+                                      keep_scale, d_res2, out_keep, out_scale, n4, i);
+  if (amax == nullptr) return;
+  __shared__ uint32_t wmax[kThreads / 32];
+  uint32_t m = max(max(__float_as_uint(fabsf(t.x)), __float_as_uint(fabsf(t.y))),
+                   max(__float_as_uint(fabsf(t.z)), __float_as_uint(fabsf(t.w))));
+  m = __reduce_max_sync(0xFFFFFFFFu, m);
+  if (threadIdx.x % 32 == 0) wmax[threadIdx.x / 32] = m;
+  __syncthreads();
+  if (threadIdx.x == 0) {
+#pragma unroll
+    for (int w = 1; w < kThreads / 32; ++w) m = max(m, wmax[w]);
+    uint32_t* slot = amax + (blockIdx.x % kAmaxSlots) * kAmaxStride;
+    if (m > *reinterpret_cast<volatile uint32_t*>(slot)) atomicMax(slot, m);
+  }
 }
 
 inline int check_dout(int32_t Dout) { return (Dout <= 0 || Dout % 4 != 0 || Dout > 1024) ? 1 : 0; }
@@ -440,13 +463,14 @@
 extern "C" int kgc_tail_bwd_apply(const float* g_ent, const float* pre, const float* stats, const float* gamma,
                                   const float* beta, const double* sums, int32_t training, int64_t n_rows,
                                   int64_t n_rows_global, int32_t Dout, float* d_out, const uint8_t* keep, float keep_scale,
-                                  float* d_res2, const uint8_t* out_keep, float out_scale, void* stream) {
+                                  float* d_res2, const uint8_t* out_keep, float out_scale, uint32_t* amax, void* stream) {
   KGC_REQUIRE(check_dout(Dout) == 0, "Dout must be a multiple of 4 and <= 1024");
   const int Do4 = Dout / 4;
   const int64_t n4 = n_rows * Do4;
+  if (amax != nullptr) KGC_CUDA_TRY(cudaMemsetAsync(amax, 0, kAmaxSlots * kAmaxStride * sizeof(uint32_t), as_stream(stream)));
   tail_bwd_apply_kernel<<<(unsigned)ceil_div(n4, kThreads), kThreads, 0, as_stream(stream)>>>(
       (const float4*)g_ent, (const float4*)pre, (const float4*)stats, (const float4*)gamma, (const float4*)beta, sums,
-      training, n_rows, n_rows_global, Do4, (float4*)d_out, keep, keep_scale, (float4*)d_res2, out_keep, out_scale);
-  KGC_LAUNCH_CHECK();
-  return 0;
-}
+      training, n_rows, n_rows_global, Do4, (float4*)d_out, keep, keep_scale, (float4*)d_res2, out_keep, out_scale, amax);
+  KGC_LAUNCH_CHECK();
+  return 0;
+}
diff --git a/profiles/gemm_f16_ab.py b/profiles/gemm_f16_ab.py
--- /dev/null
+++ b/profiles/gemm_f16_ab.py
@@ -0,0 +1,79 @@
+import argparse
+import json
+import os
+import subprocess
+import sys
+
+import torch
+
+sys.dont_write_bytecode = True
+sys.path.insert(0, os.path.dirname(os.path.dirname(os.path.abspath(__file__))))
+
+
+def card():
+    try:
+        q = subprocess.run(['nvidia-smi', '--query-gpu=name,power.limit,clocks.max.sm', '--format=csv,noheader'],
+                           stdout=subprocess.PIPE, text=True, timeout=30).stdout.strip().splitlines()[0]
+    except Exception as exc:
+        q = 'nvidia-smi unavailable: {!r}'.format(exc)
+    return q
+
+
+def main():
+    ap = argparse.ArgumentParser()
+    ap.add_argument('--reps', type=int, default=10)
+    ap.add_argument('--rows', type=int, default=4594485)
+    args = ap.parse_args()
+    from kgc_gcn_b200 import _lib
+    from kgc_gcn_b200.conv import AMAX_WORDS, _pack_b, gemm_nt_batch, gemm_nt_f16_batch, pack_b_f16
+    M, K, N, p = args.rows, 200, 100, 0.3
+    ks = 1.0 / (1.0 - p)
+    g = torch.Generator(device='cuda').manual_seed(0)
+    d_out = torch.randn(M, K, device='cuda', generator=g) * 1e-8
+    pitch = int(_lib.lib().kgc_keep_pitch())
+    keep = torch.randint(0, 256, (M, pitch), device='cuda', dtype=torch.int32, generator=g).to(torch.uint8)
+    w = [torch.randn(N, K, device='cuda', generator=g) * 0.1 for _ in range(3)]
+    packs32 = [_pack_b(wi.t()) for wi in w]
+    packed16, inv16 = pack_b_f16(w, 1, K, N, K)
+    amax = torch.zeros(AMAX_WORDS, dtype=torch.int32, device='cuda')
+    amax[0] = torch.tensor([float(d_out.abs().max())], dtype=torch.float32).view(torch.int32)[0]
+    outs = [torch.empty(M, N, device='cuda') for _ in range(3)]
+    flush = torch.empty(256 << 20, dtype=torch.uint8, device='cuda')
+
+    def old():
+        gemm_nt_batch([d_out] * 3, packs32, outs, keep=keep, keep_scale=ks)
+
+    def new():
+        gemm_nt_f16_batch([d_out] * 3, packed16, inv16, amax, ks, outs, keep=keep, keep_scale=ks)
+
+    def timed(fn):
+        flush.random_(0, 255)
+        e0, e1 = torch.cuda.Event(enable_timing=True), torch.cuda.Event(enable_timing=True)
+        e0.record()
+        fn()
+        e1.record()
+        e1.synchronize()
+        return e0.elapsed_time(e1)
+
+    for fn in (old, new, old, new):
+        fn()
+    torch.cuda.synchronize()
+    t = {'3xtf32': [], 'f16x2': []}
+    for _ in range(args.reps):
+        t['3xtf32'].append(timed(old))
+        t['f16x2'].append(timed(new))
+    old()
+    ref = [o.clone() for o in outs]
+    new()
+    err = max(float((a - b).abs().max()) / float(b.abs().max()) for a, b in zip(outs, ref))
+    res = {'card': card(), 'shape': {'M': M, 'K': K, 'N': N, 'problems': 3, 'keep_flags': True},
+           'l2': 'overwritten (256 MB) before every timed launch', 'reps': args.reps,
+           'max_norm_rel_new_vs_old': err}
+    for k, v in t.items():
+        s = sorted(v)
+        res[k + '_ms'] = {'median': s[len(s) // 2], 'min': s[0], 'max': s[-1]}
+    print(json.dumps(res))
+
+
+if __name__ == '__main__':
+    main()
diff --git a/profiles/layer_step_ab.py b/profiles/layer_step_ab.py
--- /dev/null
+++ b/profiles/layer_step_ab.py
@@ -0,0 +1,86 @@
+import argparse
+import json
+import os
+import subprocess
+import sys
+
+import torch
+
+sys.dont_write_bytecode = True
+ROOT = os.path.dirname(os.path.dirname(os.path.abspath(__file__)))
+sys.path.insert(0, ROOT)
+import bench
+
+
+def card():
+    try:
+        return subprocess.run(['nvidia-smi', '--query-gpu=name,power.limit,clocks.max.sm', '--format=csv,noheader'],
+                              stdout=subprocess.PIPE, text=True, timeout=30).stdout.strip().splitlines()[0]
+    except Exception as exc:
+        return 'nvidia-smi unavailable: {!r}'.format(exc)
+
+
+def main():
+    ap = argparse.ArgumentParser()
+    ap.add_argument('workload', nargs='?', default='wikidata5m')
+    ap.add_argument('--reps', type=int, default=12)
+    args = ap.parse_args()
+    import kgc_gcn_b200 as k
+    dev = torch.device('cuda', 0)
+    case = bench.LayerCase(k, bench.oracle(), args.workload, dev)
+    flush = bench.Flusher(dev)
+    modes = ('3', '1')
+    graphs = {}
+    for m in modes:
+        os.environ['KGC_TAIL_PLANES'] = m
+        side = torch.cuda.Stream()
+        side.wait_stream(torch.cuda.current_stream())
+        with torch.cuda.stream(side):
+            for _ in range(3):
+                case.step()
+        torch.cuda.current_stream().wait_stream(side)
+        torch.cuda.synchronize()
+        for t in case.leaves:
+            t.grad = None
+        g = torch.cuda.CUDAGraph()
+        with torch.cuda.graph(g):
+            case.step()
+        graphs[m] = g
+    for m in modes * 3:
+        graphs[m].replay()
+    torch.cuda.synchronize()
+    times = {m: [] for m in modes}
+    for _ in range(args.reps):
+        for m in modes:
+            flush()
+            a, b = torch.cuda.Event(enable_timing=True), torch.cuda.Event(enable_timing=True)
+            a.record()
+            graphs[m].replay()
+            b.record()
+            b.synchronize()
+            times[m].append(a.elapsed_time(b))
+    res = {'card': card(), 'workload': args.workload, 'reps': args.reps, 'l2': 'flushed before every replay'}
+    for m in modes:
+        s = sorted(times[m])
+        res['planes_' + m + '_ms'] = {'median': s[len(s) // 2], 'min': s[0], 'max': s[-1]}
+    print(json.dumps(res), flush=True)
+    from torch.profiler import ProfilerActivity, profile
+    for m in modes:
+        os.environ['KGC_TAIL_PLANES'] = m
+        case.step()
+        torch.cuda.synchronize()
+        with profile(activities=[ProfilerActivity.CUDA]) as prof:
+            case.step()
+            torch.cuda.synchronize()
+        per = {}
+        for e in prof.events():
+            if e.device_type == torch.autograd.DeviceType.CUDA:
+                name = e.name if len(e.name) < 60 else e.name[:57] + '...'
+                per[name] = per.get(name, 0.0) + e.time_range.elapsed_us() / 1e3
+        top = sorted(per.items(), key=lambda kv: -kv[1])[:16]
+        print(json.dumps({'planes': m, 'kernel_ms': {n: round(t, 3) for n, t in top},
+                          'sum_ms': round(sum(per.values()), 3)}), flush=True)
+
+
+if __name__ == '__main__':
+    main()
```

New measurement: 874.8 million, median of 6. About the same (+0.5%).
